# JuliaSmoothOptimizers/Krylov.jl

Measured on NVIDIA B200. Metric: CG iterations/s, higher is better.
Workload: dtype f64

## Files before the change

### include/krylov_b200.h

```cpp
#ifndef KRYLOV_B200_H
#define KRYLOV_B200_H

#ifdef __cplusplus
extern "C" {
#endif


#ifndef KRYLOV_H

#define KRYLOV_VERSION_MAJOR 0
#define KRYLOV_VERSION_MINOR 10
#define KRYLOV_VERSION_PATCH 8

typedef enum { KRYLOV_FLOAT32 = 0, KRYLOV_FLOAT64 = 1, KRYLOV_COMPLEX32 = 2, KRYLOV_COMPLEX64 = 3 } KrylovDataType;

typedef enum { KRYLOV_CPU = 0, KRYLOV_CUDA = 1 } KrylovDeviceType;

typedef enum {
  KRYLOV_CG = 0, KRYLOV_CR = 1, KRYLOV_SYMMLQ = 2, KRYLOV_MINRES = 3, KRYLOV_MINRES_QLP = 4, KRYLOV_DIOM = 5,
  KRYLOV_DQGMRES = 6, KRYLOV_FOM = 7, KRYLOV_GMRES = 8, KRYLOV_FGMRES = 9, KRYLOV_BICGSTAB = 10, KRYLOV_CGS = 11,
  KRYLOV_BILQ = 12, KRYLOV_QMR = 13, KRYLOV_USYMLQ = 14, KRYLOV_USYMQR = 15, KRYLOV_TRICG = 16, KRYLOV_TRIMR = 17,
  KRYLOV_TRILQR = 18, KRYLOV_BILQR = 19, KRYLOV_LSLQ = 20, KRYLOV_LSQR = 21, KRYLOV_LSMR = 22, KRYLOV_USYMLQR = 23,
  KRYLOV_CGLS = 24, KRYLOV_CRLS = 25, KRYLOV_CGNE = 26, KRYLOV_CRMR = 27, KRYLOV_CRAIG = 28, KRYLOV_CRAIGMR = 29,
  KRYLOV_LNLQ = 30, KRYLOV_GPMR = 31, KRYLOV_CAR = 32, KRYLOV_MINARES = 33
} KrylovSolverType;

typedef enum { KRYLOV_BLOCK_GMRES = 0, KRYLOV_BLOCK_MINRES = 1 } KrylovBlockSolverType;

typedef void (*KrylovMatvec)(const void *x, void *y, void *userdata);
typedef void (*KrylovBlockMatvec)(const void *X, void *Y, int p, void *userdata);

typedef struct {
  int memory;
  int window;
} KrylovWorkspaceOptions;

typedef struct {
  double atol;
  double rtol;
  int itmax;
  int verbose;
  double lambda;
  double tau;
  double nu;
  double timemax;
  double radius;
  int restart;
  int reorthogonalization;
  int linesearch;
} KrylovOptions;

#endif

int krylov_workspace_create(KrylovSolverType solver, int m, int n, KrylovDataType dtype, KrylovDeviceType device,
                            const KrylovWorkspaceOptions *wopts, void **ws_out);
KrylovWorkspaceOptions krylov_default_workspace_options(void);
KrylovOptions krylov_default_options(void);
void krylov_get_version(int *major, int *minor, int *patch);
int krylov_solve(void *ws, KrylovMatvec matvec_A, KrylovMatvec matvec_At, KrylovMatvec matvec_M, KrylovMatvec matvec_N,
                 const void *b, const void *c, void *userdata, const KrylovOptions *opts);
int krylov_get_x(void *ws, void *x, int n);
int krylov_get_y(void *ws, void *y, int m);
int krylov_is_solved(void *ws);
int krylov_niter(void *ws);
double krylov_elapsed_time(void *ws);
int krylov_warm_start(void *ws, const void *x0, int n);
int krylov_warm_start2(void *ws, const void *x0, const void *y0, int nx, int ny);
int krylov_workspace_free(void *ws);

int krylov_block_workspace_create(KrylovBlockSolverType solver, int m, int n, int p, KrylovDataType dtype,
                                  KrylovDeviceType device, const KrylovWorkspaceOptions *wopts, void **ws_out);
int krylov_block_solve(void *ws, KrylovBlockMatvec matvec_A, KrylovBlockMatvec matvec_M, KrylovBlockMatvec matvec_N,
                       const void *B, void *userdata, const KrylovOptions *opts);
int krylov_block_get_X(void *ws, void *X, int n, int p);
int krylov_block_is_solved(void *ws);
int krylov_block_niter(void *ws);
double krylov_block_elapsed_time(void *ws);
int krylov_block_warm_start(void *ws, const void *x0, int n, int p);
int krylov_block_workspace_free(void *ws);
long long krylov_b200_block_qr_fallbacks(void *ws);


int krylov_b200_device_count(void);
int krylov_b200_set_device(int device);
const char *krylov_b200_last_error(void);

int krylov_b200_set_operator_csr(void *ws, int n, long long nnz, const void *rowptr, const void *colind,
                                 const void *values, int index_base, int index_bytes, int location);
int krylov_b200_share_operator(void *ws, void *src);
int krylov_b200_attach_csr(void *ws, void *csr);
int krylov_b200_set_preconditioner_diag(void *ws, int which, const void *d, int location);
int krylov_b200_set_preconditioner_blockdiag(void *ws, int which, int bs, const void *blocks, int location);

#define KRYLOV_B200_CG_LANCZOS 100

typedef struct {
  int history;
  int ldiv;
  double etol;
  double conlim;
  int fused;
  int batch;
  int (*callback)(void *ws, void *user);
  void *callback_user;
  int time_kernels;
  int check_curvature;
  double cr_gamma;
} KrylovB200Options;
KrylovB200Options krylov_b200_default_options(void);
int krylov_b200_set_options(void *ws, const KrylovB200Options *opts);

typedef struct {
  int niter;
  int solved;
  int inconsistent;
  int indefinite;
  int npcCount;
  int nresiduals;
  int nAresiduals;
  int nAcond;
  double allocation_timer;
  double timer;
  char status[96];
  double Anorm;
} KrylovB200Stats;
int krylov_b200_get_stats(void *ws, KrylovB200Stats *out);
int krylov_b200_get_history(void *ws, int which, double *out, int cap);
int krylov_b200_get_vector(void *ws, const char *name, void **dev_ptr);
int krylov_b200_get_kernel_times(void *ws, double *out3);
long long krylov_b200_launch_count(void *ws);
void *krylov_b200_stream(void *ws);
int krylov_b200_wait_stream(void *ws, void *producer_stream);

int krylov_b200_dist_handle_bytes(void);
int krylov_b200_dist_init(void *ws, int rank, int world, int nhalo, const int *halo_rank, const int *halo_off);
int krylov_b200_dist_set_push(void *ws, int nranges, const int *ranges4, const int *nhalo_all);
int krylov_b200_dist_set_sendlist(void *ws, int nsend, const int *rows, const int *peers, const int *slots,
                                  const int *nhalo_all, long long nglobal);
int krylov_b200_dist_export(void *ws, void *handles_out);
int krylov_b200_dist_import(void *ws, const void *all_handles);

void *kb200_ctx_create(int device);
void kb200_ctx_destroy(void *ctx);
int kb200_sync(void *ctx);
void *kb200_alloc(long long bytes);
int kb200_free(void *p);
int kb200_h2d(void *dst, const void *src, long long bytes);
int kb200_d2h(void *dst, const void *src, long long bytes);
int kb200_dot(void *ctx, int dtype, int n, const void *x, const void *y, double *result);
int kb200_nrm2(void *ctx, int dtype, int n, const void *x, double *result);
int kb200_axpy(void *ctx, int dtype, int n, double s, const void *x, void *y);
int kb200_axpby(void *ctx, int dtype, int n, double s, const void *x, double t, void *y);
int kb200_scal(void *ctx, int dtype, int n, double s, void *x);
int kb200_copy(void *ctx, int dtype, int n, void *y, const void *x);
int kb200_scalcopy(void *ctx, int dtype, int n, void *y, double s, const void *x);
int kb200_divcopy(void *ctx, int dtype, int n, void *y, const void *x, double s);
int kb200_fill(void *ctx, int dtype, int n, void *x, double v);
void *kb200_csr_create(void *ctx, int dtype, int n, long long nnz, const void *rowptr, const void *colind,
                       const void *values, int index_base, int index_bytes, int location);
void kb200_csr_destroy(void *csr);
void *kb200_csr_read_mtx(void *ctx, const char *path, int dtype);
void *kb200_csr_transpose(void *ctx, void *csr);
int kb200_csr_info(void *csr, int *n, long long *nnz);
int kb200_csr_download(void *ctx, void *csr, int *rowptr, int *colind, void *values);
int kb200_mtx_read(const char *path, int *n, long long *nnz, int *rowptr, int *colind, double *values);
int kb200_host_householder(int m, int k, double *Q, double *R, double *tau, int compact);
int kb200_host_cholqr_factors(int p, const double *G, double *R, double *Rinv);
int kb200_host_householder_signs(int p, const double *top, double *s);
int kb200_spmv_csr(void *ctx, void *csr, const void *x, void *y, int variant);
int kb200_csr_plan(void *csr, long long *out7);

#ifdef __cplusplus
}
#endif
#endif
```

### krylov.jl_b200/csrc/capi.cu

```cuda
#include <cmath>
#include <cstring>
#include <memory>
#include <mutex>
#include <unordered_map>

#include "../../include/krylov_b200.h"
#include "kb_internal.h"
#include "block.h"
#include "mtx.h"
#include "dense_small.h"

using namespace kb;

namespace {

thread_local std::string g_last_error;
int g_device = -1;

struct CsrAny {
  int dtype = 1;
  Csr<double> d;
  Csr<float> f;
  Ctx* owner_ctx = nullptr;
  ~CsrAny() { csr_free(d); csr_free(f); }
};

struct Handle {
  int solver = 0, dtype = 1, device_kind = 0;
  bool block = false;
  int p = 0;
  void* ws = nullptr;
  std::shared_ptr<CsrAny> csr;
  void* Mdiag = nullptr;
  void* Ndiag = nullptr;
  void* Pblk[2] = {nullptr, nullptr};
  void* Pblk_inv[2] = {nullptr, nullptr};
  int Pbs[2] = {0, 0};
  KrylovB200Options ext;
  void *hx = nullptr, *hy = nullptr;
};

std::mutex g_mu;
std::unordered_map<void*, Handle*> g_handles;

Handle* lookup_any(void* p) {
  std::lock_guard<std::mutex> lk(g_mu);
  auto it = g_handles.find(p);
  return it == g_handles.end() ? nullptr : it->second;
}
Handle* lookup(void* p) { Handle* h = lookup_any(p); return (h && !h->block) ? h : nullptr; }
Handle* lookup_block(void* p) { Handle* h = lookup_any(p); return (h && h->block) ? h : nullptr; }

int fail(const char* where, const std::exception& e) {
  g_last_error = std::string(where) + ": " + e.what();
  fprintf(stderr, "[krylov_b200] %s\n", g_last_error.c_str());
  return -1;
}
int fail(const char* where, const char* msg) {
  g_last_error = std::string(where) + ": " + msg;
  fprintf(stderr, "[krylov_b200] %s\n", g_last_error.c_str());
  return -1;
}

bool supported_solver(int s) {
  return s == S_CG || s == S_MINRES || s == S_GMRES || s == S_BICGSTAB || s == S_FOM || s == S_FGMRES || s == S_CGS ||
         s == S_CG_LANCZOS || s == S_CR || s == S_DIOM || s == S_DQGMRES;
}

int pick_device() {
  int cnt = 0;
  if (cudaGetDeviceCount(&cnt) != cudaSuccess || cnt <= 0) {
    cudaGetLastError();
    throw std::runtime_error("no usable CUDA device: libkrylov_b200 has no CPU compute path");
  }
  int dev = g_device;
  if (dev < 0) { if (cudaGetDevice(&dev) != cudaSuccess) dev = 0; }
  if (dev >= cnt) throw std::runtime_error("device index out of range");
  cudaDeviceProp prop;
  KB_CUDA(cudaGetDeviceProperties(&prop, dev));
  if (prop.major < 10) throw std::runtime_error("libkrylov_b200 is built for sm_100a only");
  return dev;
}

template <class T> Workspace<T>* W(Handle* h) { return reinterpret_cast<Workspace<T>*>(h->ws); }
template <class T> BlockWorkspace<T>* BW(Handle* h) { return reinterpret_cast<BlockWorkspace<T>*>(h->ws); }
Ctx& ctx_of(Handle* h) {
  if (h->block) return h->dtype == KRYLOV_FLOAT64 ? BW<double>(h)->ctx : BW<float>(h)->ctx;
  return h->dtype == KRYLOV_FLOAT64 ? W<double>(h)->ctx : W<float>(h)->ctx;
}
int n_of(Handle* h) {
  if (h->block) return h->dtype == KRYLOV_FLOAT64 ? BW<double>(h)->n : BW<float>(h)->n;
  return h->dtype == KRYLOV_FLOAT64 ? W<double>(h)->n : W<float>(h)->n;
}
template <class T> Csr<T>& csr_of(CsrAny& a);
template <> Csr<double>& csr_of<double>(CsrAny& a) { return a.d; }
template <> Csr<float>& csr_of<float>(CsrAny& a) { return a.f; }

template <class T> void destroy_handle(Handle* h) {
  Workspace<T>* ws = W<T>(h);
  if (ws) {
    KB_CUDA(cudaSetDevice(ws->ctx.device));
    if (ws->ctx.stream) cudaStreamSynchronize(ws->ctx.stream);
  }
  h->csr.reset();
  dev_free(h->Mdiag); dev_free(h->Ndiag);
  for (int w = 0; w < 2; w++) { dev_free(h->Pblk[w]); dev_free(h->Pblk_inv[w]); }
  if (h->hx) cudaFreeHost(h->hx);
  if (h->hy) cudaFreeHost(h->hy);
  ws_destroy<T>(ws);
  delete h;
}

template <class T> const T* stage_in(Handle* h, Workspace<T>* ws, const void* src, T*& buf) {
  if (!src) return nullptr;
  if (h->device_kind == KRYLOV_CUDA) return (const T*)src;
  if (!buf) buf = dev_alloc<T>((size_t)ws->n);
  KB_CUDA(cudaMemcpyAsync(buf, src, sizeof(T) * (size_t)ws->n, cudaMemcpyHostToDevice, ws->ctx.stream));
  return buf;
}

template <class T> LinOp<T> make_cb_op(Handle* h, Workspace<T>* ws, KrylovMatvec fn, void* ud) {
  LinOp<T> op;
  op.n = ws->n;
  if (!fn) return op;
  op.fn = fn; op.userdata = ud;
  if (h->device_kind == KRYLOV_CUDA) { op.kind = LinOp<T>::DEV_CB; return op; }
  op.kind = LinOp<T>::HOST_CB;
  if (!h->hx) {
    KB_CUDA(cudaHostAlloc(&h->hx, sizeof(T) * (size_t)ws->n, cudaHostAllocDefault));
    KB_CUDA(cudaHostAlloc(&h->hy, sizeof(T) * (size_t)ws->n, cudaHostAllocDefault));
  }
  op.hx = (T*)h->hx; op.hy = (T*)h->hy;
  return op;
}

SolveOpts map_opts(const Handle* h, const KrylovOptions* o) {
  SolveOpts s;
  KrylovOptions d = krylov_default_options();
  if (!o) o = &d;
  s.atol = std::isnan(o->atol) ? -1 : o->atol;
  s.rtol = std::isnan(o->rtol) ? -1 : o->rtol;
  s.itmax = o->itmax;
  s.verbose = o->verbose;
  s.timemax = std::isnan(o->timemax) ? INFINITY : o->timemax;
  if (h->solver == S_CG || h->solver == S_CR) { s.radius = o->radius; s.linesearch = o->linesearch != 0; }
  if (h->solver == S_DIOM || h->solver == S_DQGMRES) s.reorthogonalization = o->reorthogonalization != 0;
  s.cr_gamma = std::isnan(h->ext.cr_gamma) ? -1 : h->ext.cr_gamma;
  if (h->solver == S_MINRES) { s.lambda = o->lambda; s.linesearch = o->linesearch != 0; }
  if (h->solver == S_GMRES || h->solver == S_FGMRES || h->solver == S_FOM) {
    s.restart = o->restart != 0; s.reorthogonalization = o->reorthogonalization != 0;
  }
  s.check_curvature = h->ext.check_curvature != 0;
  s.history = h->ext.history != 0;
  s.ldiv = h->ext.ldiv != 0;
  s.etol = std::isnan(h->ext.etol) ? -1 : h->ext.etol;
  s.conlim = std::isnan(h->ext.conlim) ? -1 : h->ext.conlim;
  s.fused = h->ext.fused;
  s.persist = h->ext.fused != 2;
  s.batch = h->ext.batch;
  s.callback = h->ext.callback;
  s.callback_user = h->ext.callback_user;
  s.time_kernels = h->ext.time_kernels;
  return s;
}

template <class T>
int do_solve(Handle* h, KrylovMatvec fA, KrylovMatvec fM, KrylovMatvec fN, const void* b, const void* c, void* ud,
             const KrylovOptions* opts) {
  Workspace<T>* ws = W<T>(h);
  KB_CUDA(cudaSetDevice(ws->ctx.device));
  SolveOpts so = map_opts(h, opts);
  LinOp<T> A;
  if (fA) A = make_cb_op<T>(h, ws, fA, ud);
  else if (h->csr) {
    A.kind = LinOp<T>::CSR; A.csr = &csr_of<T>(*h->csr); A.n = ws->n;
    const long long ncols = (long long)ws->n + (ws->dist.world > 1 ? ws->dist.halo.nhalo : 0);
    if (A.csr->n != ws->n || A.csr->max_col >= ncols)
      throw std::runtime_error("CSR operator: size or column index inconsistent with the workspace (n = " + std::to_string(ws->n) +
                               ", operator rows = " + std::to_string(A.csr->n) + ", largest column = " + std::to_string(A.csr->max_col) + ")");
  }
  else throw std::runtime_error("no operator: pass matvec_A or attach one with krylov_b200_set_operator_csr");
  if (A.kind == LinOp<T>::CSR && A.csr->n != ws->n) throw std::runtime_error("(workspace.m, workspace.n) is inconsistent with size(A)");
  LinOp<T> M = make_cb_op<T>(h, ws, fM, ud), N = make_cb_op<T>(h, ws, fN, ud);
  if (!fM && h->Mdiag) { M.kind = LinOp<T>::DIAG; M.diag = (const T*)h->Mdiag; }
  if (!fN && h->Ndiag) { N.kind = LinOp<T>::DIAG; N.diag = (const T*)h->Ndiag; }
  if (!fM && !h->Mdiag && h->Pblk[0]) { M.kind = LinOp<T>::BDIAG; M.blocks = (const T*)h->Pblk[0]; M.blocks_inv = (const T*)h->Pblk_inv[0]; M.bs = h->Pbs[0]; M.n = ws->n; }
  if (!fN && !h->Ndiag && h->Pblk[1]) { N.kind = LinOp<T>::BDIAG; N.blocks = (const T*)h->Pblk[1]; N.blocks_inv = (const T*)h->Pblk_inv[1]; N.bs = h->Pbs[1]; N.n = ws->n; }
  if (!b) throw std::runtime_error("b is NULL");
  const T* bd = stage_in<T>(h, ws, b, ws->bbuf);
  dist_check_alive(ws->ctx);
  switch (h->solver) {
    case S_CG: cg_solve<T>(*ws, A, bd, M, so); break;
    case S_MINRES: minres_solve<T>(*ws, A, bd, M, so); break;
    case S_GMRES: gmres_solve<T>(*ws, A, bd, M, N, so); break;
    case S_FOM: fom_solve<T>(*ws, A, bd, M, N, so); break;
    case S_FGMRES: fgmres_solve<T>(*ws, A, bd, M, N, so); break;
    case S_CG_LANCZOS: cg_lanczos_solve<T>(*ws, A, bd, M, so); break;
    case S_CR: cr_solve<T>(*ws, A, bd, M, so); break;
    case S_DQGMRES: dqgmres_solve<T>(*ws, A, bd, M, N, so); break;
    case S_DIOM: diom_solve<T>(*ws, A, bd, M, N, so); break;
    case S_CGS: {
      const T* cd = stage_in<T>(h, ws, c, ws->cbuf);
      cgs_solve<T>(*ws, A, bd, cd, M, N, so);
      break;
    }
    case S_BICGSTAB: {
      const T* cd = stage_in<T>(h, ws, c, ws->cbuf);
      bicgstab_solve<T>(*ws, A, bd, cd, M, N, so);
      break;
    }
  }
  dist_check_alive(ws->ctx);
  return 0;
}

template <class T> int do_get_x(Handle* h, void* x, int n) {
  Workspace<T>* ws = W<T>(h);
  if (n > ws->n) n = ws->n;
  KB_CUDA(cudaSetDevice(ws->ctx.device));
  KB_CUDA(cudaMemcpyAsync(x, ws->x, sizeof(T) * (size_t)n,
                          h->device_kind == KRYLOV_CUDA ? cudaMemcpyDeviceToDevice : cudaMemcpyDeviceToHost, ws->ctx.stream));
  ws->ctx.sync();
  return 0;
}

template <class T> int do_warm_start(Handle* h, const void* x0, int n) {
  Workspace<T>* ws = W<T>(h);
  if (n != ws->n) throw std::runtime_error("x0 should have size n");
  KB_CUDA(cudaSetDevice(ws->ctx.device));
  if (!ws->dx) ws->dx = dev_alloc<T>((size_t)ws->n);
  KB_CUDA(cudaMemcpyAsync(ws->dx, x0, sizeof(T) * (size_t)n,
                          h->device_kind == KRYLOV_CUDA ? cudaMemcpyDeviceToDevice : cudaMemcpyHostToDevice, ws->ctx.stream));
  ws->ctx.sync();
  ws->warm_start = true;
  return 0;
}

template <class T> Stats& stats_of(Handle* h) { return W<T>(h)->stats; }
Stats& stats_any(Handle* h) {
  if (h->block) return h->dtype == KRYLOV_FLOAT64 ? BW<double>(h)->stats : BW<float>(h)->stats;
  return h->dtype == KRYLOV_FLOAT64 ? stats_of<double>(h) : stats_of<float>(h);
}

template <class T> void* vec_by_name(Workspace<T>* ws, const char* nm) {
  struct { const char* n; T* p; } tab[] = {
      {"x", ws->x}, {"dx", ws->dx}, {"r", ws->r}, {"p", ws->p}, {"Ap", ws->Ap}, {"z", ws->z}, {"npc_dir", ws->npc_dir},
      {"v", ws->kind == S_MINRES ? (ws->vv ? ws->vv : ws->r2) : ws->v}, {"s", ws->s}, {"qd", ws->qd}, {"t", ws->t}, {"yz", ws->yz},
      {"r1", ws->r1}, {"r2", ws->r2}, {"w1", ws->w1}, {"w2", ws->w2}, {"y", ws->y}, {"w", ws->w}, {"q", ws->q},
      {"u", ws->u}, {"ts", ws->ts}, {"vw", ws->vw}, {"Mv", ws->Mv}, {"Mv_prev", ws->Mv_prev}, {"Mv_next", ws->Mv_next}};
  for (auto& e : tab) if (!strcmp(e.n, nm)) return e.p;
  if (nm[0] == 'P' && nm[1]) { int i = atoi(nm + 1); if (i >= 1 && i <= (int)ws->Z.size()) return ws->Z[i - 1]; return nullptr; }
  if (!strcmp(nm, "Ar")) return ws->Ap;
  if (!strcmp(nm, "Mq")) return ws->z;
  if (nm[0] == 'Z') { int i = atoi(nm + 1); if (i >= 1 && i <= (int)ws->Z.size()) return ws->Z[i - 1]; return nullptr; }
  if (nm[0] == 'V') { int i = atoi(nm + 1); if (i >= 1 && i <= (int)ws->V.size()) return ws->V[i - 1]; }
  return nullptr;
}

}

extern "C" {

int krylov_workspace_create(KrylovSolverType solver, int m, int n, KrylovDataType dtype, KrylovDeviceType device,
                            const KrylovWorkspaceOptions* wopts, void** ws_out) {
  try {
    if (!supported_solver((int)solver) || (dtype != KRYLOV_FLOAT32 && dtype != KRYLOV_FLOAT64)) return -2;
    if (device != KRYLOV_CPU && device != KRYLOV_CUDA) return fail("krylov_workspace_create", "unknown device");
    if (!ws_out) return fail("krylov_workspace_create", "ws_out is NULL");
    if (m < 0 || n < 0) return fail("krylov_workspace_create", "negative dimension");
    const int dev = pick_device();
    const int memory = wopts ? wopts->memory : 0, window = wopts ? wopts->window : 0;
    Handle* h = new Handle();
    h->solver = (int)solver; h->dtype = (int)dtype; h->device_kind = (int)device;
    h->ext = krylov_b200_default_options();
    try {
      if (dtype == KRYLOV_FLOAT64) h->ws = ws_create<double>((SolverKind)solver, m, n, memory, window, dev);
      else h->ws = ws_create<float>((SolverKind)solver, m, n, memory, window, dev);
    } catch (...) { delete h; throw; }
    {
      std::lock_guard<std::mutex> lk(g_mu);
      g_handles[h] = h;
    }
    *ws_out = h;
    return 0;
  } catch (const std::exception& e) { return fail("krylov_workspace_create", e); }
}

KrylovWorkspaceOptions krylov_default_workspace_options(void) { KrylovWorkspaceOptions w = {0, 0}; return w; }

KrylovOptions krylov_default_options(void) {
  KrylovOptions o;
  o.atol = NAN; o.rtol = NAN; o.itmax = 0; o.verbose = 0; o.lambda = 0.0; o.tau = NAN; o.nu = NAN;
  o.timemax = NAN; o.radius = 0.0; o.restart = 0; o.reorthogonalization = 0; o.linesearch = 0;
  return o;
}

void krylov_get_version(int* major, int* minor, int* patch) {
  if (major) *major = KRYLOV_VERSION_MAJOR;
  if (minor) *minor = KRYLOV_VERSION_MINOR;
  if (patch) *patch = KRYLOV_VERSION_PATCH;
}

int krylov_solve(void* ws, KrylovMatvec matvec_A, KrylovMatvec matvec_At, KrylovMatvec matvec_M, KrylovMatvec matvec_N,
                 const void* b, const void* c, void* userdata, const KrylovOptions* opts) {
  (void)matvec_At;
  try {
    Handle* h = lookup(ws);
    if (!h) return fail("krylov_solve", "unknown workspace handle");
    return h->dtype == KRYLOV_FLOAT64 ? do_solve<double>(h, matvec_A, matvec_M, matvec_N, b, c, userdata, opts)
                                      : do_solve<float>(h, matvec_A, matvec_M, matvec_N, b, c, userdata, opts);
  } catch (const std::exception& e) { return fail("krylov_solve", e); }
}

int krylov_get_x(void* ws, void* x, int n) {
  try {
    Handle* h = lookup(ws);
    if (!h) return fail("krylov_get_x", "unknown workspace handle");
    return h->dtype == KRYLOV_FLOAT64 ? do_get_x<double>(h, x, n) : do_get_x<float>(h, x, n);
  } catch (const std::exception& e) { return fail("krylov_get_x", e); }
}

int krylov_get_y(void* ws, void* y, int m) {
  (void)y; (void)m;
  Handle* h = lookup(ws);
  if (!h) return fail("krylov_get_y", "unknown workspace handle");
  return -2;
}

int krylov_is_solved(void* ws) { Handle* h = lookup(ws); return h ? (stats_any(h).solved ? 1 : 0) : -1; }
int krylov_niter(void* ws) { Handle* h = lookup(ws); return h ? stats_any(h).niter : -1; }
double krylov_elapsed_time(void* ws) { Handle* h = lookup(ws); return h ? stats_any(h).timer : -1.0; }

int krylov_warm_start(void* ws, const void* x0, int n) {
  try {
    Handle* h = lookup(ws);
    if (!h) return fail("krylov_warm_start", "unknown workspace handle");
    return h->dtype == KRYLOV_FLOAT64 ? do_warm_start<double>(h, x0, n) : do_warm_start<float>(h, x0, n);
  } catch (const std::exception& e) { return fail("krylov_warm_start", e); }
}

int krylov_warm_start2(void* ws, const void* x0, const void* y0, int nx, int ny) {
  (void)x0; (void)y0; (void)nx; (void)ny;
  Handle* h = lookup(ws);
  if (!h) return fail("krylov_warm_start2", "unknown workspace handle");
  return -2;
}

static void destroy_any(Handle* h) {
  if (h->block) {
    Ctx& c = ctx_of(h);
    KB_CUDA(cudaSetDevice(c.device));
    if (c.stream) cudaStreamSynchronize(c.stream);
    h->csr.reset();
    dev_free(h->Mdiag); dev_free(h->Ndiag);
    if (h->hx) cudaFreeHost(h->hx);
    if (h->hy) cudaFreeHost(h->hy);
    if (h->dtype == KRYLOV_FLOAT64) block_ws_destroy<double>(BW<double>(h)); else block_ws_destroy<float>(BW<float>(h));
    delete h;
  } else if (h->dtype == KRYLOV_FLOAT64) {
    destroy_handle<double>(h);
  } else {
    destroy_handle<float>(h);
  }
}

int krylov_workspace_free(void* ws) {
  Handle* h = nullptr;
  {
    std::lock_guard<std::mutex> lk(g_mu);
    auto it = g_handles.find(ws);
    if (it == g_handles.end()) return 1;
    h = it->second;
    g_handles.erase(it);
  }
  try {
    destroy_any(h);
  } catch (const std::exception& e) { fail("krylov_workspace_free", e); }
  return 0;
}

int krylov_block_workspace_create(KrylovBlockSolverType solver, int m, int n, int p, KrylovDataType dtype, KrylovDeviceType device,
                                  const KrylovWorkspaceOptions* wopts, void** ws_out) {
  try {
    if (solver != KRYLOV_BLOCK_GMRES || (dtype != KRYLOV_FLOAT32 && dtype != KRYLOV_FLOAT64)) return -2;
    if (device != KRYLOV_CPU && device != KRYLOV_CUDA) return fail("krylov_block_workspace_create", "unknown device");
    if (!ws_out) return fail("krylov_block_workspace_create", "ws_out is NULL");
    if (m < 0 || n < 0 || p < 1) return fail("krylov_block_workspace_create", "bad dimensions");
    const int dev = pick_device();
    const int memory = wopts ? wopts->memory : 0;
    Handle* h = new Handle();
    h->block = true; h->p = p; h->solver = (int)solver; h->dtype = (int)dtype; h->device_kind = (int)device;
    h->ext = krylov_b200_default_options();
    try {
      if (dtype == KRYLOV_FLOAT64) h->ws = block_ws_create<double>(m, n, p, memory, dev);
      else h->ws = block_ws_create<float>(m, n, p, memory, dev);
    } catch (...) { delete h; throw; }
    {
      std::lock_guard<std::mutex> lk(g_mu);
      g_handles[h] = h;
    }
    *ws_out = h;
    return 0;
  } catch (const std::exception& e) { return fail("krylov_block_workspace_create", e); }
}

}
namespace {
template <class T> BlockOp<T> make_block_cb(Handle* h, KrylovBlockMatvec fn, void* ud) {
  BlockOp<T> op;
  if (!fn) return op;
  op.fn = fn; op.userdata = ud;
  op.kind = h->device_kind == KRYLOV_CUDA ? BlockOp<T>::DEV_CB : BlockOp<T>::HOST_CB;
  return op;
}
template <class T> const T* stage_block(Handle* h, BlockWorkspace<T>* ws, const void* src) {
  if (h->device_kind == KRYLOV_CUDA) return (const T*)src;
  const size_t np = (size_t)ws->n * ws->p;
  if (!ws->tmp2) ws->tmp2 = dev_alloc<T>(np);
  KB_CUDA(cudaMemcpyAsync(ws->tmp2, src, sizeof(T) * np, cudaMemcpyHostToDevice, ws->ctx.stream));
  return ws->tmp2;
}
template <class T> int do_block_solve(Handle* h, KrylovBlockMatvec fA, KrylovBlockMatvec fM, KrylovBlockMatvec fN, const void* B,
                                      void* ud, const KrylovOptions* opts) {
  BlockWorkspace<T>* ws = BW<T>(h);
  KB_CUDA(cudaSetDevice(ws->ctx.device));
  SolveOpts so = map_opts(h, opts);
  KrylovOptions d = krylov_default_options();
  const KrylovOptions* o = opts ? opts : &d;
  so.restart = o->restart != 0; so.reorthogonalization = o->reorthogonalization != 0;
  BlockOp<T> A = make_block_cb<T>(h, fA, ud);
  if (!fA) {
    if (!h->csr) throw std::runtime_error("no operator: pass matvec_A or attach one with krylov_b200_set_operator_csr");
    A.kind = BlockOp<T>::CSR; A.csr = &csr_of<T>(*h->csr);
    if (A.csr->n != ws->n) throw std::runtime_error("(workspace.m, workspace.n) is inconsistent with size(A)");
  }
  BlockOp<T> M = make_block_cb<T>(h, fM, ud), N = make_block_cb<T>(h, fN, ud);
  if (!fM && h->Mdiag) { M.kind = BlockOp<T>::DIAG; M.diag = (const T*)h->Mdiag; }
  if (!fN && h->Ndiag) { N.kind = BlockOp<T>::DIAG; N.diag = (const T*)h->Ndiag; }
  if (!B) throw std::runtime_error("B is NULL");
  const T* Bd = stage_block<T>(h, ws, B);
  block_gmres_solve<T>(*ws, A, Bd, M, N, so);
  return 0;
}
template <class T> int do_block_get_X(Handle* h, void* X, int n, int p) {
  BlockWorkspace<T>* ws = BW<T>(h);
  if (n != ws->n || p != ws->p) throw std::runtime_error("X should have size n x p");
  KB_CUDA(cudaSetDevice(ws->ctx.device));
  const size_t np = (size_t)n * p;
  if (h->device_kind == KRYLOV_CUDA) { block_get_X<T>(*ws, (T*)X); return 0; }
  block_get_X<T>(*ws, ws->tmp);
  KB_CUDA(cudaMemcpyAsync(X, ws->tmp, sizeof(T) * np, cudaMemcpyDeviceToHost, ws->ctx.stream));
  ws->ctx.sync();
  return 0;
}
template <class T> int do_block_warm_start(Handle* h, const void* X0, int n, int p) {
  BlockWorkspace<T>* ws = BW<T>(h);
  if (n != ws->n || p != ws->p) throw std::runtime_error("X0 should have size n x p");
  KB_CUDA(cudaSetDevice(ws->ctx.device));
  block_warm_start<T>(*ws, stage_block<T>(h, ws, X0));
  return 0;
}
}
extern "C" {

int krylov_block_solve(void* ws, KrylovBlockMatvec matvec_A, KrylovBlockMatvec matvec_M, KrylovBlockMatvec matvec_N, const void* B,
                       void* userdata, const KrylovOptions* opts) {
  try {
    Handle* h = lookup_block(ws);
    if (!h) return fail("krylov_block_solve", "unknown block workspace handle");
    return h->dtype == KRYLOV_FLOAT64 ? do_block_solve<double>(h, matvec_A, matvec_M, matvec_N, B, userdata, opts)
                                      : do_block_solve<float>(h, matvec_A, matvec_M, matvec_N, B, userdata, opts);
  } catch (const std::exception& e) { return fail("krylov_block_solve", e); }
}
int krylov_block_get_X(void* ws, void* X, int n, int p) {
  try {
    Handle* h = lookup_block(ws);
    if (!h || !X) return fail("krylov_block_get_X", "bad arguments");
    return h->dtype == KRYLOV_FLOAT64 ? do_block_get_X<double>(h, X, n, p) : do_block_get_X<float>(h, X, n, p);
  } catch (const std::exception& e) { return fail("krylov_block_get_X", e); }
}
int krylov_block_is_solved(void* ws) { Handle* h = lookup_block(ws); return h ? (stats_any(h).solved ? 1 : 0) : -1; }
int krylov_block_niter(void* ws) { Handle* h = lookup_block(ws); return h ? stats_any(h).niter : -1; }
double krylov_block_elapsed_time(void* ws) { Handle* h = lookup_block(ws); return h ? stats_any(h).timer : -1.0; }
int krylov_block_warm_start(void* ws, const void* x0, int n, int p) {
  try {
    Handle* h = lookup_block(ws);
    if (!h || !x0) return fail("krylov_block_warm_start", "bad arguments");
    return h->dtype == KRYLOV_FLOAT64 ? do_block_warm_start<double>(h, x0, n, p) : do_block_warm_start<float>(h, x0, n, p);
  } catch (const std::exception& e) { return fail("krylov_block_warm_start", e); }
}
long long krylov_b200_block_qr_fallbacks(void* ws) {
  Handle* h = lookup_block(ws);
  if (!h) return -1;
  return h->dtype == KRYLOV_FLOAT64 ? BW<double>(h)->qr_fallbacks : BW<float>(h)->qr_fallbacks;
}
int krylov_block_workspace_free(void* ws) {
  try {
    Handle* h = lookup_block(ws);
    if (!h) return 1;
    {
      std::lock_guard<std::mutex> lk(g_mu);
      g_handles.erase(ws);
    }
    destroy_any(h);
    return 0;
  } catch (const std::exception& e) { return fail("krylov_block_workspace_free", e); }
}

int krylov_b200_device_count(void) {
  int cnt = 0;
  if (cudaGetDeviceCount(&cnt) != cudaSuccess) { cudaGetLastError(); return 0; }
  return cnt;
}
int krylov_b200_set_device(int device) { g_device = device; return 0; }
const char* krylov_b200_last_error(void) { return g_last_error.c_str(); }

int krylov_b200_set_operator_csr(void* ws, int n, long long nnz, const void* rowptr, const void* colind, const void* values,
                                 int index_base, int index_bytes, int location) {
  try {
    Handle* h = lookup_any(ws);
    if (!h) return fail("krylov_b200_set_operator_csr", "unknown workspace handle");
    auto a = std::make_shared<CsrAny>();
    a->dtype = h->dtype;
    Ctx& cx = ctx_of(h);
    KB_CUDA(cudaSetDevice(cx.device));
    if (n != n_of(h)) throw std::runtime_error("(workspace.m, workspace.n) is inconsistent with size(A)");
    if (h->dtype == KRYLOV_FLOAT64)
      csr_upload<double>(cx, a->d, n, nnz, rowptr, colind, (const double*)values, index_base, index_bytes, location != 0);
    else
      csr_upload<float>(cx, a->f, n, nnz, rowptr, colind, (const float*)values, index_base, index_bytes, location != 0);
    h->csr = a;
    return 0;
  } catch (const std::exception& e) { return fail("krylov_b200_set_operator_csr", e); }
}

int krylov_b200_share_operator(void* ws, void* src) {
  Handle* h = lookup_any(ws); Handle* s = lookup_any(src);
  if (!h || !s) return fail("krylov_b200_share_operator", "unknown workspace handle");
  if (!s->csr || s->dtype != h->dtype) return fail("krylov_b200_share_operator", "source has no CSR operator of this dtype");
  h->csr = s->csr;
  return 0;
}

int krylov_b200_attach_csr(void* ws, void* csr) {
  Handle* h = lookup_any(ws);
  if (!h || !csr) return fail("krylov_b200_attach_csr", "bad arguments");
  CsrAny* a = (CsrAny*)csr;
  if (a->dtype != h->dtype) return fail("krylov_b200_attach_csr", "dtype mismatch");
  h->csr = std::shared_ptr<CsrAny>(std::shared_ptr<CsrAny>(), a);
  return 0;
}

int krylov_b200_set_preconditioner_diag(void* ws, int which, const void* d, int location) {
  try {
    Handle* h = lookup_any(ws);
    if (!h) return fail("krylov_b200_set_preconditioner_diag", "unknown workspace handle");
    void*& slot = which == 0 ? h->Mdiag : h->Ndiag;
    if (!d) { dev_free(slot); slot = nullptr; return 0; }
    const size_t esz = h->dtype == KRYLOV_FLOAT64 ? 8 : 4;
    const int n = n_of(h);
    KB_CUDA(cudaSetDevice(ctx_of(h).device));
    if (!slot) slot = dev_alloc<char>(esz * (size_t)n);
    KB_CUDA(cudaMemcpy(slot, d, esz * (size_t)n, location ? cudaMemcpyDeviceToDevice : cudaMemcpyHostToDevice));
    return 0;
  } catch (const std::exception& e) { return fail("krylov_b200_set_preconditioner_diag", e); }
}

int krylov_b200_set_preconditioner_blockdiag(void* ws, int which, int bs, const void* blocks, int location) {
  try {
    Handle* h = lookup(ws);
    if (!h) return fail("krylov_b200_set_preconditioner_blockdiag", "unknown (single right-hand side) workspace handle");
    if (which != 0 && which != 1) return fail("krylov_b200_set_preconditioner_blockdiag", "which must be 0 (M) or 1 (N)");
    dev_free(h->Pblk[which]); dev_free(h->Pblk_inv[which]);
    h->Pblk[which] = h->Pblk_inv[which] = nullptr; h->Pbs[which] = 0;
    if (!blocks) return 0;
    if (bs < 2 || bs > 8) return fail("krylov_b200_set_preconditioner_blockdiag", "block size must be in 2..8");
    const size_t esz = h->dtype == KRYLOV_FLOAT64 ? 8 : 4;
    const int n = n_of(h);
    const size_t cnt = (size_t)((n + bs - 1) / bs) * bs * bs;
    Ctx& c = ctx_of(h);
    KB_CUDA(cudaSetDevice(c.device));
    h->Pblk[which] = dev_alloc<char>(esz * cnt);
    h->Pblk_inv[which] = dev_alloc<char>(esz * cnt);
    h->Pbs[which] = bs;
    KB_CUDA(cudaMemcpyAsync(h->Pblk[which], blocks, esz * cnt, location ? cudaMemcpyDeviceToDevice : cudaMemcpyHostToDevice, c.stream));
    int* dsing = nullptr;
    KB_CUDA(cudaMalloc((void**)&dsing, sizeof(int)));
    KB_CUDA(cudaMemsetAsync(dsing, 0, sizeof(int), c.stream));
    if (h->dtype == KRYLOV_FLOAT64) k_blockdiag_invert<double>(c, n, bs, (const double*)h->Pblk[which], (double*)h->Pblk_inv[which], dsing);
    else k_blockdiag_invert<float>(c, n, bs, (const float*)h->Pblk[which], (float*)h->Pblk_inv[which], dsing);
    int sing = 0;
    KB_CUDA(cudaMemcpyAsync(&sing, dsing, sizeof(int), cudaMemcpyDeviceToHost, c.stream));
    c.sync();
    cudaFree(dsing);
    if (sing) fprintf(stderr, "[krylov_b200] warning: a diagonal block of the block-Jacobi preconditioner is singular (its inverse, used by ldiv = true, is zero)\n");
    return 0;
  } catch (const std::exception& e) { return fail("krylov_b200_set_preconditioner_blockdiag", e); }
}

KrylovB200Options krylov_b200_default_options(void) {
  KrylovB200Options o;
  memset(&o, 0, sizeof(o));
  o.etol = NAN; o.conlim = NAN; o.fused = 1; o.cr_gamma = NAN;
  return o;
}

int krylov_b200_set_options(void* ws, const KrylovB200Options* opts) {
  Handle* h = lookup_any(ws);
  if (!h) return fail("krylov_b200_set_options", "unknown workspace handle");
  h->ext = opts ? *opts : krylov_b200_default_options();
  return 0;
}

int krylov_b200_get_stats(void* ws, KrylovB200Stats* out) {
  Handle* h = lookup_any(ws);
  if (!h || !out) return fail("krylov_b200_get_stats", "unknown workspace handle");
  const Stats& s = stats_any(h);
  memset(out, 0, sizeof(*out));
  out->niter = s.niter; out->solved = s.solved; out->inconsistent = s.inconsistent; out->indefinite = s.indefinite;
  out->npcCount = s.npcCount; out->nresiduals = (int)s.residuals.size(); out->nAresiduals = (int)s.Aresiduals.size();
  out->nAcond = (int)s.Acond.size(); out->allocation_timer = s.allocation_timer; out->timer = s.timer;
  strncpy(out->status, s.status.c_str(), sizeof(out->status) - 1);
  out->Anorm = s.Anorm;
  return 0;
}

int krylov_b200_get_history(void* ws, int which, double* out, int cap) {
  Handle* h = lookup_any(ws);
  if (!h) return fail("krylov_b200_get_history", "unknown workspace handle");
  if (!out || cap < 0) return fail("krylov_b200_get_history", "bad arguments (out is NULL or cap < 0)");
  const Stats& s = stats_any(h);
  const std::vector<double>& v = which == 0 ? s.residuals : which == 1 ? s.Aresiduals : s.Acond;
  int k = (int)v.size() < cap ? (int)v.size() : cap;
  for (int i = 0; i < k; i++) out[i] = v[i];
  return k;
}

int krylov_b200_get_vector(void* ws, const char* name, void** dev_ptr) {
  Handle* h = lookup(ws);
  if (!h || !name || !dev_ptr) return fail("krylov_b200_get_vector", "bad arguments");
  void* p = h->dtype == KRYLOV_FLOAT64 ? vec_by_name<double>(W<double>(h), name) : vec_by_name<float>(W<float>(h), name);
  *dev_ptr = p;
  return p ? 0 : -2;
}

int krylov_b200_get_kernel_times(void* ws, double* out) {
  Handle* h = lookup(ws);
  if (!h || !out) return fail("krylov_b200_get_kernel_times", "bad arguments");
  if (h->dtype == KRYLOV_FLOAT64) { auto* w = W<double>(h); out[0] = w->k1_ms; out[1] = w->k2_ms; out[2] = w->timed_pairs; }
  else { auto* w = W<float>(h); out[0] = w->k1_ms; out[1] = w->k2_ms; out[2] = w->timed_pairs; }
  return 0;
}

long long krylov_b200_launch_count(void* ws) {
  Handle* h = lookup_any(ws);
  if (!h) return -1;
  return ctx_of(h).launches;
}

void* krylov_b200_stream(void* ws) {
  Handle* h = lookup_any(ws);
  if (!h) return nullptr;
  return (void*)ctx_of(h).stream;
}

int krylov_b200_wait_stream(void* ws, void* producer_stream) {
  try {
    Handle* h = lookup_any(ws);
    if (!h) return fail("krylov_b200_wait_stream", "unknown workspace handle");
    Ctx& c = ctx_of(h);
    KB_CUDA(cudaSetDevice(c.device));
    cudaEvent_t ev;
    KB_CUDA(cudaEventCreateWithFlags(&ev, cudaEventDisableTiming));
    cudaError_t e1 = cudaEventRecord(ev, (cudaStream_t)producer_stream);
    cudaError_t e2 = e1 == cudaSuccess ? cudaStreamWaitEvent(c.stream, ev, 0) : e1;
    cudaEventDestroy(ev);
    if (e2 != cudaSuccess) throw std::runtime_error(cudaGetErrorString(e2));
    return 0;
  } catch (const std::exception& e) { return fail("krylov_b200_wait_stream", e); }
}

}
namespace {
constexpr int kIpcHandles = 6;
constexpr size_t kMailBytes = kMailWords * sizeof(unsigned long long);

template <class T> int dist_init_t(Handle* h, int rank, int world, int nhalo, const int* halo_rank, const int* halo_off) {
  Workspace<T>* ws = W<T>(h);
  if (world < 1 || world > kMaxRanks || rank < 0 || rank >= world) throw std::runtime_error("bad rank/world");
  KB_CUDA(cudaSetDevice(ws->ctx.device));
  if (h->solver == S_CG) {
    KB_CUDA(cudaStreamSynchronize(ws->ctx.stream));
    const size_t len = (size_t)ws->n + (size_t)(nhalo > 0 ? nhalo : 0);
    T** bufs[3] = {&ws->r, &ws->p, &ws->p2};
    for (T** b : bufs) {
      dev_free(*b);
      *b = dev_alloc<T>(len);
      KB_CUDA(cudaMemset(*b, 0, sizeof(T) * len));
    }
  }
  ws->dist.rank = rank; ws->dist.world = world;
  int *dr = nullptr, *dof = nullptr;
  KB_CUDA(cudaMalloc((void**)&dr, sizeof(int) * (size_t)(nhalo > 0 ? nhalo : 1)));
  KB_CUDA(cudaMalloc((void**)&dof, sizeof(int) * (size_t)(nhalo > 0 ? nhalo : 1)));
  if (nhalo > 0) {
    KB_CUDA(cudaMemcpy(dr, halo_rank, sizeof(int) * (size_t)nhalo, cudaMemcpyHostToDevice));
    KB_CUDA(cudaMemcpy(dof, halo_off, sizeof(int) * (size_t)nhalo, cudaMemcpyHostToDevice));
  }
  ws->dist.halo = HaloMap{ws->n, nhalo, dr, dof};
  KB_CUDA(cudaMalloc(&ws->dist.mailbox, kMailBytes));
  KB_CUDA(cudaMemset(ws->dist.mailbox, 0, kMailBytes));
  ws->dist.halo_buf = dev_alloc<T>(3 * (size_t)(nhalo > 0 ? nhalo : 1));
  KB_CUDA(cudaMemset(ws->dist.halo_buf, 0, sizeof(T) * 3 * (size_t)(nhalo > 0 ? nhalo : 1)));
  ws->dist.npush = 0;
  ws->dist.xhalo = dev_alloc<T>(2 * (size_t)(nhalo > 0 ? nhalo : 1));
  KB_CUDA(cudaMemset(ws->dist.xhalo, 0, sizeof(T) * 2 * (size_t)(nhalo > 0 ? nhalo : 1)));
  ws->dist.nglobal = ws->n;
  if (h->solver != S_CG) for (int i = 0; i < 3; i++) KB_CUDA(cudaMalloc(&ws->dist.dummy[i], 256));
  return 0;
}

template <class T> int dist_export_t(Handle* h, void* out) {
  Workspace<T>* ws = W<T>(h);
  if (!ws->dist.mailbox) throw std::runtime_error("call krylov_b200_dist_init first");
  KB_CUDA(cudaSetDevice(ws->ctx.device));
  cudaIpcMemHandle_t* hs = (cudaIpcMemHandle_t*)out;
  void* vr = ws->kind == S_CG ? (void*)ws->r : ws->dist.dummy[0];
  void* vp = ws->kind == S_CG ? (void*)ws->p : ws->dist.dummy[1];
  void* vp2 = ws->kind == S_CG ? (void*)ws->p2 : ws->dist.dummy[2];
  void* ptrs[kIpcHandles] = {vr, vp, vp2, ws->dist.mailbox, ws->dist.halo_buf, ws->dist.xhalo};
  for (int i = 0; i < kIpcHandles; i++) KB_CUDA(cudaIpcGetMemHandle(&hs[i], ptrs[i]));
  return 0;
}

template <class T> int dist_import_t(Handle* h, const void* all) {
  Workspace<T>* ws = W<T>(h);
  auto& D = ws->dist;
  KB_CUDA(cudaSetDevice(ws->ctx.device));
  const cudaIpcMemHandle_t* hs = (const cudaIpcMemHandle_t*)all;
  DistComm hc;
  memset(&hc, 0, sizeof(hc));
  hc.rank = D.rank; hc.world = D.world;
  {
    const char* es = getenv("KB200_DIST_TIMEOUT_S");
    double secs = es ? atof(es) : 30.0;
    if (!(secs > 0)) secs = 30.0;
    int khz = 0;
    cudaDeviceGetAttribute(&khz, cudaDevAttrClockRate, ws->ctx.device);
    hc.timeout_cycles = (long long)(secs * 1e3 * (khz > 0 ? khz : 1965000));
  }
  for (int k = 0; k < D.world; k++) {
    void* ptr[kIpcHandles];
    if (k == D.rank) {
      ptr[0] = ws->r; ptr[1] = ws->p; ptr[2] = ws->p2; ptr[3] = D.mailbox; ptr[4] = D.halo_buf; ptr[5] = D.xhalo;
    } else {
      for (int i = 0; i < kIpcHandles; i++) {
        KB_CUDA(cudaIpcOpenMemHandle(&ptr[i], hs[k * kIpcHandles + i], cudaIpcMemLazyEnablePeerAccess));
        D.opened.push_back(ptr[i]);
      }
    }
    D.r_peer[k] = (T*)ptr[0]; D.bufA_peer[k] = (T*)ptr[1]; D.bufB_peer[k] = (T*)ptr[2];
    D.halo_buf_peer[k] = (T*)ptr[4];
    D.xhalo_peer[k] = (T*)ptr[5];
    hc.mail[k] = (unsigned long long*)ptr[3];
  }
  D.swapped = false;
  DistExchange* ex = ws->ctx.dex ? ws->ctx.dex : new DistExchange();
  memset(ex, 0, sizeof(*ex));
  ex->nsend = D.nsend; ex->send_row = D.send_row; ex->send_peer = D.send_peer; ex->send_slot = D.send_slot;
  for (int k = 0; k < D.world; k++) { ex->xhalo_peer[k] = D.xhalo_peer[k]; ex->nhalo_peer[k] = D.nhalo_peer[k]; }
  ex->xhalo = D.xhalo; ex->nhalo = D.halo.nhalo; ex->nloc = ws->n; ex->count = 0;
  ws->ctx.dex = ex;
  if (!ws->ctx.dcomm) KB_CUDA(cudaMalloc((void**)&ws->ctx.dcomm, sizeof(DistComm)));
  KB_CUDA(cudaMemcpy(ws->ctx.dcomm, &hc, sizeof(DistComm), cudaMemcpyHostToDevice));
  return 0;
}
}
extern "C" {

int krylov_b200_dist_handle_bytes(void) { return (int)(kIpcHandles * sizeof(cudaIpcMemHandle_t)); }

int krylov_b200_dist_init(void* ws, int rank, int world, int nhalo, const int* halo_rank, const int* halo_off) {
  try {
    Handle* h = lookup(ws);
    if (!h) return fail("krylov_b200_dist_init", "unknown workspace handle");
    return h->dtype == KRYLOV_FLOAT64 ? dist_init_t<double>(h, rank, world, nhalo, halo_rank, halo_off)
                                      : dist_init_t<float>(h, rank, world, nhalo, halo_rank, halo_off);
  } catch (const std::exception& e) { return fail("krylov_b200_dist_init", e); }
}
int krylov_b200_dist_set_sendlist(void* ws, int nsend, const int* rows, const int* peers, const int* slots,
                                  const int* nhalo_all, long long nglobal) {
  try {
    Handle* h = lookup(ws);
    if (!h) return fail("krylov_b200_dist_set_sendlist", "unknown workspace handle");
    auto apply = [&](auto* w) {
      KB_CUDA(cudaSetDevice(w->ctx.device));
      auto up = [&](const int* src) {
        int* d = nullptr;
        KB_CUDA(cudaMalloc((void**)&d, sizeof(int) * (size_t)(nsend > 0 ? nsend : 1)));
        if (nsend > 0) KB_CUDA(cudaMemcpy(d, src, sizeof(int) * (size_t)nsend, cudaMemcpyHostToDevice));
        return d;
      };
      w->dist.send_row = up(rows); w->dist.send_peer = up(peers); w->dist.send_slot = up(slots);
      w->dist.nsend = nsend;
      for (int k = 0; k < w->dist.world; k++) w->dist.nhalo_peer[k] = nhalo_all[k];
      w->dist.nglobal = nglobal;
    };
    if (h->dtype == KRYLOV_FLOAT64) apply(W<double>(h)); else apply(W<float>(h));
    return 0;
  } catch (const std::exception& e) { return fail("krylov_b200_dist_set_sendlist", e); }
}
int krylov_b200_dist_set_push(void* ws, int nranges, const int* ranges4, const int* nhalo_all) {
  try {
    Handle* h = lookup(ws);
    if (!h) return fail("krylov_b200_dist_set_push", "unknown workspace handle");
    if (nranges < 0 || nranges > kMaxPushRanges) return fail("krylov_b200_dist_set_push", "too many ranges (pull mode stays on)");
    auto apply = [&](auto* w) {
      for (int q = 0; q < nranges; q++) w->dist.push[q] = PushRange{ranges4[4 * q], ranges4[4 * q + 1], ranges4[4 * q + 2], ranges4[4 * q + 3]};
      for (int k = 0; k < w->dist.world; k++) w->dist.nhalo_peer[k] = nhalo_all[k];
      w->dist.npush = nranges;
    };
    if (h->dtype == KRYLOV_FLOAT64) apply(W<double>(h)); else apply(W<float>(h));
    return 0;
  } catch (const std::exception& e) { return fail("krylov_b200_dist_set_push", e); }
}
int krylov_b200_dist_export(void* ws, void* handles_out) {
  try {
    Handle* h = lookup(ws);
    if (!h) return fail("krylov_b200_dist_export", "unknown workspace handle");
    return h->dtype == KRYLOV_FLOAT64 ? dist_export_t<double>(h, handles_out) : dist_export_t<float>(h, handles_out);
  } catch (const std::exception& e) { return fail("krylov_b200_dist_export", e); }
}
int krylov_b200_dist_import(void* ws, const void* all_handles) {
  try {
    Handle* h = lookup(ws);
    if (!h) return fail("krylov_b200_dist_import", "unknown workspace handle");
    return h->dtype == KRYLOV_FLOAT64 ? dist_import_t<double>(h, all_handles) : dist_import_t<float>(h, all_handles);
  } catch (const std::exception& e) { return fail("krylov_b200_dist_import", e); }
}

void* kb200_ctx_create(int device) {
  try {
    if (device < 0) device = pick_device();
    Ctx* c = new Ctx();
    c->init(device);
    return c;
  } catch (const std::exception& e) { fail("kb200_ctx_create", e); return nullptr; }
}
void kb200_ctx_destroy(void* ctx) {
  Ctx* c = (Ctx*)ctx;
  if (!c) return;
  cudaSetDevice(c->device);
  if (c->stream) cudaStreamSynchronize(c->stream);
  c->destroy();
  delete c;
}
int kb200_sync(void* ctx) {
  try { ((Ctx*)ctx)->sync(); return 0; } catch (const std::exception& e) { return fail("kb200_sync", e); }
}
void* kb200_alloc(long long bytes) {
  try { return dev_alloc<char>((size_t)bytes); } catch (const std::exception& e) { fail("kb200_alloc", e); return nullptr; }
}
int kb200_free(void* p) { dev_free(p); return 0; }
int kb200_h2d(void* dst, const void* src, long long bytes) {
  return cudaMemcpy(dst, src, (size_t)bytes, cudaMemcpyHostToDevice) == cudaSuccess ? 0 : fail("kb200_h2d", "cudaMemcpy failed");
}
int kb200_d2h(void* dst, const void* src, long long bytes) {
  return cudaMemcpy(dst, src, (size_t)bytes, cudaMemcpyDeviceToHost) == cudaSuccess ? 0 : fail("kb200_d2h", "cudaMemcpy failed");
}

#define FLAT(name, body_d, body_f)                                                        \
  try {                                                                                   \
    Ctx& c = *(Ctx*)ctx;                                                                  \
    if (dtype == KRYLOV_FLOAT64) { typedef double T; (void)sizeof(T); body_d; }           \
    else if (dtype == KRYLOV_FLOAT32) { typedef float T; (void)sizeof(T); body_f; }       \
    else return -2;                                                                       \
    return 0;                                                                             \
  } catch (const std::exception& e) { return fail(name, e); }

int kb200_dot(void* ctx, int dtype, int n, const void* x, const void* y, double* result) {
  FLAT("kb200_dot", *result = k_dot<T>(c, n, (const T*)x, (const T*)y), *result = k_dot<T>(c, n, (const T*)x, (const T*)y))
}
int kb200_nrm2(void* ctx, int dtype, int n, const void* x, double* result) {
  FLAT("kb200_nrm2", *result = k_nrm2<T>(c, n, (const T*)x), *result = k_nrm2<T>(c, n, (const T*)x))
}
int kb200_axpy(void* ctx, int dtype, int n, double s, const void* x, void* y) {
  FLAT("kb200_axpy", k_axpy<T>(c, n, (T)s, (const T*)x, (T*)y), k_axpy<T>(c, n, (T)s, (const T*)x, (T*)y))
}
int kb200_axpby(void* ctx, int dtype, int n, double s, const void* x, double t, void* y) {
  FLAT("kb200_axpby", k_axpby<T>(c, n, (T)s, (const T*)x, (T)t, (T*)y), k_axpby<T>(c, n, (T)s, (const T*)x, (T)t, (T*)y))
}
int kb200_scal(void* ctx, int dtype, int n, double s, void* x) {
  FLAT("kb200_scal", k_scal<T>(c, n, (T)s, (T*)x), k_scal<T>(c, n, (T)s, (T*)x))
}
int kb200_copy(void* ctx, int dtype, int n, void* y, const void* x) {
  FLAT("kb200_copy", k_copy<T>(c, n, (T*)y, (const T*)x), k_copy<T>(c, n, (T*)y, (const T*)x))
}
int kb200_scalcopy(void* ctx, int dtype, int n, void* y, double s, const void* x) {
  FLAT("kb200_scalcopy", k_scalcopy<T>(c, n, (T*)y, (T)s, (const T*)x), k_scalcopy<T>(c, n, (T*)y, (T)s, (const T*)x))
}
int kb200_divcopy(void* ctx, int dtype, int n, void* y, const void* x, double s) {
  FLAT("kb200_divcopy", k_divcopy<T>(c, n, (T*)y, (const T*)x, (T)s), k_divcopy<T>(c, n, (T*)y, (const T*)x, (T)s))
}
int kb200_fill(void* ctx, int dtype, int n, void* x, double v) {
  FLAT("kb200_fill", k_fill<T>(c, n, (T*)x, (T)v), k_fill<T>(c, n, (T*)x, (T)v))
}

void* kb200_csr_create(void* ctx, int dtype, int n, long long nnz, const void* rowptr, const void* colind, const void* values,
                       int index_base, int index_bytes, int location) {
  try {
    Ctx& c = *(Ctx*)ctx;
    CsrAny* a = new CsrAny();
    a->dtype = dtype; a->owner_ctx = &c;
    try {
      if (dtype == KRYLOV_FLOAT64) csr_upload<double>(c, a->d, n, nnz, rowptr, colind, (const double*)values, index_base, index_bytes, location != 0);
      else if (dtype == KRYLOV_FLOAT32) csr_upload<float>(c, a->f, n, nnz, rowptr, colind, (const float*)values, index_base, index_bytes, location != 0);
      else throw std::runtime_error("unsupported dtype");
    } catch (...) { delete a; throw; }
    return a;
  } catch (const std::exception& e) { fail("kb200_csr_create", e); return nullptr; }
}
void kb200_csr_destroy(void* csr) { delete (CsrAny*)csr; }

void* kb200_csr_read_mtx(void* ctx, const char* path, int dtype) {
  try {
    if (!ctx || !path) throw std::runtime_error("bad arguments");
    Ctx& c = *(Ctx*)ctx;
    HostCsr h;
    read_matrix_market(path, h);
    CsrAny* a = new CsrAny();
    a->dtype = dtype; a->owner_ctx = &c;
    try {
      if (dtype == KRYLOV_FLOAT64) csr_from_host<double>(c, a->d, h);
      else if (dtype == KRYLOV_FLOAT32) csr_from_host<float>(c, a->f, h);
      else throw std::runtime_error("unsupported dtype");
    } catch (...) { delete a; throw; }
    return a;
  } catch (const std::exception& e) { fail("kb200_csr_read_mtx", e); return nullptr; }
}

void* kb200_csr_transpose(void* ctx, void* csr) {
  try {
    if (!ctx || !csr) throw std::runtime_error("bad arguments");
    Ctx& c = *(Ctx*)ctx;
    CsrAny* src = (CsrAny*)csr;
    HostCsr h, ht;
    if (src->dtype == KRYLOV_FLOAT64) csr_to_host<double>(c, src->d, h); else csr_to_host<float>(c, src->f, h);
    transpose_csr(h, ht);
    CsrAny* a = new CsrAny();
    a->dtype = src->dtype; a->owner_ctx = &c;
    try {
      if (a->dtype == KRYLOV_FLOAT64) csr_from_host<double>(c, a->d, ht); else csr_from_host<float>(c, a->f, ht);
    } catch (...) { delete a; throw; }
    return a;
  } catch (const std::exception& e) { fail("kb200_csr_transpose", e); return nullptr; }
}

int kb200_csr_info(void* csr, int* n, long long* nnz) {
  CsrAny* a = (CsrAny*)csr;
  if (!a) return -1;
  if (n) *n = a->dtype == KRYLOV_FLOAT64 ? a->d.n : a->f.n;
  if (nnz) *nnz = a->dtype == KRYLOV_FLOAT64 ? a->d.nnz : a->f.nnz;
  return 0;
}

int kb200_csr_download(void* ctx, void* csr, int* rowptr, int* colind, void* values) {
  try {
    if (!ctx || !csr) throw std::runtime_error("bad arguments");
    Ctx& c = *(Ctx*)ctx;
    CsrAny* a = (CsrAny*)csr;
    HostCsr h;
    if (a->dtype == KRYLOV_FLOAT64) csr_to_host<double>(c, a->d, h); else csr_to_host<float>(c, a->f, h);
    if (rowptr) for (size_t i = 0; i < h.rowptr.size(); i++) rowptr[i] = (int)h.rowptr[i];
    if (colind) for (size_t i = 0; i < h.colind.size(); i++) colind[i] = (int)h.colind[i];
    if (values) {
      if (a->dtype == KRYLOV_FLOAT64) std::memcpy(values, h.val.data(), sizeof(double) * h.val.size());
      else for (size_t i = 0; i < h.val.size(); i++) ((float*)values)[i] = (float)h.val[i];
    }
    return 0;
  } catch (const std::exception& e) { return fail("kb200_csr_download", e); }
}

int kb200_mtx_read(const char* path, int* n, long long* nnz, int* rowptr, int* colind, double* values) {
  try {
    if (!path) throw std::runtime_error("path is NULL");
    HostCsr h;
    read_matrix_market(path, h);
    if (n) *n = h.n;
    if (nnz) *nnz = (long long)h.colind.size();
    if (rowptr) for (size_t i = 0; i < h.rowptr.size(); i++) rowptr[i] = (int)h.rowptr[i];
    if (colind) for (size_t i = 0; i < h.colind.size(); i++) colind[i] = (int)h.colind[i];
    if (values) std::memcpy(values, h.val.data(), sizeof(double) * h.val.size());
    return 0;
  } catch (const std::exception& e) { return fail("kb200_mtx_read", e); }
}

int kb200_host_householder(int m, int k, double* Q, double* R, double* tau, int compact) {
  if (!Q || !R || !tau || m < k || k < 1) return fail("kb200_host_householder", "bad arguments");
  dense::householder_compact<double>(m, k, Q, R, tau);
  if (!compact) dense::org2r<double>(m, k, Q, m, tau);
  return 0;
}

int kb200_host_cholqr_factors(int p, const double* G, double* R, double* Rinv) {
  if (!G || !R || !Rinv || p < 1) return fail("kb200_host_cholqr_factors", "bad arguments");
  if (!dense::cholesky_upper<double>(p, G, R)) return 1;
  dense::inv_upper<double>(p, R, Rinv);
  return 0;
}

int kb200_host_householder_signs(int p, const double* top, double* s) {
  if (!top || !s || p < 1) return fail("kb200_host_householder_signs", "bad arguments");
  std::vector<double> W(top, top + (size_t)p * p);
  dense::householder_signs<double>(p, W.data(), s);
  return 0;
}

int kb200_spmv_csr(void* ctx, void* csr, const void* x, void* y, int variant) {
  try {
    Ctx& c = *(Ctx*)ctx;
    CsrAny* a = (CsrAny*)csr;
    if (a->dtype == KRYLOV_FLOAT64) k_spmv<double>(c, a->d, (const double*)x, (double*)y, variant);
    else k_spmv<float>(c, a->f, (const float*)x, (float*)y, variant);
    return 0;
  } catch (const std::exception& e) { return fail("kb200_spmv_csr", e); }
}

int kb200_csr_plan(void* csr, long long* out) {
  CsrAny* a = (CsrAny*)csr;
  if (!a || !out) return -1;
  if (a->dtype == KRYLOV_FLOAT64) {
    const Csr<double>& A = a->d;
    out[0] = A.ntiles; out[1] = A.tile_cap; out[2] = A.max_row; out[3] = A.tma_ok; out[4] = A.stages; out[5] = A.grid; out[6] = (long long)A.smem_bytes;
  } else {
    const Csr<float>& A = a->f;
    out[0] = A.ntiles; out[1] = A.tile_cap; out[2] = A.max_row; out[3] = A.tma_ok; out[4] = A.stages; out[5] = A.grid; out[6] = (long long)A.smem_bytes;
  }
  return 0;
}

}
```

### krylov.jl_b200/csrc/cg_fused.cu

```cuda
#include "solver_common.h"
#include "spmv_tiles.cuh"

namespace kb {

constexpr int kHist = 64;

template <class T>
struct CgState {
  T gamma, pAp, alpha, beta, pNorm2, rNorm, eps_tol, pad0;
  int iter, itmax, done, linesearch;
  int solved, tired, zero_curvature, inconsistent;
  int npc, not_spd, comm_error, pad2;
  T hist[kHist];
};

static_assert(sizeof(CgState<double>) % 8 == 0 && sizeof(CgState<float>) % 8 == 0, "CgState is copied as 8-byte words");

template <class T>
struct CgPeers {
  HaloMap halo;
  const T* r[kMaxRanks];
  const T* p_old[kMaxRanks];
  const T* mdiag;
  const T* r_halo;
  const T* p_halo_old;
  PushPlan<T> push_p;
};

template <class T>
__device__ __forceinline__ void cg_k1_finalize(CgState<T>* st, T pAp) {
  st->pAp = pAp;
  const T lim = mul_rn(Eps<T>::v, st->pNorm2);
  if (pAp <= lim) {
    if (fabs(pAp) <= lim) { st->zero_curvature = 1; st->inconsistent = !st->linesearch; }
    if (st->linesearch) { st->npc = 1; st->solved = 1; }
    if (st->zero_curvature || st->solved) { st->done = 1; return; }
  }
  st->alpha = div_rn(st->gamma, pAp);
}

template <class T>
__device__ __forceinline__ void cg_k2_finalize(CgState<T>* st, T gamma_next) {
  if (!(gamma_next >= T(0))) { st->not_spd = 1; st->done = 1; return; }
  const T rNorm = sqrt_rn(gamma_next);
  st->rNorm = rNorm;
  const int it1 = st->iter + 1;
  st->hist[it1 % kHist] = rNorm;
  const bool solved = (rNorm <= st->eps_tol) || (add_rn(rNorm, T(1)) <= T(1));
  if (!solved) {
    const T beta = div_rn(gamma_next, st->gamma);
    st->beta = beta;
    st->pNorm2 = add_rn(gamma_next, mul_rn(mul_rn(beta, beta), st->pNorm2));
    st->gamma = gamma_next;
  }
  st->iter = it1;
  st->solved = solved;
  st->tired = it1 >= st->itmax;
  st->done = solved || st->tired;
}

template <class T>
__device__ __forceinline__ bool cg_global_sum(CgState<T>* st, DistComm* dc, T& v) {
  if (dc) {
    v = dist_reduce(dc, v);
    if (dc->error) { st->comm_error = 1; st->done = 1; return false; }
  }
  return true;
}

constexpr int kPlain = 0, kDist = 1, kJacobi = 2, kBlockJac = 3;

template <class T, int MODE>
struct PVal {
  const T* r; const T* p_old; T beta; const CgPeers<T>* peers;
  const T* mdiag;
  __device__ __forceinline__ T operator()(int j) const {
    if (MODE == kDist && j >= peers->halo.nloc) {
      const int h = j - peers->halo.nloc;
      if (peers->r_halo)
        return add_rn(__ldg(&peers->r_halo[h]), mul_rn(beta, __ldg(&peers->p_halo_old[h])));
      const int rk = __ldg(&peers->halo.src_rank[h]), off = __ldg(&peers->halo.src_off[h]);
      return add_rn(__ldg(&peers->r[rk][off]), mul_rn(beta, __ldg(&peers->p_old[rk][off])));
    }
    T z = __ldg(&r[j]);
    if (MODE == kJacobi) z = mul_rn(__ldg(&mdiag[j]), z);
    return add_rn(z, mul_rn(beta, __ldg(&p_old[j])));
  }
};

template <class T> struct RowPre { T pn, po, xr; };

template <class T, int MODE, int MINB, bool XUP>
__global__ void __launch_bounds__(kTileThreads, MINB) cg_k1_tma(Csr<T> A, const T* __restrict__ r, const T* __restrict__ p_old,
                                                          T* __restrict__ p_new, T* __restrict__ Ap, CgState<T>* st,
                                                          T* part, unsigned* ticket, DistComm* dc, CgPeers<T> peers,
                                                          T* __restrict__ x) {
  extern __shared__ __align__(128) unsigned char smem[];
  __shared__ T sm[32];
  if (*(volatile int*)&st->done) return;
  T dacc = T(0);
  bool sent = false;
  const T beta = st->beta, alpha_prev = st->alpha;
  const bool xup = XUP && st->iter > 0;
  const PVal<T, MODE> pval{r, p_old, beta, &peers, peers.mdiag};
  auto row_begin = [&](int row) {
    RowPre<T> q;
    q.po = __ldg(&p_old[row]);
    T z = __ldg(&r[row]);
    if (MODE == kJacobi) z = mul_rn(__ldg(&peers.mdiag[row]), z);
    q.pn = add_rn(z, mul_rn(beta, q.po));
    q.xr = xup ? x[row] : T(0);
    return q;
  };
  spmv_tiles_run<T>(A, smem, pval, row_begin, [&](int row, T acc, RowPre<T> q) {
    p_new[row] = q.pn;
    if (MODE == kDist) sent |= peers.push_p(row, q.pn);
    Ap[row] = acc;
    if (xup) x[row] = add_rn(q.xr, mul_rn(alpha_prev, q.po));
    dacc += q.pn * acc;
  });
  if (MODE == kDist && sent) __threadfence_system();
  T mine[1] = {block_sum(dacc, sm)}, tot[1];
  if (grid_sum_last<T, 1>(mine, part, ticket, sm, tot) && threadIdx.x == 0) {
    if (cg_global_sum(st, MODE == kDist ? dc : nullptr, tot[0])) cg_k1_finalize(st, tot[0]);
  }
}

template <class T, int MODE, bool XUP>
__global__ void __launch_bounds__(kBlock) cg_k1_rows(Csr<T> A, const T* __restrict__ r, const T* __restrict__ p_old,
                                                     T* __restrict__ p_new, T* __restrict__ Ap, CgState<T>* st, T* part,
                                                     unsigned* ticket, DistComm* dc, CgPeers<T> peers, T* __restrict__ x) {
  __shared__ T sm[32];
  if (*(volatile int*)&st->done) return;
  T dacc = T(0);
  bool sent = false;
  const T alpha_prev = st->alpha;
  const bool xup = XUP && st->iter > 0;
  const PVal<T, MODE> pval{r, p_old, st->beta, &peers, peers.mdiag};
  const int stride = gridDim.x * blockDim.x;
  for (int row = blockIdx.x * blockDim.x + threadIdx.x; row < A.n; row += stride) {
    const int kb = A.rowptr[row], ke = A.rowptr[row + 1];
    T acc = T(0);
    for (int k = kb; k < ke; k++) acc = add_rn(acc, mul_rn(A.val[k], pval(A.colind[k])));
    const T pn = pval(row);
    p_new[row] = pn;
    if (MODE == kDist) sent |= peers.push_p(row, pn);
    Ap[row] = acc;
    if (xup) x[row] = add_rn(x[row], mul_rn(alpha_prev, __ldg(&p_old[row])));
    dacc += pn * acc;
  }
  if (MODE == kDist && sent) __threadfence_system();
  T mine[1] = {block_sum(dacc, sm)}, tot[1];
  if (grid_sum_last<T, 1>(mine, part, ticket, sm, tot) && threadIdx.x == 0) {
    if (cg_global_sum(st, MODE == kDist ? dc : nullptr, tot[0])) cg_k1_finalize(st, tot[0]);
  }
}

template <class T, int MODE, bool XK2>
__global__ void __launch_bounds__(kBlock) cg_k2(int n, T* __restrict__ x, T* __restrict__ r, const T* __restrict__ p,
                                                const T* __restrict__ Ap, CgState<T>* st, T* part, unsigned* ticket,
                                                DistComm* dc, const T* __restrict__ mdiag, PushPlan<T> push_r) {
  __shared__ T sm[32];
  if (*(volatile int*)&st->done) return;
  const T alpha = st->alpha, nalpha = -alpha;
  T acc = T(0);
  bool sent = false;
  const int stride = gridDim.x * blockDim.x;
  int i = blockIdx.x * blockDim.x + threadIdx.x;
  for (; i + 3 * stride < n; i += 4 * stride) {
    T xv[4], rv[4], pv[4], av[4];
#pragma unroll
    for (int u = 0; u < 4; u++) {
      const int j = i + u * stride;
      rv[u] = r[j]; av[u] = __ldg(&Ap[j]);
      if (XK2) { xv[u] = x[j]; pv[u] = __ldg(&p[j]); }
    }
#pragma unroll
    for (int u = 0; u < 4; u++) {
      const int j = i + u * stride;
      if (XK2) x[j] = add_rn(xv[u], mul_rn(alpha, pv[u]));
      const T rn = add_rn(rv[u], mul_rn(nalpha, av[u]));
      r[j] = rn;
      if (MODE == kDist) sent |= push_r(j, rn);
      acc += rn * (MODE == kJacobi ? mul_rn(__ldg(&mdiag[j]), rn) : rn);
    }
  }
  for (; i < n; i += stride) {
    const int j = i;
    if (XK2) x[j] = add_rn(x[j], mul_rn(alpha, p[j]));
    const T rn = add_rn(r[j], mul_rn(nalpha, Ap[j]));
    r[j] = rn;
    if (MODE == kDist) sent |= push_r(j, rn);
    acc += rn * (MODE == kJacobi ? mul_rn(__ldg(&mdiag[j]), rn) : rn);
  }
  if (MODE == kDist && sent) __threadfence_system();
  T mine[1] = {block_sum(acc, sm)}, tot[1];
  if (grid_sum_last<T, 1>(mine, part, ticket, sm, tot) && threadIdx.x == 0) {
    if (cg_global_sum(st, dc, tot[0])) cg_k2_finalize(st, tot[0]);
  }
}

struct GridBar { unsigned count, gen, halo_ready, timed_iters; unsigned long long ns_a, ns_b; };

__device__ __forceinline__ unsigned ld_acquire_gpu_u32(const unsigned* p) {
  unsigned v;
  asm volatile("ld.acquire.gpu.global.u32 %0, [%1];" : "=r"(v) : "l"(p) : "memory");
  return v;
}
__device__ __forceinline__ void st_release_gpu_u32(unsigned* p, unsigned v) {
  asm volatile("st.release.gpu.global.u32 [%0], %1;" ::"l"(p), "r"(v) : "memory");
}
__device__ __forceinline__ double ld_sys(const double* p) {
  double v;
  asm volatile("ld.relaxed.sys.global.f64 %0, [%1];" : "=d"(v) : "l"(p) : "memory");
  return v;
}
__device__ __forceinline__ float ld_sys(const float* p) {
  float v;
  asm volatile("ld.relaxed.sys.global.f32 %0, [%1];" : "=f"(v) : "l"(p) : "memory");
  return v;
}

template <class T> struct CgScal { T alpha, beta; int iter, done; };
template <class T>
__device__ __forceinline__ void cg_load_scal(const CgState<T>* st, CgScal<T>* sc) {
  const volatile CgState<T>* v = st;
  const T al = v->alpha, be = v->beta;
  const int it = v->iter, dn = v->done;
  sc->alpha = al; sc->beta = be; sc->iter = it; sc->done = dn;
}

template <class T, class Fin>
__device__ __forceinline__ bool grid_reduce_barrier(GridBar* gb, T v, T* part, T* sm, unsigned* sflag, const CgState<T>* st,
                                                    CgScal<T>* sc, Fin fin) {
  const T mine = block_sum(v, sm);
  if (threadIdx.x == 0) {
    const unsigned g = *(volatile unsigned*)&gb->gen;
    __stcg(&part[blockIdx.x], mine);
    __threadfence();
    const unsigned t = atomicAdd(&gb->count, 1u);
    sflag[0] = (t == gridDim.x - 1);
    sflag[1] = g;
  }
  __syncthreads();
  const bool last = sflag[0] != 0;
  const unsigned g = sflag[1];
  bool ok = true;
  if (last) {
    if (threadIdx.x < 32) {
      __threadfence();
      T acc = T(0);
      for (int i = threadIdx.x; i < (int)gridDim.x; i += 32) acc += __ldcg(&part[i]);
      const T tot = warp_sum(acc);
      fin(tot);
      __syncwarp();
      if (threadIdx.x == 0) {
        cg_load_scal<T>(st, sc);
        gb->count = 0u;
        st_release_gpu_u32(&gb->gen, g + 1u);
      }
    }
  } else if (threadIdx.x == 0) {
    const long long t0 = clock64();
    while (ld_acquire_gpu_u32(&gb->gen) == g) {
      if (clock64() - t0 > 120000000000LL) { sflag[0] = 2; break; }
    }
    cg_load_scal<T>(st, sc);
  }
  __syncthreads();
  if (sflag[0] == 2) ok = false;
  __syncthreads();
  return ok;
}

template <class T>
struct CgPeerTab {
  const T* r[kMaxRanks];
  const T* p[2][kMaxRanks];
};

template <class T>
struct CgPersistArgs {
  T* r; T* P0; T* P1; T* Ap; T* x;
  const T* mdiag;
  T* z;
  const T* mblocks;
  int mbs;
  HaloMap halo;
  const CgPeerTab<T>* tab;
  const int* tile_order;
  int n_interior;
  int max_iters;
  int timed;
  CgState<T>* hsnap;
  unsigned long long* hseq;
  unsigned long long seq;
};

template <class T>
__device__ __forceinline__ void cg_report_to_host(const CgPersistArgs<T>& a, const CgState<T>* st) {
  if (blockIdx.x != 0 || threadIdx.x >= 32 || a.hsnap == nullptr) return;
  const unsigned long long* src = reinterpret_cast<const unsigned long long*>(st);
  unsigned long long* dst = reinterpret_cast<unsigned long long*>(a.hsnap);
  for (int w = threadIdx.x; w < (int)(sizeof(CgState<T>) / 8); w += 32) dst[w] = __ldcg(&src[w]);
  __threadfence_system();
  __syncwarp();
  if (threadIdx.x == 0) { *(volatile unsigned long long*)a.hseq = a.seq; __threadfence_system(); }
}

__device__ __forceinline__ unsigned long long globaltimer_ns() {
  unsigned long long t;
  asm volatile("mov.u64 %0, %globaltimer;" : "=l"(t));
  return t;
}

template <class T, int BS>
__device__ __forceinline__ T cg_phase_b_block(int n, int bs_rt, T nalpha, T* r, const T* Ap, T* z, const T* __restrict__ B, int first, int stride) {
  const int bs = BS ? BS : bs_rt;
  const int nb = (n + bs - 1) / bs;
  T acc = T(0);
  for (int blk = first; blk < nb; blk += stride) {
    const int r0 = blk * bs, rows = min(bs, n - r0);
    T rn[BS ? BS : 8];
#pragma unroll
    for (int i = 0; i < (BS ? BS : 8); i++)
      if (i < rows) { rn[i] = add_rn(r[r0 + i], mul_rn(nalpha, Ap[r0 + i])); r[r0 + i] = rn[i]; }
    const T* Bk = B + (size_t)blk * bs * bs;
#pragma unroll
    for (int i = 0; i < (BS ? BS : 8); i++) {
      if (i < rows) {
        T zi = T(0);
#pragma unroll
        for (int j = 0; j < (BS ? BS : 8); j++)
          if (j < rows) zi = add_rn(zi, mul_rn(__ldg(&Bk[i * bs + j]), rn[j]));
        z[r0 + i] = zi;
        acc += rn[i] * zi;
      }
    }
  }
  return acc;
}

template <class T>
__device__ __forceinline__ void cg_stage_halo(HaloMap halo, const CgPeerTab<T>* tab, T* r, T* p_old, int pb, int G, int tid, int nthreads) {
  const int nh = halo.nhalo, nloc = halo.nloc;
  const int per = (nh + G - 1) / G;
  const int h0 = (int)blockIdx.x * per, h1 = min(nh, h0 + per);
  for (int h = h0 + tid; h < h1; h += nthreads) {
    const int rk = __ldg(&halo.src_rank[h]), off = __ldg(&halo.src_off[h]);
    const T rv = ld_sys(tab->r[rk] + off);
    const T pv = ld_sys(tab->p[pb][rk] + off);
    __stcg(&r[nloc + h], rv);
    __stcg(&p_old[nloc + h], pv);
  }
}

template <class T, int MODE, int MINB, int DEPTH>
__global__ void __launch_bounds__(kTileThreads, MINB) cg_persist(Csr<T> A, CgPersistArgs<T> a, CgState<T>* st, T* part,
                                                                GridBar* gb, DistComm* dc) {
  extern __shared__ __align__(128) unsigned char smem[];
  __shared__ T sm[32];
  __shared__ unsigned sflag[2];
  __shared__ CgScal<T> sc;
  volatile CgState<T>* vst = st;
  if (vst->done) { cg_report_to_host<T>(a, st); return; }
  if (threadIdx.x == 0) cg_load_scal<T>(st, &sc);
  TilePipe<T> P;
  P.init(A, smem);
  const int G = gridDim.x, tid = threadIdx.x, warp = tid >> 5, lane = tid & 31;
  const int cnt = (A.ntiles - (int)blockIdx.x + G - 1) / G;
  auto tile_at = [&](int j) -> int {
    const int q = blockIdx.x + j * G;
    return MODE == kDist ? __ldg(&a.tile_order[q]) : q;
  };
  const int cnt_int = MODE == kDist ? max(0, min(cnt, (a.n_interior - (int)blockIdx.x + G - 1) / G)) : cnt;
  const unsigned pre = (unsigned)min(P.S, cnt);
  const uint64_t pol = l2_evict_first_policy();
  unsigned ppos = 0, cpos = 0;
  int passes = 0;
  const int n = A.n;
  for (int k = 0; k < a.max_iters; k++) {
    const int iter = sc.iter;
    const T beta = sc.beta, alpha_prev = sc.alpha;
    const bool xup = iter > 0;
    T* p_old = (iter & 1) ? a.P1 : a.P0;
    T* p_new = (iter & 1) ? a.P0 : a.P1;
    T dacc = T(0);
    const bool timing = a.timed && blockIdx.x == 0 && tid == 0;
    unsigned long long t0 = 0, t1 = 0;
    if (timing) t0 = globaltimer_ns();
    if (warp == kConsumerWarps) {
      if (lane == 0) {
        const unsigned target = (unsigned)(k + 1) * (unsigned)cnt + (k + 1 < a.max_iters ? pre : 0u);
        tile_issue_until<T>(A, P, ppos, target, cnt, tile_at, pol);
      }
    } else {
      const T* r = MODE == kBlockJac ? a.z : a.r;
      const T* mdiag = a.mdiag;
      auto gather = [&](int j) -> T {
        T z = r[j];
        if (MODE == kJacobi) z = mul_rn(__ldg(&mdiag[j]), z);
        return add_rn(z, mul_rn(beta, p_old[j]));
      };
      auto row_begin = [&](int row) {
        RowPre<T> q;
        q.po = p_old[row];
        T z = r[row];
        if (MODE == kJacobi) z = mul_rn(__ldg(&mdiag[row]), z);
        q.pn = add_rn(z, mul_rn(beta, q.po));
        q.xr = xup ? a.x[row] : T(0);
        return q;
      };
      auto row_done = [&](int row, T acc, RowPre<T> q) {
        p_new[row] = q.pn;
        a.Ap[row] = acc;
        if (xup) a.x[row] = add_rn(q.xr, mul_rn(alpha_prev, q.po));
        dacc += q.pn * acc;
      };
      if (MODE == kDist) {
        cg_stage_halo<T>(a.halo, a.tab, a.r, p_old, iter & 1, G, tid, kTileRows);
        __threadfence();
        __syncwarp();
        if (lane == 0) atomicAdd(&gb->halo_ready, 1u);
        tile_consume_pass<T, DEPTH>(A, P, cpos, 0, cnt_int, tile_at, gather, row_begin, row_done);
        if (cnt_int < cnt) {
          if (lane == 0) { while (ld_acquire_gpu_u32(&gb->halo_ready) < (unsigned)(G * kConsumerWarps)) { } }
          __syncwarp();
          tile_consume_pass<T, DEPTH>(A, P, cpos, cnt_int, cnt, tile_at, gather, row_begin, row_done);
        }
      } else {
        tile_consume_pass<T, DEPTH>(A, P, cpos, 0, cnt, tile_at, gather, row_begin, row_done);
      }
    }
    passes = k + 1;
    bool ok = grid_reduce_barrier<T>(gb, dacc, part, sm, sflag, st, &sc, [&](T tot) {
      if (MODE == kDist) {
        tot = (T)dist_allreduce_sum_warp<T>(dc, (double)tot);
        if (*(volatile int*)&dc->error) { if (lane == 0) { st->comm_error = 1; st->done = 1; } return; }
      }
      if (lane == 0) cg_k1_finalize(st, tot);
    });
    if (!ok || sc.done) break;
    if (timing) t1 = globaltimer_ns();
    {
      const T alpha = sc.alpha, nalpha = -alpha;
      T* r = a.r;
      const T* Ap = a.Ap;
      const T* mdiag = a.mdiag;
      T acc = T(0);
      const int stride = G * kTileThreads;
      int i = (int)blockIdx.x * kTileThreads + tid;
      if (MODE == kBlockJac) {
        if (a.mbs == 4) acc = cg_phase_b_block<T, 4>(n, 4, nalpha, r, Ap, a.z, a.mblocks, i, stride);
        else if (a.mbs == 2) acc = cg_phase_b_block<T, 2>(n, 2, nalpha, r, Ap, a.z, a.mblocks, i, stride);
        else if (a.mbs == 8) acc = cg_phase_b_block<T, 8>(n, 8, nalpha, r, Ap, a.z, a.mblocks, i, stride);
        else acc = cg_phase_b_block<T, 0>(n, a.mbs, nalpha, r, Ap, a.z, a.mblocks, i, stride);
        i = n;
      }
      for (; i + 3 * stride < n; i += 4 * stride) {
        T rv[4], av[4];
#pragma unroll
        for (int u = 0; u < 4; u++) { rv[u] = r[i + u * stride]; av[u] = Ap[i + u * stride]; }
#pragma unroll
        for (int u = 0; u < 4; u++) {
          const int j = i + u * stride;
          const T rn = add_rn(rv[u], mul_rn(nalpha, av[u]));
          r[j] = rn;
          acc += rn * (MODE == kJacobi ? mul_rn(__ldg(&mdiag[j]), rn) : rn);
        }
      }
      for (; i < n; i += stride) {
        const T rn = add_rn(r[i], mul_rn(nalpha, Ap[i]));
        r[i] = rn;
        acc += rn * (MODE == kJacobi ? mul_rn(__ldg(&mdiag[i]), rn) : rn);
      }
      ok = grid_reduce_barrier<T>(gb, acc, part, sm, sflag, st, &sc, [&](T tot) {
        if (MODE == kDist) {
          tot = (T)dist_allreduce_sum_warp<T>(dc, (double)tot);
          if (*(volatile int*)&dc->error) { if (lane == 0) { st->comm_error = 1; st->done = 1; } return; }
        }
        if (lane == 0) {
          cg_k2_finalize(st, tot);
          gb->halo_ready = 0u;
        }
      });
      if (timing) {
        const unsigned long long t2 = globaltimer_ns();
        gb->ns_a += t1 - t0; gb->ns_b += t2 - t1; gb->timed_iters += 1;
      }
      if (!ok || sc.done) break;
    }
  }
  if (warp == kConsumerWarps && lane == 0) tile_drain<T>(P, (unsigned)passes * (unsigned)cnt, ppos);
  cg_report_to_host<T>(a, st);
}

template <class T>
__global__ void push_ranges_kernel(const T* __restrict__ v, PushPlan<T> plan) {
  const int stride = gridDim.x * blockDim.x, tid = blockIdx.x * blockDim.x + threadIdx.x;
  for (int q = 0; q < plan.nranges; q++)
    for (int d = tid; d < plan.rg[q].count; d += stride) plan.dst[q][plan.rg[q].slot + d] = v[plan.rg[q].start + d];
  __threadfence_system();
}

template <class T> void cg_dist_push_r(Workspace<T>& ws) {
  if (ws.dist.world <= 1 || ws.dist.npush <= 0) return;
  PushPlan<T> plan;
  memset(&plan, 0, sizeof(plan));
  plan.nranges = ws.dist.npush;
  for (int q = 0; q < ws.dist.npush; q++) { plan.rg[q] = ws.dist.push[q]; plan.dst[q] = ws.dist.halo_buf_peer[plan.rg[q].peer]; }
  push_ranges_kernel<T><<<sm_count(), kBlock, 0, ws.ctx.stream>>>(ws.r, plan);
  KB_CUDA(cudaGetLastError());
  ws.ctx.launches++;
}

constexpr size_t kOffGridBar = 1024, kOffPeerTab = 2048, kOffHostSeq = 3072;

template <class T> void cg_fused_prepare(Workspace<T>& ws) {
  static_assert(sizeof(CgState<T>) <= kOffGridBar && sizeof(CgPeerTab<T>) <= kFusedBlockBytes - kOffPeerTab, "block layout");
  if (!ws.fused_state) {
    KB_CUDA(cudaMalloc(&ws.fused_state, kFusedBlockBytes));
    KB_CUDA(cudaMemset(ws.fused_state, 0, kFusedBlockBytes));
    KB_CUDA(cudaHostAlloc(&ws.fused_host, kFusedBlockBytes, cudaHostAllocPortable | cudaHostAllocMapped));
    memset(ws.fused_host, 0, kFusedBlockBytes);
  }
  if (!ws.p2) ws.p2 = dev_alloc<T>((size_t)ws.n);
  for (int i = 0; i < 2; i++)
    if (!ws.fused_ev[i]) KB_CUDA(cudaEventCreateWithFlags(&ws.fused_ev[i], cudaEventDisableTiming));
}

template <class T>
__global__ void tile_halo_flags_kernel(Csr<T> A, int nloc, int* flags) {
  const int warp = (blockIdx.x * blockDim.x + threadIdx.x) >> 5, lane = threadIdx.x & 31;
  const int nw = (gridDim.x * blockDim.x) >> 5;
  for (int t = warp; t < A.ntiles; t += nw) {
    const int k0 = A.rowptr[t * kTileRows], k1 = A.rowptr[min(t * kTileRows + kTileRows, A.n)];
    bool any = false;
    for (int k = k0 + lane; k < k1; k += 32) any |= A.colind[k] >= nloc;
    any = __any_sync(0xffffffffu, any);
    if (lane == 0) flags[t] = any ? 1 : 0;
  }
}

template <class T> void cg_dist_tile_order(Workspace<T>& ws, const Csr<T>& A) {
  if (ws.dist.tile_order && ws.dist.tile_order_for == (const void*)A.rowptr && ws.dist.tile_order_n == A.ntiles) return;
  Ctx& c = ws.ctx;
  if (ws.dist.tile_order) { cudaFree(ws.dist.tile_order); ws.dist.tile_order = nullptr; }
  const int nt = A.ntiles;
  KB_CUDA(cudaMalloc((void**)&ws.dist.tile_order, sizeof(int) * (size_t)(nt > 0 ? nt : 1)));
  if (nt > 0) {
    tile_halo_flags_kernel<T><<<sm_count() * 4, 256, 0, c.stream>>>(A, ws.n, ws.dist.tile_order);
    KB_CUDA(cudaGetLastError());
    std::vector<int> fl(nt), ord;
    KB_CUDA(cudaMemcpyAsync(fl.data(), ws.dist.tile_order, sizeof(int) * nt, cudaMemcpyDeviceToHost, c.stream));
    c.sync();
    ord.reserve(nt);
    for (int t = 0; t < nt; t++) if (!fl[t]) ord.push_back(t);
    ws.dist.tile_order_interior = (int)ord.size();
    for (int t = 0; t < nt; t++) if (fl[t]) ord.push_back((int)((unsigned)t | 0x80000000u));
    KB_CUDA(cudaMemcpyAsync(ws.dist.tile_order, ord.data(), sizeof(int) * nt, cudaMemcpyHostToDevice, c.stream));
    c.sync();
  }
  ws.dist.tile_order_for = (const void*)A.rowptr;
  ws.dist.tile_order_n = nt;
}

template <class T> bool cg_fused_eligible(const LinOp<T>& A, const LinOp<T>& M, const SolveOpts& o) {
  const bool m_ok = M.is_identity() || (M.kind == LinOp<T>::DIAG && !o.ldiv);
  if (o.fused && A.kind == LinOp<T>::CSR && M.kind == LinOp<T>::BDIAG && !o.ldiv && o.radius == 0) {
    const char* epers = getenv("KB200_PERSIST");
    const bool single_step = (o.callback != nullptr) || (o.timemax < 1e300) || o.verbose > 0;
    return A.csr->tma_ok && o.persist != 0 && !single_step && !(epers && atoi(epers) == 0);
  }
  return o.fused && A.kind == LinOp<T>::CSR && m_ok && o.radius == 0;
}

template <class T>
void cg_fused_loop(Workspace<T>& ws, const Csr<T>& A, const SolveOpts& o, T gamma0, T eps_tol, int itmax, double start_time,
                   bool& solved, bool& tired, bool& zero_curvature, bool& inconsistent, bool& user_exit, bool& overtimed,
                   int& iter) {
  Ctx& c = ws.ctx;
  const int n = ws.n;
  typedef CgState<T> St;
  const bool dist = ws.dist.world > 1;
  cg_fused_prepare<T>(ws);
  St* dst = (St*)ws.fused_state;
  St* hst = (St*)ws.fused_host;
  auto hslot = [&](int i) -> St* { return (St*)((char*)hst + (size_t)i * kOffGridBar); };

  St init;
  memset(&init, 0, sizeof(init));
  init.gamma = gamma0; init.pNorm2 = gamma0; init.beta = T(0); init.eps_tol = eps_tol;
  init.rNorm = sqrt(gamma0); init.itmax = itmax; init.linesearch = o.linesearch ? 1 : 0;
  *hslot(0) = init;
  KB_CUDA(cudaMemcpyAsync(dst, hslot(0), sizeof(St), cudaMemcpyHostToDevice, c.stream));
  KB_CUDA(cudaMemsetAsync((char*)ws.fused_state + kOffGridBar, 0, sizeof(GridBar), c.stream));

  const bool jac = ws.mdiag_fused != nullptr;
  const bool single_step = (o.callback != nullptr) || (o.timemax < 1e300) || o.verbose > 0;
  const char* exu = getenv("KB200_XUP");
  const bool xup = !single_step && !(exu && atoi(exu) == 0);
  typedef void (*K1Fn)(Csr<T>, const T*, const T*, T*, T*, CgState<T>*, T*, unsigned*, DistComm*, CgPeers<T>, T*);
  typedef void (*K2Fn)(int, T*, T*, const T*, const T*, CgState<T>*, T*, unsigned*, DistComm*, const T*, PushPlan<T>);
  K1Fn k1 = nullptr;
  K2Fn k2 = nullptr;
  if (A.tma_ok) {
    if (dist) k1 = xup ? cg_k1_tma<T, kDist, 3, true> : cg_k1_tma<T, kDist, 3, false>;
    else if (jac) k1 = xup ? cg_k1_tma<T, kJacobi, 3, true> : cg_k1_tma<T, kJacobi, 3, false>;
    else if (A.ctas_per_sm >= 4) k1 = xup ? cg_k1_tma<T, kPlain, 4, true> : cg_k1_tma<T, kPlain, 4, false>;
    else if (A.ctas_per_sm == 3) k1 = xup ? cg_k1_tma<T, kPlain, 3, true> : cg_k1_tma<T, kPlain, 3, false>;
    else k1 = xup ? cg_k1_tma<T, kPlain, 1, true> : cg_k1_tma<T, kPlain, 1, false>;
  } else {
    if (dist) k1 = xup ? cg_k1_rows<T, kDist, true> : cg_k1_rows<T, kDist, false>;
    else if (jac) k1 = xup ? cg_k1_rows<T, kJacobi, true> : cg_k1_rows<T, kJacobi, false>;
    else k1 = xup ? cg_k1_rows<T, kPlain, true> : cg_k1_rows<T, kPlain, false>;
  }
  if (dist) k2 = xup ? cg_k2<T, kDist, false> : cg_k2<T, kDist, true>;
  else if (jac) k2 = xup ? cg_k2<T, kJacobi, false> : cg_k2<T, kJacobi, true>;
  else k2 = xup ? cg_k2<T, kPlain, false> : cg_k2<T, kPlain, true>;
  int k1_grid = A.grid;
  if (A.tma_ok) {
    ensure_dyn_smem((const void*)k1, 220 * 1024);
    int occ = 0;
    KB_CUDA(cudaOccupancyMaxActiveBlocksPerMultiprocessor(&occ, k1, kTileThreads, A.smem_bytes));
    if (occ < 1) throw std::runtime_error("cg_k1_tma does not fit on an SM with the planned shared-memory ring");
    const int resident = std::min(occ, A.ctas_per_sm) * sm_count();
    k1_grid = std::min(resident, std::max(1, A.ntiles));
  }
  const int g2 = stream_grid(n, 4, 8);
  const int g1r = stream_grid(n, 1, 8);
  T* P[2] = {ws.p, ws.p2};
  T* part = (T*)c.partials;
  CgPeers<T> peersP[2];
  memset(peersP, 0, sizeof(peersP));
  const T* md = ws.mdiag_fused;
  peersP[0].mdiag = md; peersP[1].mdiag = md;
  PushPlan<T> push_r;
  memset(&push_r, 0, sizeof(push_r));
  if (dist) {
    for (int b = 0; b < 2; b++) {
      peersP[b].halo = ws.dist.halo;
      const bool wantB = (b == 1) != ws.dist.swapped;
      for (int k = 0; k < ws.dist.world; k++) {
        peersP[b].r[k] = ws.dist.r_peer[k];
        peersP[b].p_old[k] = wantB ? ws.dist.bufB_peer[k] : ws.dist.bufA_peer[k];
      }
      if (ws.dist.npush > 0) {
        const size_t nh = (size_t)ws.dist.halo.nhalo;
        peersP[b].r_halo = ws.dist.halo_buf;
        peersP[b].p_halo_old = ws.dist.halo_buf + (wantB ? 2 : 1) * nh;
        peersP[b].push_p.nranges = ws.dist.npush;
        for (int q = 0; q < ws.dist.npush; q++) {
          const PushRange& rg = ws.dist.push[q];
          peersP[b].push_p.rg[q] = rg;
          peersP[b].push_p.dst[q] = ws.dist.halo_buf_peer[rg.peer] + (wantB ? 1 : 2) * (size_t)ws.dist.nhalo_peer[rg.peer];
          push_r.rg[q] = rg;
          push_r.dst[q] = ws.dist.halo_buf_peer[rg.peer];
        }
        push_r.nranges = ws.dist.npush;
      }
    }
  }

  static const char* ebatch = getenv("KB200_BATCH");
  int batch = o.batch > 0 ? o.batch : (single_step ? 1 : (ebatch && atoi(ebatch) > 0 ? atoi(ebatch) : 32));
  if (batch > kHist / 2) batch = kHist / 2;
  if (single_step) batch = 1;

  const char* epers = getenv("KB200_PERSIST");
  const bool persist = A.tma_ok && xup && !(epers && atoi(epers) == 0) && o.persist != 0;
  const bool bjac = ws.mblocks_fused != nullptr;
  if (bjac && !persist) throw std::runtime_error("block-Jacobi M reached the fused CG loop without the persistent kernel");
  typedef void (*KpFn)(Csr<T>, CgPersistArgs<T>, CgState<T>*, T*, GridBar*, DistComm*);
  KpFn kp = nullptr;
  int pgrid = 0;
  CgPersistArgs<T> pa;
  memset(&pa, 0, sizeof(pa));
  GridBar* gbar = (GridBar*)((char*)ws.fused_state + kOffGridBar);
  if (persist) {
    static const char* edep = getenv("KB200_GATHER_DEPTH");
    const int depth = edep ? atoi(edep) : 0;
    if (A.ctas_per_sm >= 3) {
      if (bjac) kp = cg_persist<T, kBlockJac, 2, 8>;
      else if (depth == 4) kp = dist ? cg_persist<T, kDist, 3, 4> : (jac ? cg_persist<T, kJacobi, 3, 4> : cg_persist<T, kPlain, 3, 4>);
      else kp = dist ? cg_persist<T, kDist, 3, 8> : (jac ? cg_persist<T, kJacobi, 3, 8> : cg_persist<T, kPlain, 3, 8>);
    } else {
      if (bjac) kp = cg_persist<T, kBlockJac, 2, 8>;
      else if (depth == 4) kp = dist ? cg_persist<T, kDist, 2, 4> : (jac ? cg_persist<T, kJacobi, 2, 4> : cg_persist<T, kPlain, 2, 4>);
      else kp = dist ? cg_persist<T, kDist, 2, 8> : (jac ? cg_persist<T, kJacobi, 2, 8> : cg_persist<T, kPlain, 2, 8>);
    }
    ensure_dyn_smem((const void*)kp, 220 * 1024);
    int occ = 0;
    KB_CUDA(cudaOccupancyMaxActiveBlocksPerMultiprocessor(&occ, kp, kTileThreads, A.smem_bytes));
    if (occ < 1) throw std::runtime_error("cg_persist does not fit on an SM with the planned shared-memory ring");
    pgrid = std::min(std::min(occ, A.ctas_per_sm) * sm_count(), std::max(1, A.ntiles));
    pa.r = ws.r; pa.P0 = ws.p; pa.P1 = ws.p2; pa.Ap = ws.Ap; pa.x = ws.x;
    pa.mdiag = md;
    pa.z = ws.z; pa.mblocks = ws.mblocks_fused; pa.mbs = ws.mbs_fused;
    pa.max_iters = batch;
    pa.timed = o.time_kernels ? 1 : 0;
    if (dist) {
      cg_dist_tile_order<T>(ws, A);
      CgPeerTab<T>* htab = (CgPeerTab<T>*)((char*)ws.fused_host + kOffPeerTab);
      memset(htab, 0, sizeof(*htab));
      for (int b = 0; b < 2; b++) {
        const bool wantB = (b == 1) != ws.dist.swapped;
        for (int k = 0; k < ws.dist.world; k++) {
          htab->r[k] = ws.dist.r_peer[k];
          htab->p[b][k] = wantB ? ws.dist.bufB_peer[k] : ws.dist.bufA_peer[k];
        }
      }
      CgPeerTab<T>* dtab = (CgPeerTab<T>*)((char*)ws.fused_state + kOffPeerTab);
      KB_CUDA(cudaMemcpyAsync(dtab, htab, sizeof(*htab), cudaMemcpyHostToDevice, c.stream));
      pa.halo = ws.dist.halo;
      pa.tab = dtab;
      pa.tile_order = ws.dist.tile_order;
      pa.n_interior = ws.dist.tile_order_interior;
    }
  }

  cudaEvent_t* ev = ws.fused_ev;
  int enq = 0;
  constexpr int kTimedFirst = 8, kTimedCount = 32;
  std::vector<cudaEvent_t> tev;
  if (o.time_kernels) {
    tev.resize(3 * kTimedCount);
    for (auto& e : tev) KB_CUDA(cudaEventCreate(&e));
  }
  unsigned long long* hseq = (unsigned long long*)((char*)ws.fused_host + kOffHostSeq);
  unsigned long long expect[2] = {0, 0};
  auto wait_report = [&](int slot) {
    long spins = 0;
    while (__atomic_load_n(&hseq[slot], __ATOMIC_ACQUIRE) != expect[slot]) {
      if ((++spins & 1023) == 0) {
        const cudaError_t q = cudaStreamQuery(c.stream);
        if (q != cudaSuccess && q != cudaErrorNotReady) throw CudaError(std::string("persistent CG kernel failed: ") + cudaGetErrorString(q));
        if (q == cudaSuccess && __atomic_load_n(&hseq[slot], __ATOMIC_ACQUIRE) != expect[slot])
          throw std::runtime_error("persistent CG kernel finished without reporting its state");
      }
#if defined(__x86_64__)
      __builtin_ia32_pause();
#endif
    }
  };
  auto enqueue = [&](int slot) {
    if (persist) {
      DistComm* dcm = dist ? c.dcomm : nullptr;
      Csr<T> Acopy = A;
      T* partp = part;
      pa.hsnap = hslot(slot);
      pa.hseq = hseq + slot;
      pa.seq = expect[slot] = ++ws.fused_seq;
      void* args[] = {(void*)&Acopy, (void*)&pa, (void*)&dst, (void*)&partp, (void*)&gbar, (void*)&dcm};
      KB_CUDA(cudaLaunchCooperativeKernel((const void*)kp, dim3(pgrid), dim3(kTileThreads), args, A.smem_bytes, c.stream));
      c.launches += 1;
      enq += batch;
      return;
    }
    for (int b = 0; !persist && b < batch; b++, enq++) {
      T* p_old = P[enq & 1];
      T* p_new = P[(enq + 1) & 1];
      const CgPeers<T>& pe = peersP[enq & 1];
      const int ti = enq - kTimedFirst;
      const bool timed = o.time_kernels && ti >= 0 && ti < kTimedCount;
      if (timed) KB_CUDA(cudaEventRecord(tev[3 * ti], c.stream));
      DistComm* dcm = dist ? c.dcomm : nullptr;
      if (A.tma_ok) k1<<<k1_grid, kTileThreads, A.smem_bytes, c.stream>>>(A, ws.r, p_old, p_new, ws.Ap, dst, part, c.tickets + 2, dcm, pe, ws.x);
      else k1<<<g1r, kBlock, 0, c.stream>>>(A, ws.r, p_old, p_new, ws.Ap, dst, part, c.tickets + 2, dcm, pe, ws.x);
      if (timed) KB_CUDA(cudaEventRecord(tev[3 * ti + 1], c.stream));
      k2<<<g2, kBlock, 0, c.stream>>>(n, ws.x, ws.r, p_new, ws.Ap, dst, part, c.tickets + 3, dcm, md, push_r);
      if (timed) KB_CUDA(cudaEventRecord(tev[3 * ti + 2], c.stream));
      c.launches += 2;
    }
    KB_CUDA(cudaGetLastError());
    KB_CUDA(cudaMemcpyAsync(hslot(slot), dst, sizeof(St), cudaMemcpyDeviceToHost, c.stream));
    KB_CUDA(cudaEventRecord(ev[slot], c.stream));
  };

  int cur = 0, seen = 0;
  St last;
  enqueue(0);
  for (;;) {
    if (!single_step) enqueue(cur ^ 1);
    if (persist) wait_report(cur);
    else KB_CUDA(cudaEventSynchronize(ev[cur]));
    last = *hslot(cur);
    for (int k = seen + 1; k <= last.iter; k++) {
      if (o.history) ws.stats.residuals.push_back((double)last.hist[k % kHist]);
    }
    seen = last.iter;
    if (last.done) break;
    if (single_step) {
      if (o.verbose > 0 && (last.iter % o.verbose == 0))
        fprintf(stdout, "%5d  %7.1e  %8.1e  %8.1e\n", last.iter, (double)last.rNorm, (double)last.pAp, (double)last.alpha);
      if (o.callback) {
        ws.stats.niter = last.iter;
        user_exit = o.callback(&ws, o.callback_user) != 0;
      }
      overtimed = (now_seconds() - start_time) > o.timemax;
      agree_exit(ws, o, user_exit, overtimed);
      if (user_exit || overtimed) break;
      enqueue(cur);
    } else {
      cur ^= 1;
    }
  }
  c.sync();
  if (o.time_kernels && persist) {
    GridBar hb;
    KB_CUDA(cudaMemcpy(&hb, gbar, sizeof(hb), cudaMemcpyDeviceToHost));
    ws.timed_pairs = (int)hb.timed_iters;
    ws.k1_ms = hb.timed_iters ? 1e-6 * (double)hb.ns_a / hb.timed_iters : 0;
    ws.k2_ms = hb.timed_iters ? 1e-6 * (double)hb.ns_b / hb.timed_iters : 0;
    for (auto& e : tev) cudaEventDestroy(e);
  } else if (o.time_kernels) {
    const int pairs = std::min(kTimedCount, std::max(0, std::min(enq, last.iter) - kTimedFirst));
    double s1 = 0, s2 = 0;
    for (int i = 0; i < pairs; i++) {
      float a = 0, b = 0;
      cudaEventElapsedTime(&a, tev[3 * i], tev[3 * i + 1]);
      cudaEventElapsedTime(&b, tev[3 * i + 1], tev[3 * i + 2]);
      s1 += a; s2 += b;
    }
    ws.timed_pairs = pairs;
    ws.k1_ms = pairs ? s1 / pairs : 0;
    ws.k2_ms = pairs ? s2 / pairs : 0;
    for (auto& e : tev) cudaEventDestroy(e);
  }
  if (last.comm_error) throw std::runtime_error("cross-GPU all-reduce timed out: a peer rank is not participating");
  if (last.not_spd) throw std::runtime_error("The linear operator `A` or the preconditioner `M` is not symmetric positive definite.");

  iter = last.iter;
  solved = last.solved != 0;
  tired = last.tired != 0;
  zero_curvature = last.zero_curvature != 0;
  inconsistent = last.inconsistent != 0;
  const bool k1_exit = zero_curvature || last.npc;
  T* pcur = k1_exit ? P[(iter + 1) & 1] : P[iter & 1];
  if (pcur != ws.p) { T* tmp = ws.p; ws.p = ws.p2; ws.p2 = tmp; ws.dist.swapped = !ws.dist.swapped; }
  if (xup && !k1_exit && iter > 0) k_axpy<T>(c, n, last.alpha, ws.p, ws.x);
  if (last.npc) {
    if (iter == 0) k_copy<T>(c, n, ws.x, ws.p);
    k_copy<T>(c, n, ws.npc_dir, ws.p);
    ws.stats.npcCount = 1;
    ws.stats.indefinite = true;
  }
}

#define INST(T)                                                                                              \
  template bool cg_fused_eligible<T>(const LinOp<T>&, const LinOp<T>&, const SolveOpts&);                    \
  template void cg_fused_prepare<T>(Workspace<T>&);                                                          \
  template void cg_dist_push_r<T>(Workspace<T>&);                                                            \
  template void cg_fused_loop<T>(Workspace<T>&, const Csr<T>&, const SolveOpts&, T, T, int, double, bool&, bool&, \
                                 bool&, bool&, bool&, bool&, int&);
INST(double)
INST(float)
#undef INST

}
```

### krylov.jl_b200/csrc/kb_internal.h

```cpp
#pragma once
#include <cuda_runtime.h>
#include <cstddef>
#include <cstdint>
#include <string>
#include <vector>

#include "common.cuh"
#include "dist.cuh"

namespace kb {

struct Ctx {
  int device = 0;
  cudaStream_t stream = nullptr;
  bool own_stream = false;
  void* partials = nullptr;
  unsigned* tickets = nullptr;
  void* dscal = nullptr;
  void* hscal = nullptr;
  long long launches = 0;
  DistComm* dcomm = nullptr;
  DistExchange* dex = nullptr;

  void init(int dev);
  void destroy();
  void sync() { KB_CUDA(cudaStreamSynchronize(stream)); }
};

template <class T> T* dev_alloc(size_t n);
void dev_free(void* p);

template <class T> T    k_dot(Ctx& c, int n, const T* x, const T* y);
template <class T> T    k_nrm2(Ctx& c, int n, const T* x);
template <class T> T    k_cg_prologue(Ctx& c, int n, const T* b, T* x, T* r, T* p);
template <class T> void k_dot2(Ctx& c, int n, const T* a, const T* b, const T* u, const T* v, T* r1, T* r2);
template <class T> void k_dot_dev(Ctx& c, int n, const T* x, const T* y, int slot);
template <class T> void k_axpy(Ctx& c, int n, T s, const T* x, T* y);
template <class T> void k_axpby(Ctx& c, int n, T s, const T* x, T t, T* y);
template <class T> void k_scal(Ctx& c, int n, T s, T* x);
template <class T> void k_copy(Ctx& c, int n, T* y, const T* x);
template <class T> void k_scalcopy(Ctx& c, int n, T* y, T s, const T* x);
template <class T> void k_divcopy(Ctx& c, int n, T* y, const T* x, T s);
template <class T> void k_fill(Ctx& c, int n, T* x, T v);
template <class T> void k_diagmul(Ctx& c, int n, T* y, const T* d, const T* x, bool ldiv);
template <class T> void k_blockdiag_mul(Ctx& c, int n, int bs, const T* blocks, const T* x, T* y);
template <class T> void k_blockdiag_invert(Ctx& c, int n, int bs, const T* blocks, T* inv, int* singular);
double k_dist_sum(Ctx& c, double v);
void dist_agree_on_exit(Ctx& c, bool& user_exit, bool& overtimed);
void dist_check_alive(Ctx& c);
inline void dist_nan_guard(Ctx& c, double v) { if (c.dcomm && v != v) dist_check_alive(c); }

constexpr int kTileRows = 256;

template <class T>
struct Csr {
  int n = 0;
  long long nnz = 0;
  int* rowptr = nullptr;
  int* colind = nullptr;
  T* val = nullptr;
  int ntiles = 0;
  int tile_cap = 0;
  int max_row = 0;
  int max_col = -1;
  bool tma_ok = false;
  int stages = 0;
  size_t smem_bytes = 0;
  int grid = 0;
  int ctas_per_sm = 0;
};

template <class T> void csr_upload(Ctx& c, Csr<T>& A, int n, long long nnz, const void* rowptr, const void* colind,
                                   const T* val, int index_base, int index_bytes, bool on_device);
template <class T> void csr_free(Csr<T>& A);
template <class T> void csr_plan(Ctx& c, Csr<T>& A);
template <class T> void k_spmv(Ctx& c, const Csr<T>& A, const T* x, T* y, int variant = 0);
template <class T> void k_halo_exchange(Ctx& c, const T* x);

typedef void (*MatvecFn)(const void* x, void* y, void* userdata);

template <class T>
struct LinOp {
  enum Kind { NONE, CSR, DIAG, BDIAG, HOST_CB, DEV_CB } kind = NONE;
  const Csr<T>* csr = nullptr;
  const T* diag = nullptr;
  const T* blocks = nullptr;
  const T* blocks_inv = nullptr;
  int bs = 0;
  MatvecFn fn = nullptr;
  void* userdata = nullptr;
  T* hx = nullptr;
  T* hy = nullptr;
  int n = 0;
  bool is_identity() const { return kind == NONE; }
};
template <class T> void op_apply(Ctx& c, const LinOp<T>& op, const T* x, T* y, bool ldiv = false);

struct SolveOpts {
  double atol = -1, rtol = -1;
  int itmax = 0;
  double timemax = 1.0 / 0.0;
  int verbose = 0;
  bool history = false;
  double radius = 0;
  bool linesearch = false;
  double lambda = 0;
  double etol = -1, conlim = -1;
  bool restart = false;
  bool reorthogonalization = false;
  bool check_curvature = false;
  double cr_gamma = -1;
  bool ldiv = false;
  int (*callback)(void* ws, void* user) = nullptr;
  void* callback_user = nullptr;
  int fused = 1;
  int batch = 0;
  int time_kernels = 0;
  int persist = 1;
};

struct Stats {
  int niter = 0;
  bool solved = false, inconsistent = false, indefinite = false;
  int npcCount = 0;
  std::vector<double> residuals, Aresiduals, Acond;
  double allocation_timer = 0, timer = 0;
  double Anorm = NAN;
  std::string status = "unknown";
  void reset() { residuals.clear(); Aresiduals.clear(); Acond.clear(); indefinite = false; npcCount = 0; }
};

enum SolverKind { S_CG = 0, S_CR = 1, S_MINRES = 3, S_DIOM = 5, S_DQGMRES = 6, S_FOM = 7, S_GMRES = 8, S_FGMRES = 9, S_BICGSTAB = 10,
                  S_CGS = 11, S_CG_LANCZOS = 100 };

template <class T>
struct Workspace {
  SolverKind kind;
  int m = 0, n = 0;
  Ctx ctx;
  Stats stats;
  bool warm_start = false;
  T *x = nullptr, *dx = nullptr;
  T *r = nullptr, *p = nullptr, *Ap = nullptr, *z = nullptr, *npc_dir = nullptr;
  T *p2 = nullptr;
  T *v = nullptr, *s = nullptr, *qd = nullptr, *t = nullptr, *yz = nullptr;
  T *r1 = nullptr, *r2 = nullptr, *w1 = nullptr, *w2 = nullptr, *y = nullptr, *vv = nullptr;
  T *w = nullptr, *q = nullptr, *pp = nullptr;
  T *u = nullptr, *ts = nullptr, *vw = nullptr;
  T *Mv = nullptr, *Mv_prev = nullptr, *Mv_next = nullptr;
  std::vector<T*> V;
  std::vector<T*> Z;
  std::vector<T> c, sgiv, zg, R;
  std::vector<T> err_vec;
  int memory = 20, window = 5;
  int inner_iter = 0;
  const T* mdiag_fused = nullptr;
  const T* mblocks_fused = nullptr;
  int mbs_fused = 0;
  double k1_ms = 0, k2_ms = 0;
  int timed_pairs = 0;
  void* fused_state = nullptr;
  void* fused_host = nullptr;
  cudaEvent_t fused_ev[2] = {nullptr, nullptr};
  unsigned long long fused_seq = 0;
  T* bbuf = nullptr;
  T* cbuf = nullptr;
  struct Dist {
    int rank = 0, world = 1;
    HaloMap halo{0, 0, nullptr, nullptr};
    void* mailbox = nullptr;
    T* bufA_peer[kMaxRanks] = {};
    T* bufB_peer[kMaxRanks] = {};
    T* r_peer[kMaxRanks] = {};
    std::vector<void*> opened;
    bool swapped = false;
    T* halo_buf = nullptr;
    T* halo_buf_peer[kMaxRanks] = {};
    int nhalo_peer[kMaxRanks] = {};
    void* dummy[3] = {nullptr, nullptr, nullptr};
    T* xhalo = nullptr;
    T* xhalo_peer[kMaxRanks] = {};
    int nsend = 0;
    int* send_row = nullptr; int* send_peer = nullptr; int* send_slot = nullptr;
    long long nglobal = 0;
    int npush = 0;
    int* tile_order = nullptr;
    const void* tile_order_for = nullptr;
    int tile_order_n = 0;
    int tile_order_interior = 0;
    PushRange push[kMaxPushRanges];
  } dist;
};

template <class T> Workspace<T>* ws_create(SolverKind kind, int m, int n, int memory, int window, int device);
template <class T> void ws_destroy(Workspace<T>* ws);
template <class T> void ws_warm_start(Workspace<T>* ws, const T* x0_dev);

template <class T> void cg_solve(Workspace<T>& ws, const LinOp<T>& A, const T* b, const LinOp<T>& M, const SolveOpts& o);
template <class T> void gmres_solve(Workspace<T>& ws, const LinOp<T>& A, const T* b, const LinOp<T>& M, const LinOp<T>& N, const SolveOpts& o);
template <class T> void bicgstab_solve(Workspace<T>& ws, const LinOp<T>& A, const T* b, const T* c, const LinOp<T>& M, const LinOp<T>& N, const SolveOpts& o);
template <class T> void minres_solve(Workspace<T>& ws, const LinOp<T>& A, const T* b, const LinOp<T>& M, const SolveOpts& o);
template <class T> void cgs_solve(Workspace<T>& ws, const LinOp<T>& A, const T* b, const T* c, const LinOp<T>& M, const LinOp<T>& N, const SolveOpts& o);
template <class T> void cg_lanczos_solve(Workspace<T>& ws, const LinOp<T>& A, const T* b, const LinOp<T>& M, const SolveOpts& o);
template <class T> void fom_solve(Workspace<T>& ws, const LinOp<T>& A, const T* b, const LinOp<T>& M, const LinOp<T>& N, const SolveOpts& o);
template <class T> void fgmres_solve(Workspace<T>& ws, const LinOp<T>& A, const T* b, const LinOp<T>& M, const LinOp<T>& N, const SolveOpts& o);
template <class T> void dqgmres_solve(Workspace<T>& ws, const LinOp<T>& A, const T* b, const LinOp<T>& M, const LinOp<T>& N, const SolveOpts& o);
template <class T> void diom_solve(Workspace<T>& ws, const LinOp<T>& A, const T* b, const LinOp<T>& M, const LinOp<T>& N, const SolveOpts& o);
template <class T> void cr_solve(Workspace<T>& ws, const LinOp<T>& A, const T* b, const LinOp<T>& M, const SolveOpts& o);

template <class T> bool cg_fused_eligible(const LinOp<T>& A, const LinOp<T>& M, const SolveOpts& o);
template <class T> void cg_dist_push_r(Workspace<T>& ws);
template <class T> void cg_fused_prepare(Workspace<T>& ws);
constexpr size_t kFusedBlockBytes = 4096;
template <class T> void cg_fused_loop(Workspace<T>& ws, const Csr<T>& A, const SolveOpts& o, T gamma0, T eps_tol, int itmax,
                                      double start_time, bool& solved, bool& tired, bool& zero_curvature,
                                      bool& inconsistent, bool& user_exit, bool& overtimed, int& iter);

template <class T> void bicgstab_fused_iteration(Workspace<T>& ws, const Csr<T>& A, const T* cvec, bool first, T rho_in, T* alpha,
                                                 T* omega, T* next_rho, T* rNorm);
template <class T> void minres_fused_lanczos(Workspace<T>& ws, const Csr<T>& A, int iter, T lambda, T beta, T oldbeta, T cs, T sn,
                                             T deltabar, T eps_rot, T* w, T* alpha, T* beta2);
template <class T> T minres_fused_update(Workspace<T>& ws, T* w, T gamma, T phi);
template <class T> void gmres_fused_arnoldi(Workspace<T>& ws, const Csr<T>& A, int k, T* h_out, T* Hbis, const T* xin = nullptr);
template <class T> void fused_multi_axpy(Workspace<T>& ws, T* xr, int k, const T* y, T* const* vecs);
template <class T> void fused_orth_chain(Workspace<T>& ws, const Csr<T>& A, const T* xin, T* q, const T* const* vecs, int cnt, T* h_out, T* Hbis);
template <class T> void trunc_fused_direction(Workspace<T>& ws, T* pp, int cnt, T* const* pvecs, const T* coefs, const T* z, T h0, T step);
template <class T> T cgs_fused_sigma(Workspace<T>& ws, const Csr<T>& A, const T* cvec);
template <class T> void cgs_fused_update(Workspace<T>& ws, const Csr<T>& A, const T* cvec, T alpha, T* rho_next, T* rr);
template <class T> void cgs_fused_directions(Workspace<T>& ws, T beta);
template <class T> T lanczos_fused_delta(Workspace<T>& ws, const Csr<T>& A);
template <class T> T lanczos_fused_recur(Workspace<T>& ws, T delta, T beta, bool later);
template <class T> void lanczos_fused_update(Workspace<T>& ws, T beta, T gamma, T sigma, T omega);
template <class T> void cr_fused_step(Workspace<T>& ws, const Csr<T>& A, T alpha, T* xx, T* rr, T* ArAr, T* rAr);
template <class T> T cr_fused_directions(Workspace<T>& ws, T beta);
template <class T> void gmres_fused_update_x(Workspace<T>& ws, T* xr, int k, const T* y);
int gmres_fused_max();

double now_seconds();

}
```

### krylov.jl_b200/csrc/spmv.cu

```cuda
#include "kb_internal.h"
#include "spmv_tiles.cuh"

#include <vector>

namespace kb {

template <class I>
__global__ void index_convert_kernel(long long cnt, const I* __restrict__ in, int* __restrict__ out, int base, int* bad) {
  long long i = (long long)blockIdx.x * blockDim.x + threadIdx.x;
  const long long stride = (long long)gridDim.x * blockDim.x;
  for (; i < cnt; i += stride) {
    long long v = (long long)in[i] - base;
    if (v < 0 || v > 2147483647LL) atomicExch(bad, 1);
    out[i] = (int)v;
  }
}

__global__ void fill_int_kernel(int cnt, int* out, int v) {
  int i = blockIdx.x * blockDim.x + threadIdx.x;
  if (i < cnt) out[i] = v;
}

template <class T>
void csr_upload(Ctx& c, Csr<T>& A, int n, long long nnz, const void* rowptr, const void* colind, const T* val,
                int index_base, int index_bytes, bool on_device) {
  if (n < 0 || nnz < 0 || nnz > 2147483647LL - 64) throw std::runtime_error("CSR operator: n/nnz out of int32 range");
  if (index_bytes != 4 && index_bytes != 8) throw std::runtime_error("CSR operator: index_bytes must be 4 or 8");
  if (index_base != 0 && index_base != 1) throw std::runtime_error("CSR operator: index_base must be 0 or 1");
  csr_free(A);
  A.n = n; A.nnz = nnz;
  const size_t rp_len = (size_t)n + 1, rp_pad = kTileRows + 16;
  A.rowptr = dev_alloc<int>(rp_len + rp_pad);
  A.colind = dev_alloc<int>((size_t)nnz + 16);
  A.val = dev_alloc<T>((size_t)nnz + 16);
  const cudaMemcpyKind kind = on_device ? cudaMemcpyDeviceToDevice : cudaMemcpyHostToDevice;
  KB_CUDA(cudaMemcpyAsync(A.val, val, sizeof(T) * (size_t)nnz, kind, c.stream));
  KB_CUDA(cudaMemsetAsync(A.val + nnz, 0, sizeof(T) * 16, c.stream));
  KB_CUDA(cudaMemsetAsync(A.colind + nnz, 0, sizeof(int) * 16, c.stream));
  int* bad = nullptr;
  KB_CUDA(cudaMalloc((void**)&bad, sizeof(int)));
  KB_CUDA(cudaMemsetAsync(bad, 0, sizeof(int), c.stream));
  void* tmp_rp = nullptr; void* tmp_ci = nullptr;
  if (index_bytes == 4 && index_base == 0) {
    KB_CUDA(cudaMemcpyAsync(A.rowptr, rowptr, sizeof(int) * rp_len, kind, c.stream));
    KB_CUDA(cudaMemcpyAsync(A.colind, colind, sizeof(int) * (size_t)nnz, kind, c.stream));
  } else {
    const void* drp = rowptr; const void* dci = colind;
    if (!on_device) {
      KB_CUDA(cudaMalloc(&tmp_rp, (size_t)index_bytes * rp_len));
      KB_CUDA(cudaMalloc(&tmp_ci, (size_t)index_bytes * (size_t)(nnz ? nnz : 1)));
      KB_CUDA(cudaMemcpyAsync(tmp_rp, rowptr, (size_t)index_bytes * rp_len, cudaMemcpyHostToDevice, c.stream));
      KB_CUDA(cudaMemcpyAsync(tmp_ci, colind, (size_t)index_bytes * (size_t)nnz, cudaMemcpyHostToDevice, c.stream));
      drp = tmp_rp; dci = tmp_ci;
    }
    const int g = sm_count() * 8;
    if (index_bytes == 8) {
      index_convert_kernel<long long><<<g, 256, 0, c.stream>>>((long long)rp_len, (const long long*)drp, A.rowptr, index_base, bad);
      index_convert_kernel<long long><<<g, 256, 0, c.stream>>>(nnz, (const long long*)dci, A.colind, index_base, bad);
    } else {
      index_convert_kernel<int><<<g, 256, 0, c.stream>>>((long long)rp_len, (const int*)drp, A.rowptr, index_base, bad);
      index_convert_kernel<int><<<g, 256, 0, c.stream>>>(nnz, (const int*)dci, A.colind, index_base, bad);
    }
    KB_CUDA(cudaGetLastError());
  }
  fill_int_kernel<<<((int)rp_pad + 255) / 256, 256, 0, c.stream>>>((int)rp_pad, A.rowptr + rp_len, (int)nnz);
  KB_CUDA(cudaGetLastError());
  int hbad = 0;
  KB_CUDA(cudaMemcpyAsync(&hbad, bad, sizeof(int), cudaMemcpyDeviceToHost, c.stream));
  c.sync();
  cudaFree(bad);
  if (tmp_rp) cudaFree(tmp_rp);
  if (tmp_ci) cudaFree(tmp_ci);
  if (hbad) { csr_free(A); throw std::runtime_error("CSR operator: index outside int32 range after rebasing"); }
  try { csr_plan(c, A); } catch (...) { csr_free(A); throw; }
}

template <class T> void csr_free(Csr<T>& A) {
  dev_free(A.rowptr); dev_free(A.colind); dev_free(A.val);
  A = Csr<T>();
}

__global__ void plan_kernel(int n, int ntiles, const int* __restrict__ rowptr,
                            int* out ,
                            const int* __restrict__ colind, long long nnz) {
  int t = blockIdx.x * blockDim.x + threadIdx.x;
  const int stride = gridDim.x * blockDim.x;
  int cap = 0, mr = 0, uns = 0, bad = 0, mc = -1, neg = 0;
  for (int i = t; i < n; i += stride) {
    const int kb = rowptr[i], ke = rowptr[i + 1];
    if (kb > ke || kb < 0 || (long long)ke > nnz) { bad = 1; continue; }
    mr = max(mr, ke - kb);
    for (int k = kb; k < ke; k++) { const int cj = colind[k]; mc = max(mc, cj); neg |= cj < 0; }
    for (int k = kb + 1; k < ke; k++) uns |= (colind[k] <= colind[k - 1]) && colind[k] < n && colind[k - 1] < n;
  }
  if (bad) atomicExch(&out[3], 1);
  __syncthreads();
  for (int i = t; i < ntiles; i += stride) {
    const int r0 = i * kTileRows, r1 = min(r0 + kTileRows, n);
    cap = max(cap, rowptr[r1] - rowptr[r0]);
  }
  atomicMax(&out[0], cap);
  atomicMax(&out[1], mr);
  atomicMax(&out[4], mc);
  if (uns) atomicExch(&out[2], 1);
  if (neg) atomicExch(&out[5], 1);
}

template <class T> void csr_plan(Ctx& c, Csr<T>& A) {
  A.ntiles = (A.n + kTileRows - 1) / kTileRows;
  int* dout = nullptr;
  KB_CUDA(cudaMalloc((void**)&dout, 6 * sizeof(int)));
  KB_CUDA(cudaMemsetAsync(dout, 0, 6 * sizeof(int), c.stream));
  int h[6] = {0, 0, 0, 0, -1, 0};
  int ends[2] = {0, (int)A.nnz};
  if (A.n > 0) {
    KB_CUDA(cudaMemcpyAsync(dout + 4, &h[4], sizeof(int), cudaMemcpyHostToDevice, c.stream));
    plan_kernel<<<sm_count() * 4, 256, 0, c.stream>>>(A.n, A.ntiles, A.rowptr, dout, A.colind, A.nnz);
    KB_CUDA(cudaGetLastError());
    KB_CUDA(cudaMemcpyAsync(&ends[0], A.rowptr, sizeof(int), cudaMemcpyDeviceToHost, c.stream));
    KB_CUDA(cudaMemcpyAsync(&ends[1], A.rowptr + A.n, sizeof(int), cudaMemcpyDeviceToHost, c.stream));
  }
  KB_CUDA(cudaMemcpyAsync(h, dout, sizeof(h), cudaMemcpyDeviceToHost, c.stream));
  c.sync();
  cudaFree(dout);
  if (ends[0] != 0 || (long long)ends[1] != A.nnz || h[3])
    throw std::runtime_error("CSR operator: row pointers must start at 0 (after rebasing), be non-decreasing and end at nnz");
  if (h[5]) throw std::runtime_error("CSR operator: negative column index (after rebasing)");
  A.max_col = h[4];
  if (h[2]) fprintf(stderr, "[krylov_b200] warning: CSR column indices are not strictly ascending within rows; "
                            "results remain correct but are no longer bit-comparable to SparseArrays' order\n");
  A.tile_cap = h[0];
  A.max_row = h[1];
  TileLayout<T> L{A.tile_cap};
  const size_t two_cta = 110 * 1024, one_cta = 220 * 1024;
  A.tma_ok = false;
  int per_sm = 2;
  const char* es = getenv("KB200_STAGES");
  const char* ec = getenv("KB200_CTAS_PER_SM");
  if (es && ec) {
    const int s = atoi(es), cps = atoi(ec);
    if (s >= 1 && s <= 8 && cps >= 1 && cps <= 8 && L.total_bytes(s) * cps <= 226 * 1024) { A.tma_ok = true; A.stages = s; per_sm = cps; }
  }
  if (!A.tma_ok && L.total_bytes(2) * 3 <= 226 * 1024) { A.tma_ok = true; A.stages = 2; per_sm = 3; }
  for (int s = 4; s >= 2 && !A.tma_ok; s--)
    if (L.total_bytes(s) <= two_cta) { A.tma_ok = true; A.stages = s; per_sm = 2; }
  for (int s = 4; s >= 2 && !A.tma_ok; s--)
    if (L.total_bytes(s) <= one_cta) { A.tma_ok = true; A.stages = s; per_sm = 1; }
  if (A.tma_ok) {
    A.smem_bytes = L.total_bytes(A.stages);
    int g = sm_count() * per_sm;
    A.grid = g < A.ntiles ? g : (A.ntiles > 0 ? A.ntiles : 1);
    A.ctas_per_sm = per_sm;
  } else {
    A.stages = 0; A.smem_bytes = 0; A.grid = 0;
  }
}

template <class T, bool DOT, class G>
__global__ void __launch_bounds__(kBlock) spmv_rows_kernel(Csr<T> A, G xg, T* __restrict__ y, T* part,
                                                           unsigned* ticket, T* out) {
  __shared__ T sm[32];
  T dacc = T(0);
  const int stride = gridDim.x * blockDim.x;
  for (int row = blockIdx.x * blockDim.x + threadIdx.x; row < A.n; row += stride) {
    const int kb = A.rowptr[row], ke = A.rowptr[row + 1];
    T acc = T(0);
    for (int k = kb; k < ke; k++) acc = add_rn(acc, mul_rn(A.val[k], xg(A.colind[k])));
    y[row] = acc;
    if (DOT) dacc += __ldg(&xg.x[row]) * acc;
  }
  if (DOT) {
    T mine[1] = {block_sum(dacc, sm)}, tot[1];
    if (grid_sum_last<T, 1>(mine, part, ticket, sm, tot) && threadIdx.x == 0) out[0] = tot[0];
  }
}

template <class T, bool DOT, class G>
__global__ void __launch_bounds__(kTileThreads, 3) spmv_tma_kernel(Csr<T> A, G xg, T* __restrict__ y, T* part,
                                                                unsigned* ticket, T* out) {
  extern __shared__ __align__(128) unsigned char smem[];
  __shared__ T sm[32];
  T dacc = T(0);
  spmv_tiles_run<T>(
      A, smem, xg, [&](int row) { return DOT ? __ldg(&xg.x[row]) : T(0); },
      [&](int row, T acc, T xr) {
        y[row] = acc;
        if (DOT) dacc += xr * acc;
      });
  if (DOT) {
    T mine[1] = {block_sum(dacc, sm)}, tot[1];
    if (grid_sum_last<T, 1>(mine, part, ticket, sm, tot) && threadIdx.x == 0) out[0] = tot[0];
  }
}

template <class T, bool DOT, class G>
static void spmv_launch_g(Ctx& c, const Csr<T>& A, G xg, T* y, int slot, int variant) {
  T* out = reinterpret_cast<T*>(reinterpret_cast<double*>(c.dscal) + slot);
  const bool staged = variant == 2 || (variant == 0 && A.tma_ok);
  if (staged) {
    if (!A.tma_ok) throw std::runtime_error("TMA-staged SpMV requested but the tile plan does not fit shared memory");
    ensure_dyn_smem((const void*)spmv_tma_kernel<T, DOT, G>, 220 * 1024);
    int occ = 0;
    KB_CUDA(cudaOccupancyMaxActiveBlocksPerMultiprocessor(&occ, spmv_tma_kernel<T, DOT, G>, kTileThreads, A.smem_bytes));
    if (occ < 1) throw std::runtime_error("spmv_tma_kernel does not fit on an SM with the planned shared-memory ring");
    const int grid = std::min(std::min(occ, A.ctas_per_sm) * sm_count(), std::max(1, A.ntiles));
    spmv_tma_kernel<T, DOT, G><<<grid, kTileThreads, A.smem_bytes, c.stream>>>(A, xg, y, (T*)c.partials, c.tickets + 1, out);
  } else {
    const int grid = stream_grid(A.n, 1, 8);
    spmv_rows_kernel<T, DOT, G><<<grid, kBlock, 0, c.stream>>>(A, xg, y, (T*)c.partials, c.tickets + 1, out);
  }
  KB_CUDA(cudaGetLastError());
  c.launches++;
}

template <class T, bool DOT>
static void spmv_launch(Ctx& c, const Csr<T>& A, const T* x, T* y, int slot, int variant) {
  if (A.n <= 0) return;
  if (c.dex) spmv_launch_g<T, DOT, XGather<T>>(c, A, xgather_of<T>(c, x), y, slot, variant);
  else spmv_launch_g<T, DOT, XPlain<T>>(c, A, XPlain<T>{x}, y, slot, variant);
}

template <class T> void k_spmv(Ctx& c, const Csr<T>& A, const T* x, T* y, int variant) { spmv_launch<T, false>(c, A, x, y, 1, variant); }

template <class T> struct ExchangeDst { T* p[kMaxRanks]; };

template <class T>
__global__ void __launch_bounds__(kBlock) halo_exchange_kernel(const T* __restrict__ x, int nsend, const int* __restrict__ row,
                                                               const int* __restrict__ peer, const int* __restrict__ slot,
                                                               ExchangeDst<T> dst, unsigned* ticket, DistComm* dc) {
  __shared__ bool is_last;
  const int stride = gridDim.x * blockDim.x;
  bool sent = false;
  for (int e = blockIdx.x * blockDim.x + threadIdx.x; e < nsend; e += stride) {
    dst.p[peer[e]][slot[e]] = x[row[e]];
    sent = true;
  }
  if (sent) __threadfence_system();
  __syncthreads();
  if (threadIdx.x == 0) {
    __threadfence();
    const unsigned t = atomicAdd(ticket, 1u);
    is_last = (t == gridDim.x - 1);
    if (is_last) *ticket = 0u;
  }
  __syncthreads();
  if (is_last && threadIdx.x == 0) dist_allreduce_sum(dc, 0.0);
}

template <class T> void k_halo_exchange(Ctx& c, const T* x) {
  if (!c.dex) return;
  DistExchange& d = *c.dex;
  ExchangeDst<T> dst;
  const size_t par = (size_t)(d.count & 1);
  for (int k = 0; k < kMaxRanks; k++)
    dst.p[k] = d.xhalo_peer[k] ? reinterpret_cast<T*>(d.xhalo_peer[k]) + par * (size_t)d.nhalo_peer[k] : nullptr;
  const int grid = d.nsend > 0 ? std::min(sm_count(), (d.nsend + kBlock - 1) / kBlock) : 1;
  halo_exchange_kernel<T><<<grid, kBlock, 0, c.stream>>>(x, d.nsend, d.send_row, d.send_peer, d.send_slot, dst, c.tickets + 6, c.dcomm);
  KB_CUDA(cudaGetLastError());
  c.launches++;
  d.count++;
}

template <class T> void op_apply(Ctx& c, const LinOp<T>& op, const T* x, T* y, bool ldiv) {
  switch (op.kind) {
    case LinOp<T>::CSR:
      k_halo_exchange<T>(c, x);
      k_spmv<T>(c, *op.csr, x, y, 0);
      break;
    case LinOp<T>::DIAG: k_diagmul<T>(c, op.n, y, op.diag, x, ldiv); break;
    case LinOp<T>::BDIAG: k_blockdiag_mul<T>(c, op.n, op.bs, ldiv ? op.blocks_inv : op.blocks, x, y); break;
    case LinOp<T>::DEV_CB:
      c.sync();
      op.fn(x, y, op.userdata);
      KB_CUDA(cudaDeviceSynchronize());
      break;
    case LinOp<T>::HOST_CB:
      KB_CUDA(cudaMemcpyAsync(op.hx, x, sizeof(T) * (size_t)op.n, cudaMemcpyDeviceToHost, c.stream));
      c.sync();
      op.fn(op.hx, op.hy, op.userdata);
      KB_CUDA(cudaMemcpyAsync(y, op.hy, sizeof(T) * (size_t)op.n, cudaMemcpyHostToDevice, c.stream));
      break;
    case LinOp<T>::NONE: k_copy<T>(c, op.n, y, x); break;
  }
}

#define INST(T)                                                                                                  \
  template void csr_upload<T>(Ctx&, Csr<T>&, int, long long, const void*, const void*, const T*, int, int, bool); \
  template void csr_free<T>(Csr<T>&);                                                                            \
  template void csr_plan<T>(Ctx&, Csr<T>&);                                                                      \
  template void k_spmv<T>(Ctx&, const Csr<T>&, const T*, T*, int);                                               \
  template void k_halo_exchange<T>(Ctx&, const T*);                                                              \
  template void op_apply<T>(Ctx&, const LinOp<T>&, const T*, T*, bool);
INST(double)
INST(float)
#undef INST

}
```

### krylov.jl_b200/csrc/spmv_tiles.cuh

```cuda
#pragma once
#include "common.cuh"
#include "kb_internal.h"

namespace kb {

constexpr int kConsumerWarps = kTileRows / 32;
constexpr int kTileThreads = kTileRows + 32;
constexpr int kGatherDepth = 8;
#ifndef KB_CLAMP_GATHER
#define KB_CLAMP_GATHER 1
#endif

__device__ __forceinline__ uint32_t smem_u32(const void* p) { return (uint32_t)__cvta_generic_to_shared(p); }
__device__ __forceinline__ void mbar_init(uint64_t* bar, unsigned count) {
  asm volatile("mbarrier.init.shared::cta.b64 [%0], %1;" ::"r"(smem_u32(bar)), "r"(count));
}
__device__ __forceinline__ void mbar_expect_tx(uint64_t* bar, unsigned bytes) {
  asm volatile("mbarrier.arrive.expect_tx.shared::cta.b64 _, [%0], %1;" ::"r"(smem_u32(bar)), "r"(bytes) : "memory");
}
__device__ __forceinline__ void mbar_arrive(uint64_t* bar) {
  asm volatile("mbarrier.arrive.shared::cta.b64 _, [%0];" ::"r"(smem_u32(bar)) : "memory");
}
__device__ __forceinline__ void mbar_wait(uint64_t* bar, unsigned parity) {
  unsigned ok;
  do {
    asm volatile(
        "{\n\t.reg .pred p;\n\t"
        "mbarrier.try_wait.parity.shared::cta.b64 p, [%1], %2;\n\t"
        "selp.u32 %0, 1, 0, p;\n\t}"
        : "=r"(ok)
        : "r"(smem_u32(bar)), "r"(parity)
        : "memory");
  } while (!ok);
}
__device__ __forceinline__ void tma_load_1d(void* dst, const void* src, unsigned bytes, uint64_t* bar, uint64_t policy) {
  asm volatile(
      "cp.async.bulk.shared::cluster.global.mbarrier::complete_tx::bytes.L2::cache_hint [%0], [%1], %2, [%3], %4;" ::"r"(
          smem_u32(dst)),
      "l"(src), "r"(bytes), "r"(smem_u32(bar)), "l"(policy)
      : "memory");
}
template <class T>
struct XPlain {
  const T* __restrict__ x;
  __device__ __forceinline__ T operator()(int j) const { return __ldg(&x[j]); }
};

template <class T>
struct XGather {
  const T* x;
  const T* xh_minus_nloc;
  int nloc;
  __device__ __forceinline__ T operator()(int j) const {
    const T* base = j < nloc ? x : xh_minus_nloc;
    return __ldg(&base[j]);
  }
};

template <class T>
inline XGather<T> xgather_of(const Ctx& c, const T* x) {
  if (!c.dex) return XGather<T>{x, x, 2147483647};
  const DistExchange& d = *c.dex;
  const T* section = reinterpret_cast<const T*>(d.xhalo) + (size_t)((d.count + 1) & 1) * (size_t)d.nhalo;
  return XGather<T>{x, section - d.nloc, d.nloc};
}

__device__ __forceinline__ uint64_t l2_evict_first_policy() {
  uint64_t pol;
  asm volatile("createpolicy.fractional.L2::evict_first.b64 %0, 1.0;" : "=l"(pol));
  return pol;
}

template <class T>
struct TileLayout {
  int cap;
  __host__ __device__ static constexpr size_t align_up(size_t v) { return (v + 127) & ~size_t(127); }
  __host__ __device__ size_t rp_bytes() const { return align_up((kTileRows + 4) * sizeof(int)); }
  __host__ __device__ size_t val_bytes() const { return align_up((size_t)(cap + 16 / sizeof(T)) * sizeof(T)); }
  __host__ __device__ size_t col_bytes() const { return align_up((size_t)(cap + 8) * sizeof(int)); }
  __host__ __device__ size_t stage_bytes() const { return rp_bytes() + val_bytes() + col_bytes(); }
  __host__ __device__ size_t total_bytes(int stages) const { return 128 + (size_t)stages * stage_bytes(); }
};

struct NoRowBegin {
  __device__ __forceinline__ int operator()(int) const { return 0; }
};

template <class T>
__device__ __forceinline__ void tile_producer(const Csr<T>& A, const TileLayout<T>& L, int S, unsigned char* ring, uint64_t* full,
                                              uint64_t* empty) {
  constexpr int VA = 16 / sizeof(T);
  const uint64_t pol = l2_evict_first_policy();
  int it = 0;
  int t = blockIdx.x;
  int k0 = 0, k1 = 0;
  if (t < A.ntiles) { k0 = __ldg(&A.rowptr[t * kTileRows]); k1 = __ldg(&A.rowptr[min(t * kTileRows + kTileRows, A.n)]); }
  for (; t < A.ntiles; t += gridDim.x, it++) {
    const int tn = t + gridDim.x;
    int nk0 = 0, nk1 = 0;
    if (tn < A.ntiles) { nk0 = __ldg(&A.rowptr[tn * kTileRows]); nk1 = __ldg(&A.rowptr[min(tn * kTileRows + kTileRows, A.n)]); }
    const int s = it % S;
    mbar_wait(&empty[s], ((it / S) & 1) ^ 1);
    unsigned char* st = ring + (size_t)s * L.stage_bytes();
    const int r0 = t * kTileRows;
    const int k0v = k0 & ~(VA - 1), k1v = (k1 + VA - 1) & ~(VA - 1);
    const int k0c = k0 & ~3, k1c = (k1 + 3) & ~3;
    const unsigned rp_b = (kTileRows + 4) * sizeof(int);
    const unsigned v_b = (unsigned)(k1v - k0v) * sizeof(T);
    const unsigned c_b = (unsigned)(k1c - k0c) * sizeof(int);
    mbar_expect_tx(&full[s], rp_b + v_b + c_b);
    tma_load_1d(st, A.rowptr + r0, rp_b, &full[s], pol);
    if (v_b) tma_load_1d(st + L.rp_bytes(), A.val + k0v, v_b, &full[s], pol);
    if (c_b) tma_load_1d(st + L.rp_bytes() + L.val_bytes(), A.colind + k0c, c_b, &full[s], pol);
    k0 = nk0; k1 = nk1;
  }
}

template <class T, class Gather, class RowBegin, class RowDone>
__device__ __forceinline__ void spmv_tiles_run(const Csr<T>& A, unsigned char* smem, Gather gather, RowBegin row_begin,
                                               RowDone row_done) {
  const TileLayout<T> L{A.tile_cap};
  const int S = A.stages;
  uint64_t* full = reinterpret_cast<uint64_t*>(smem);
  uint64_t* empty = full + S;
  unsigned char* ring = smem + 128;
  const int tid = threadIdx.x, warp = tid >> 5, lane = tid & 31;
  constexpr int VA = 16 / sizeof(T);

  if (tid == 0) {
    for (int s = 0; s < S; s++) { mbar_init(&full[s], 1); mbar_init(&empty[s], kConsumerWarps); }
    asm volatile("fence.mbarrier_init.release.cluster;" ::: "memory");
  }
  __syncthreads();

  if (warp == kConsumerWarps) {
    if (lane == 0) tile_producer<T>(A, L, S, ring, full, empty);
  } else {
    int it = 0;
    for (int t = blockIdx.x; t < A.ntiles; t += gridDim.x, it++) {
      const int row = t * kTileRows + tid;
      auto pre = row_begin(row < A.n ? row : 0);
      const int s = it % S;
      mbar_wait(&full[s], (it / S) & 1);
      const unsigned char* st = ring + (size_t)s * L.stage_bytes();
      const int* rp = reinterpret_cast<const int*>(st);
      const T* vs = reinterpret_cast<const T*>(st + L.rp_bytes());
      const int* cs = reinterpret_cast<const int*>(st + L.rp_bytes() + L.val_bytes());
      if (row < A.n) {
        const int k0 = rp[0];
        const T* vrow = vs - (k0 & ~(VA - 1));
        const int* crow = cs - (k0 & ~3);
        const int kb = rp[tid], ke = rp[tid + 1];
        T acc = T(0);
        for (int k = kb; k < ke; k += kGatherDepth) {
          T xv[kGatherDepth], av[kGatherDepth];
#if KB_CLAMP_GATHER
#pragma unroll
          for (int u = 0; u < kGatherDepth; u++) {
            const int kk = min(k + u, ke - 1);
            av[u] = vrow[kk];
            xv[u] = gather(crow[kk]);
          }
          asm volatile("" ::: "memory");
#pragma unroll
          for (int u = 0; u < kGatherDepth; u++) {
            const T nx = add_rn(acc, mul_rn(av[u], xv[u]));
            acc = (k + u < ke) ? nx : acc;
          }
#else
#pragma unroll
          for (int u = 0; u < kGatherDepth; u++) {
            if (k + u < ke) { av[u] = vrow[k + u]; xv[u] = gather(crow[k + u]); }
          }
#pragma unroll
          for (int u = 0; u < kGatherDepth; u++) {
            if (k + u < ke) acc = add_rn(acc, mul_rn(av[u], xv[u]));
          }
#endif
        }
        row_done(row, acc, pre);
      }
      __syncwarp();
      if (lane == 0) mbar_arrive(&empty[s]);
    }
  }
}


template <class T>
struct TilePipe {
  TileLayout<T> L;
  int S;
  uint64_t* full;
  uint64_t* empty;
  unsigned char* ring;
  __device__ __forceinline__ void init(const Csr<T>& A, unsigned char* smem) {
    L = TileLayout<T>{A.tile_cap};
    S = A.stages;
    full = reinterpret_cast<uint64_t*>(smem);
    empty = full + S;
    ring = smem + 128;
    if (threadIdx.x == 0) {
      for (int s = 0; s < S; s++) { mbar_init(&full[s], 1); mbar_init(&empty[s], kConsumerWarps); }
      asm volatile("fence.mbarrier_init.release.cluster;" ::: "memory");
    }
    __syncthreads();
  }
};

template <class T, class TileAt>
__device__ __forceinline__ void tile_issue_until(const Csr<T>& A, const TilePipe<T>& P, unsigned& pos, unsigned target, int cnt,
                                                 TileAt tile_at, uint64_t pol) {
  constexpr int VA = 16 / sizeof(T);
  if (pos >= target) return;
  int t = tile_at((int)(pos % (unsigned)cnt)) & 0x7fffffff;
  int k0 = __ldg(&A.rowptr[t * kTileRows]), k1 = __ldg(&A.rowptr[min(t * kTileRows + kTileRows, A.n)]);
  for (; pos < target; pos++) {
    int tn = 0, nk0 = 0, nk1 = 0;
    if (pos + 1 < target) {
      tn = tile_at((int)((pos + 1) % (unsigned)cnt)) & 0x7fffffff;
      nk0 = __ldg(&A.rowptr[tn * kTileRows]); nk1 = __ldg(&A.rowptr[min(tn * kTileRows + kTileRows, A.n)]);
    }
    const int s = (int)(pos % (unsigned)P.S);
    mbar_wait(&P.empty[s], ((pos / (unsigned)P.S) & 1) ^ 1);
    unsigned char* st = P.ring + (size_t)s * P.L.stage_bytes();
    const int k0v = k0 & ~(VA - 1), k1v = (k1 + VA - 1) & ~(VA - 1);
    const int k0c = k0 & ~3, k1c = (k1 + 3) & ~3;
    const unsigned rp_b = (kTileRows + 4) * sizeof(int);
    const unsigned v_b = (unsigned)(k1v - k0v) * sizeof(T);
    const unsigned c_b = (unsigned)(k1c - k0c) * sizeof(int);
    mbar_expect_tx(&P.full[s], rp_b + v_b + c_b);
    tma_load_1d(st, A.rowptr + t * kTileRows, rp_b, &P.full[s], pol);
    if (v_b) tma_load_1d(st + P.L.rp_bytes(), A.val + k0v, v_b, &P.full[s], pol);
    if (c_b) tma_load_1d(st + P.L.rp_bytes() + P.L.val_bytes(), A.colind + k0c, c_b, &P.full[s], pol);
    t = tn; k0 = nk0; k1 = nk1;
  }
}

template <class T>
__device__ __forceinline__ void tile_drain(const TilePipe<T>& P, unsigned consumed, unsigned pos) {
  for (unsigned q = consumed; q < pos; q++) mbar_wait(&P.full[q % (unsigned)P.S], (q / (unsigned)P.S) & 1);
}

template <class T, int DEPTH, class TileAt, class Gather, class RowBegin, class RowDone>
__device__ __forceinline__ void tile_consume_pass(const Csr<T>& A, const TilePipe<T>& P, unsigned& cpos, int j0, int j1, TileAt tile_at,
                                                  Gather gather, RowBegin row_begin, RowDone row_done) {
  constexpr int VA = 16 / sizeof(T);
  const int tid = threadIdx.x, lane = tid & 31;
  for (int j = j0; j < j1; j++, cpos++) {
    const int t = tile_at(j) & 0x7fffffff;
    const int row = t * kTileRows + tid;
    auto pre = row_begin(row < A.n ? row : 0);
    const int s = (int)(cpos % (unsigned)P.S);
    mbar_wait(&P.full[s], (cpos / (unsigned)P.S) & 1);
    const unsigned char* st = P.ring + (size_t)s * P.L.stage_bytes();
    const int* rp = reinterpret_cast<const int*>(st);
    const T* vs = reinterpret_cast<const T*>(st + P.L.rp_bytes());
    const int* cs = reinterpret_cast<const int*>(st + P.L.rp_bytes() + P.L.val_bytes());
    if (row < A.n) {
      const int k0 = rp[0];
      const T* vrow = vs - (k0 & ~(VA - 1));
      const int* crow = cs - (k0 & ~3);
      const int kb = rp[tid], ke = rp[tid + 1];
      T acc = T(0);
      for (int k = kb; k < ke; k += DEPTH) {
        T xv[DEPTH], av[DEPTH];
#pragma unroll
        for (int u = 0; u < DEPTH; u++) xv[u] = gather(crow[min(k + u, ke - 1)]);
        asm volatile("" ::: "memory");
#pragma unroll
        for (int u = 0; u < DEPTH; u++) av[u] = vrow[min(k + u, ke - 1)];
#pragma unroll
        for (int u = 0; u < DEPTH; u++) {
          const T nx = add_rn(acc, mul_rn(av[u], xv[u]));
          acc = (k + u < ke) ? nx : acc;
        }
      }
      row_done(row, acc, pre);
    }
    __syncwarp();
    if (lane == 0) mbar_arrive(&P.empty[s]);
  }
}

}
```

### krylov.jl_b200/krylov_b200/_lib.py

```python
from __future__ import annotations

import ctypes as C
import os
import subprocess

_PKG = os.path.dirname(os.path.abspath(__file__))
ROOT = os.path.dirname(_PKG)
SO_PATH = os.environ.get("KB200_LIB") or os.path.join(ROOT, "lib", "libkrylov_b200.so")

KRYLOV_FLOAT32, KRYLOV_FLOAT64 = 0, 1
KRYLOV_CPU, KRYLOV_CUDA = 0, 1
KRYLOV_CG, KRYLOV_MINRES, KRYLOV_GMRES, KRYLOV_BICGSTAB = 0, 3, 8, 10
KRYLOV_FOM, KRYLOV_FGMRES, KRYLOV_CGS, KRYLOV_B200_CG_LANCZOS = 7, 9, 11, 100
KRYLOV_CR, KRYLOV_DIOM, KRYLOV_DQGMRES = 1, 5, 6
SOLVER_IDS = {"cg": KRYLOV_CG, "minres": KRYLOV_MINRES, "gmres": KRYLOV_GMRES, "bicgstab": KRYLOV_BICGSTAB,
              "fom": KRYLOV_FOM, "fgmres": KRYLOV_FGMRES, "cgs": KRYLOV_CGS, "cg_lanczos": KRYLOV_B200_CG_LANCZOS,
              "cr": KRYLOV_CR, "diom": KRYLOV_DIOM, "dqgmres": KRYLOV_DQGMRES}

MATVEC = C.CFUNCTYPE(None, C.c_void_p, C.c_void_p, C.c_void_p)
BLOCK_MATVEC = C.CFUNCTYPE(None, C.c_void_p, C.c_void_p, C.c_int, C.c_void_p)
CALLBACK = C.CFUNCTYPE(C.c_int, C.c_void_p, C.c_void_p)


class KrylovWorkspaceOptions(C.Structure):
    _fields_ = [("memory", C.c_int), ("window", C.c_int)]


class KrylovOptions(C.Structure):
    _fields_ = [("atol", C.c_double), ("rtol", C.c_double), ("itmax", C.c_int), ("verbose", C.c_int),
                ("lambda_", C.c_double), ("tau", C.c_double), ("nu", C.c_double), ("timemax", C.c_double),
                ("radius", C.c_double), ("restart", C.c_int), ("reorthogonalization", C.c_int),
                ("linesearch", C.c_int)]


class KrylovB200Options(C.Structure):
    _fields_ = [("history", C.c_int), ("ldiv", C.c_int), ("etol", C.c_double), ("conlim", C.c_double),
                ("fused", C.c_int), ("batch", C.c_int), ("callback", CALLBACK), ("callback_user", C.c_void_p),
                ("time_kernels", C.c_int), ("check_curvature", C.c_int), ("cr_gamma", C.c_double)]


class KrylovB200Stats(C.Structure):
    _fields_ = [("niter", C.c_int), ("solved", C.c_int), ("inconsistent", C.c_int), ("indefinite", C.c_int),
                ("npcCount", C.c_int), ("nresiduals", C.c_int), ("nAresiduals", C.c_int), ("nAcond", C.c_int),
                ("allocation_timer", C.c_double), ("timer", C.c_double), ("status", C.c_char * 96),
                ("Anorm", C.c_double)]


_P, _I, _D, _LL = C.c_void_p, C.c_int, C.c_double, C.c_longlong
SIGNATURES = {
    "krylov_workspace_create": (_I, [_I, _I, _I, _I, _I, C.POINTER(KrylovWorkspaceOptions), C.POINTER(_P)]),
    "krylov_default_workspace_options": (KrylovWorkspaceOptions, []),
    "krylov_default_options": (KrylovOptions, []),
    "krylov_get_version": (None, [C.POINTER(_I)] * 3),
    "krylov_solve": (_I, [_P, MATVEC, MATVEC, MATVEC, MATVEC, _P, _P, _P, C.POINTER(KrylovOptions)]),
    "krylov_get_x": (_I, [_P, _P, _I]),
    "krylov_get_y": (_I, [_P, _P, _I]),
    "krylov_is_solved": (_I, [_P]),
    "krylov_niter": (_I, [_P]),
    "krylov_elapsed_time": (_D, [_P]),
    "krylov_warm_start": (_I, [_P, _P, _I]),
    "krylov_warm_start2": (_I, [_P, _P, _P, _I, _I]),
    "krylov_workspace_free": (_I, [_P]),
    "krylov_block_workspace_create": (_I, [_I, _I, _I, _I, _I, _I, C.POINTER(KrylovWorkspaceOptions), C.POINTER(_P)]),
    "krylov_block_solve": (_I, [_P, BLOCK_MATVEC, BLOCK_MATVEC, BLOCK_MATVEC, _P, _P, C.POINTER(KrylovOptions)]),
    "krylov_block_get_X": (_I, [_P, _P, _I, _I]),
    "krylov_block_is_solved": (_I, [_P]),
    "krylov_block_niter": (_I, [_P]),
    "krylov_block_elapsed_time": (_D, [_P]),
    "krylov_block_warm_start": (_I, [_P, _P, _I, _I]),
    "krylov_block_workspace_free": (_I, [_P]),
    "krylov_b200_block_qr_fallbacks": (_LL, [_P]),
    "krylov_b200_device_count": (_I, []),
    "krylov_b200_set_device": (_I, [_I]),
    "krylov_b200_last_error": (C.c_char_p, []),
    "krylov_b200_set_operator_csr": (_I, [_P, _I, _LL, _P, _P, _P, _I, _I, _I]),
    "krylov_b200_share_operator": (_I, [_P, _P]),
    "krylov_b200_attach_csr": (_I, [_P, _P]),
    "krylov_b200_set_preconditioner_diag": (_I, [_P, _I, _P, _I]),
    "krylov_b200_set_preconditioner_blockdiag": (C.c_int, [_P, C.c_int, C.c_int, _P, C.c_int]),
    "krylov_b200_default_options": (KrylovB200Options, []),
    "krylov_b200_set_options": (_I, [_P, C.POINTER(KrylovB200Options)]),
    "krylov_b200_get_stats": (_I, [_P, C.POINTER(KrylovB200Stats)]),
    "krylov_b200_get_history": (_I, [_P, _I, C.POINTER(_D), _I]),
    "krylov_b200_get_vector": (_I, [_P, C.c_char_p, C.POINTER(_P)]),
    "krylov_b200_get_kernel_times": (_I, [_P, C.POINTER(_D)]),
    "krylov_b200_launch_count": (_LL, [_P]),
    "krylov_b200_stream": (_P, [_P]),
    "krylov_b200_wait_stream": (C.c_int, [_P, _P]),
    "krylov_b200_dist_handle_bytes": (_I, []),
    "krylov_b200_dist_init": (_I, [_P, _I, _I, _I, _P, _P]),
    "krylov_b200_dist_set_push": (_I, [_P, _I, _P, _P]),
    "krylov_b200_dist_set_sendlist": (_I, [_P, _I, _P, _P, _P, _P, _LL]),
    "krylov_b200_dist_export": (_I, [_P, _P]),
    "krylov_b200_dist_import": (_I, [_P, _P]),
    "kb200_ctx_create": (_P, [_I]),
    "kb200_ctx_destroy": (None, [_P]),
    "kb200_sync": (_I, [_P]),
    "kb200_alloc": (_P, [_LL]),
    "kb200_free": (_I, [_P]),
    "kb200_h2d": (_I, [_P, _P, _LL]),
    "kb200_d2h": (_I, [_P, _P, _LL]),
    "kb200_dot": (_I, [_P, _I, _I, _P, _P, C.POINTER(_D)]),
    "kb200_nrm2": (_I, [_P, _I, _I, _P, C.POINTER(_D)]),
    "kb200_axpy": (_I, [_P, _I, _I, _D, _P, _P]),
    "kb200_axpby": (_I, [_P, _I, _I, _D, _P, _D, _P]),
    "kb200_scal": (_I, [_P, _I, _I, _D, _P]),
    "kb200_copy": (_I, [_P, _I, _I, _P, _P]),
    "kb200_scalcopy": (_I, [_P, _I, _I, _P, _D, _P]),
    "kb200_divcopy": (_I, [_P, _I, _I, _P, _P, _D]),
    "kb200_fill": (_I, [_P, _I, _I, _P, _D]),
    "kb200_csr_create": (_P, [_P, _I, _I, _LL, _P, _P, _P, _I, _I, _I]),
    "kb200_csr_destroy": (None, [_P]),
    "kb200_csr_read_mtx": (_P, [_P, C.c_char_p, _I]),
    "kb200_csr_transpose": (_P, [_P, _P]),
    "kb200_csr_info": (_I, [_P, C.POINTER(_I), C.POINTER(_LL)]),
    "kb200_csr_download": (_I, [_P, _P, _P, _P, _P]),
    "kb200_mtx_read": (_I, [C.c_char_p, C.POINTER(_I), C.POINTER(_LL), _P, _P, _P]),
    "kb200_host_householder": (_I, [_I, _I, _P, _P, _P, _I]),
    "kb200_host_cholqr_factors": (_I, [_I, _P, _P, _P]),
    "kb200_host_householder_signs": (_I, [_I, _P, _P]),
    "kb200_spmv_csr": (_I, [_P, _P, _P, _P, _I]),
    "kb200_csr_plan": (_I, [_P, C.POINTER(_LL)]),
}

_LIB = None


def build(verbose: bool = False) -> str:
    cmd = ["make", "-C", ROOT, "-j8"] + ([] if verbose else ["-s"])
    subprocess.check_call(cmd)
    return SO_PATH


def lib() -> C.CDLL:
    global _LIB
    if _LIB is None:
        if not os.path.exists(SO_PATH):
            raise RuntimeError(f"{SO_PATH} is missing: run `python -c 'import __graft_entry__ as g; g.build()'` "
                               "(there is no CPU fallback)")
        L = C.CDLL(SO_PATH)
        for name, (res, args) in SIGNATURES.items():
            try:
                fn = getattr(L, name)
            except AttributeError:
                if os.environ.get("KB200_LIB"):
                    continue
                raise
            fn.restype = res
            fn.argtypes = args
        _LIB = L
    return _LIB


def last_error() -> str:
    return lib().krylov_b200_last_error().decode("utf-8", "replace")
```

Baseline: 3656.

## Dictionary-encode CSR (column offset, value) pairs into 8-bit codes for persistent CG

At setup, GPU kernels gather the distinct (column minus row, value) pairs of the matrix. When there are at most 256 of them, each nonzero is stored as a one-byte code into a dictionary that the persistent CG kernel keeps in shared memory. The TMA tile pipeline then streams the codes instead of the 8-byte values and 4-byte column indices, cutting SpMV traffic per nonzero. The cost is extra setup kernels, more template instantiations, a smaller shared-memory ring, and dictionary decode work inside the consume loop. Matrices with more distinct pairs, and the dist, block-Jacobi and depth-4 paths, keep the old path.

```diff
diff --git a/include/krylov_b200.h b/include/krylov_b200.h
--- a/include/krylov_b200.h
+++ b/include/krylov_b200.h
@@ -89,6 +89,7 @@
                                  const void *values, int index_base, int index_bytes, int location);
 int krylov_b200_share_operator(void *ws, void *src);
 int krylov_b200_attach_csr(void *ws, void *csr);
+int krylov_b200_operator_encoding(void *ws);
 int krylov_b200_set_preconditioner_diag(void *ws, int which, const void *d, int location);
 int krylov_b200_set_preconditioner_blockdiag(void *ws, int which, int bs, const void *blocks, int location);
 
diff --git a/krylov.jl_b200/csrc/capi.cu b/krylov.jl_b200/csrc/capi.cu
--- a/krylov.jl_b200/csrc/capi.cu
+++ b/krylov.jl_b200/csrc/capi.cu
@@ -551,6 +551,13 @@
   return 0;
 }
 
+int krylov_b200_operator_encoding(void* ws) {
+  Handle* h = lookup_any(ws);
+  if (!h) return fail("krylov_b200_operator_encoding", "unknown workspace handle");
+  if (!h->csr) return fail("krylov_b200_operator_encoding", "no CSR operator attached");
+  return h->dtype == KRYLOV_FLOAT64 ? h->csr->d.ndict : h->csr->f.ndict;
+}
+
 int krylov_b200_set_preconditioner_diag(void* ws, int which, const void* d, int location) {
   try {
     Handle* h = lookup_any(ws);
diff --git a/krylov.jl_b200/csrc/cg_fused.cu b/krylov.jl_b200/csrc/cg_fused.cu
--- a/krylov.jl_b200/csrc/cg_fused.cu
+++ b/krylov.jl_b200/csrc/cg_fused.cu
@@ -355,7 +355,7 @@
   }
 }
 
-template <class T, int MODE, int MINB, int DEPTH>
+template <class T, int MODE, int MINB, int DEPTH, bool DICT>
 __global__ void __launch_bounds__(kTileThreads, MINB) cg_persist(Csr<T> A, CgPersistArgs<T> a, CgState<T>* st, T* part,
                                                                 GridBar* gb, DistComm* dc) {
   extern __shared__ __align__(128) unsigned char smem[];
@@ -365,7 +365,7 @@
   volatile CgState<T>* vst = st;
   if (vst->done) { cg_report_to_host<T>(a, st); return; }
   if (threadIdx.x == 0) cg_load_scal<T>(st, &sc);
-  TilePipe<T> P;
+  TilePipe<T, DICT> P;
   P.init(A, smem);
   const int G = gridDim.x, tid = threadIdx.x, warp = tid >> 5, lane = tid & 31;
   const int cnt = (A.ntiles - (int)blockIdx.x + G - 1) / G;
@@ -392,7 +392,7 @@
     if (warp == kConsumerWarps) {
       if (lane == 0) {
         const unsigned target = (unsigned)(k + 1) * (unsigned)cnt + (k + 1 < a.max_iters ? pre : 0u);
-        tile_issue_until<T>(A, P, ppos, target, cnt, tile_at, pol);
+        tile_issue_until<T, DICT>(A, P, ppos, target, cnt, tile_at, pol);
       }
     } else {
       const T* r = MODE == kBlockJac ? a.z : a.r;
@@ -422,14 +422,14 @@
         __threadfence();
         __syncwarp();
         if (lane == 0) atomicAdd(&gb->halo_ready, 1u);
-        tile_consume_pass<T, DEPTH>(A, P, cpos, 0, cnt_int, tile_at, gather, row_begin, row_done);
+        tile_consume_pass<T, DEPTH, DICT>(A, P, cpos, 0, cnt_int, tile_at, gather, row_begin, row_done);
         if (cnt_int < cnt) {
           if (lane == 0) { while (ld_acquire_gpu_u32(&gb->halo_ready) < (unsigned)(G * kConsumerWarps)) { } }
           __syncwarp();
-          tile_consume_pass<T, DEPTH>(A, P, cpos, cnt_int, cnt, tile_at, gather, row_begin, row_done);
+          tile_consume_pass<T, DEPTH, DICT>(A, P, cpos, cnt_int, cnt, tile_at, gather, row_begin, row_done);
         }
       } else {
-        tile_consume_pass<T, DEPTH>(A, P, cpos, 0, cnt, tile_at, gather, row_begin, row_done);
+        tile_consume_pass<T, DEPTH, DICT>(A, P, cpos, 0, cnt, tile_at, gather, row_begin, row_done);
       }
     }
     passes = k + 1;
@@ -491,7 +491,7 @@
       if (!ok || sc.done) break;
     }
   }
-  if (warp == kConsumerWarps && lane == 0) tile_drain<T>(P, (unsigned)passes * (unsigned)cnt, ppos);
+  if (warp == kConsumerWarps && lane == 0) tile_drain<T, DICT>(P, (unsigned)passes * (unsigned)cnt, ppos);
   cg_report_to_host<T>(a, st);
 }
 
@@ -674,24 +674,29 @@
   typedef void (*KpFn)(Csr<T>, CgPersistArgs<T>, CgState<T>*, T*, GridBar*, DistComm*);
   KpFn kp = nullptr;
   int pgrid = 0;
+  size_t psmem = 0;
   CgPersistArgs<T> pa;
   memset(&pa, 0, sizeof(pa));
   GridBar* gbar = (GridBar*)((char*)ws.fused_state + kOffGridBar);
   if (persist) {
     static const char* edep = getenv("KB200_GATHER_DEPTH");
     const int depth = edep ? atoi(edep) : 0;
-    if (A.ctas_per_sm >= 3) {
-      if (bjac) kp = cg_persist<T, kBlockJac, 2, 8>;
-      else if (depth == 4) kp = dist ? cg_persist<T, kDist, 3, 4> : (jac ? cg_persist<T, kJacobi, 3, 4> : cg_persist<T, kPlain, 3, 4>);
-      else kp = dist ? cg_persist<T, kDist, 3, 8> : (jac ? cg_persist<T, kJacobi, 3, 8> : cg_persist<T, kPlain, 3, 8>);
+    const bool dict = A.ndict > 0 && !dist && !bjac && depth != 4;
+    if (dict) {
+      kp = jac ? cg_persist<T, kJacobi, 3, 8, true> : cg_persist<T, kPlain, 3, 8, true>;
+    } else if (A.ctas_per_sm >= 3) {
+      if (bjac) kp = cg_persist<T, kBlockJac, 2, 8, false>;
+      else if (depth == 4) kp = dist ? cg_persist<T, kDist, 3, 4, false> : (jac ? cg_persist<T, kJacobi, 3, 4, false> : cg_persist<T, kPlain, 3, 4, false>);
+      else kp = dist ? cg_persist<T, kDist, 3, 8, false> : (jac ? cg_persist<T, kJacobi, 3, 8, false> : cg_persist<T, kPlain, 3, 8, false>);
     } else {
-      if (bjac) kp = cg_persist<T, kBlockJac, 2, 8>;
-      else if (depth == 4) kp = dist ? cg_persist<T, kDist, 2, 4> : (jac ? cg_persist<T, kJacobi, 2, 4> : cg_persist<T, kPlain, 2, 4>);
-      else kp = dist ? cg_persist<T, kDist, 2, 8> : (jac ? cg_persist<T, kJacobi, 2, 8> : cg_persist<T, kPlain, 2, 8>);
-    }
+      if (bjac) kp = cg_persist<T, kBlockJac, 2, 8, false>;
+      else if (depth == 4) kp = dist ? cg_persist<T, kDist, 2, 4, false> : (jac ? cg_persist<T, kJacobi, 2, 4, false> : cg_persist<T, kPlain, 2, 4, false>);
+      else kp = dist ? cg_persist<T, kDist, 2, 8, false> : (jac ? cg_persist<T, kJacobi, 2, 8, false> : cg_persist<T, kPlain, 2, 8, false>);
+    }
+    psmem = dict ? A.dict_smem_bytes : A.smem_bytes;
     ensure_dyn_smem((const void*)kp, 220 * 1024);
     int occ = 0;
-    KB_CUDA(cudaOccupancyMaxActiveBlocksPerMultiprocessor(&occ, kp, kTileThreads, A.smem_bytes));
+    KB_CUDA(cudaOccupancyMaxActiveBlocksPerMultiprocessor(&occ, kp, kTileThreads, psmem));
     if (occ < 1) throw std::runtime_error("cg_persist does not fit on an SM with the planned shared-memory ring");
     pgrid = std::min(std::min(occ, A.ctas_per_sm) * sm_count(), std::max(1, A.ntiles));
     pa.r = ws.r; pa.P0 = ws.p; pa.P1 = ws.p2; pa.Ap = ws.Ap; pa.x = ws.x;
@@ -752,7 +757,7 @@
       pa.hseq = hseq + slot;
       pa.seq = expect[slot] = ++ws.fused_seq;
       void* args[] = {(void*)&Acopy, (void*)&pa, (void*)&dst, (void*)&partp, (void*)&gbar, (void*)&dcm};
-      KB_CUDA(cudaLaunchCooperativeKernel((const void*)kp, dim3(pgrid), dim3(kTileThreads), args, A.smem_bytes, c.stream));
+      KB_CUDA(cudaLaunchCooperativeKernel((const void*)kp, dim3(pgrid), dim3(kTileThreads), args, psmem, c.stream));
       c.launches += 1;
       enq += batch;
       return;
diff --git a/krylov.jl_b200/csrc/kb_internal.h b/krylov.jl_b200/csrc/kb_internal.h
--- a/krylov.jl_b200/csrc/kb_internal.h
+++ b/krylov.jl_b200/csrc/kb_internal.h
@@ -68,7 +68,13 @@
   size_t smem_bytes = 0;
   int grid = 0;
   int ctas_per_sm = 0;
-};
+  uint8_t* code = nullptr;
+  void* dict = nullptr;
+  int ndict = 0;
+  int dict_stages = 0;
+  size_t dict_smem_bytes = 0;
+};
+constexpr int kDictMax = 256;
 
 template <class T> void csr_upload(Ctx& c, Csr<T>& A, int n, long long nnz, const void* rowptr, const void* colind,
                                    const T* val, int index_base, int index_bytes, bool on_device);
diff --git a/krylov.jl_b200/csrc/spmv.cu b/krylov.jl_b200/csrc/spmv.cu
--- a/krylov.jl_b200/csrc/spmv.cu
+++ b/krylov.jl_b200/csrc/spmv.cu
@@ -1,6 +1,8 @@
 #include "kb_internal.h"
 #include "spmv_tiles.cuh"
 
+#include <algorithm>
+#include <type_traits>
 #include <vector>
 
 namespace kb {
@@ -76,7 +78,7 @@
 }
 
 template <class T> void csr_free(Csr<T>& A) {
-  dev_free(A.rowptr); dev_free(A.colind); dev_free(A.val);
+  dev_free(A.rowptr); dev_free(A.colind); dev_free(A.val); dev_free(A.code); dev_free(A.dict);
   A = Csr<T>();
 }
 
@@ -104,6 +106,171 @@
   atomicMax(&out[4], mc);
   if (uns) atomicExch(&out[2], 1);
   if (neg) atomicExch(&out[5], 1);
+}
+
+template <class T> using DictBits = typename std::conditional<sizeof(T) == 8, unsigned long long, unsigned>::type;
+__device__ __forceinline__ unsigned long long dict_bits(double v) { return (unsigned long long)__double_as_longlong(v); }
+__device__ __forceinline__ unsigned dict_bits(float v) { return __float_as_uint(v); }
+
+template <class B>
+__device__ __forceinline__ int dict_warp_insert(int* toff, B* tbits, int cnt, bool have, int off, B bits) {
+  const int lane = threadIdx.x & 31;
+  bool need = have;
+  for (int e = 0; need && e < cnt; e++) need = !(toff[e] == off && tbits[e] == bits);
+  const unsigned needm = __ballot_sync(0xffffffffu, need);
+  if (!needm) return cnt;
+  const unsigned same = __match_any_sync(0xffffffffu, off) & __match_any_sync(0xffffffffu, bits) & needm;
+  const bool lead = need && (__ffs(same) - 1 == lane);
+  const unsigned leads = __ballot_sync(0xffffffffu, lead);
+  const int slot = cnt + __popc(leads & ((1u << lane) - 1u));
+  if (lead && slot < kDictMax) { toff[slot] = off; tbits[slot] = bits; }
+  __syncwarp();
+  return cnt + __popc(leads);
+}
+
+constexpr int kDictWarps = 8;
+
+template <class T>
+__global__ void __launch_bounds__(kDictWarps * 32) dict_collect_kernel(int n, const int* __restrict__ rowptr, const int* __restrict__ colind,
+                                                                     const T* __restrict__ val, int* cta_off, DictBits<T>* cta_bits,
+                                                                     int* cta_cnt, int* overflow) {
+  typedef DictBits<T> B;
+  __shared__ int soff[kDictWarps][kDictMax];
+  __shared__ B sbits[kDictWarps][kDictMax];
+  __shared__ int scnt[kDictWarps];
+  const int warp = threadIdx.x >> 5, lane = threadIdx.x & 31;
+  const int stride = gridDim.x * kDictWarps * 32;
+  int cnt = 0;
+  for (int base = (blockIdx.x * kDictWarps + warp) * 32; base < n && cnt <= kDictMax; base += stride) {
+    if (__any_sync(0xffffffffu, *(volatile int*)overflow != 0)) break;
+    const int row = base + lane;
+    int kb = 0, ke = 0;
+    if (row < n) { kb = rowptr[row]; ke = rowptr[row + 1]; }
+    const int len = __reduce_max_sync(0xffffffffu, (unsigned)(ke - kb));
+    for (int j = 0; j < len && cnt <= kDictMax; j++) {
+      const bool have = kb + j < ke;
+      const int off = have ? colind[kb + j] - row : 0;
+      const B bits = have ? dict_bits(val[kb + j]) : B(0);
+      cnt = dict_warp_insert<B>(soff[warp], sbits[warp], cnt, have, off, bits);
+    }
+  }
+  if (lane == 0) { scnt[warp] = cnt; if (cnt > kDictMax) atomicExch(overflow, 1); }
+  __syncthreads();
+  if (warp != 0) return;
+  for (int w = 1; w < kDictWarps && cnt <= kDictMax; w++) {
+    const int m = min(scnt[w], kDictMax);
+    for (int e0 = 0; e0 < m && cnt <= kDictMax; e0 += 32) {
+      const int e = e0 + lane;
+      cnt = dict_warp_insert<B>(soff[0], sbits[0], cnt, e < m, e < m ? soff[w][e] : 0, e < m ? sbits[w][e] : B(0));
+    }
+  }
+  if (cnt > kDictMax) { if (lane == 0) atomicExch(overflow, 1); }
+  for (int e = lane; e < min(cnt, kDictMax); e += 32) {
+    cta_off[blockIdx.x * kDictMax + e] = soff[0][e];
+    cta_bits[blockIdx.x * kDictMax + e] = sbits[0][e];
+  }
+  if (lane == 0) cta_cnt[blockIdx.x] = cnt;
+}
+
+template <class B>
+__global__ void dict_merge_kernel(int ncta, const int* cta_off, const B* cta_bits, const int* cta_cnt, const int* overflow,
+                                  int* out_off, B* out_bits, int* out_cnt) {
+  __shared__ int soff[kDictMax];
+  __shared__ B sbits[kDictMax];
+  const int lane = threadIdx.x;
+  int cnt = *(volatile const int*)overflow ? kDictMax + 1 : 0;
+  for (int b = 0; b < ncta && cnt <= kDictMax; b++) {
+    const int m = cta_cnt[b];
+    for (int e0 = 0; e0 < m && cnt <= kDictMax; e0 += 32) {
+      const int e = e0 + lane;
+      const bool have = e < m;
+      cnt = dict_warp_insert<B>(soff, sbits, cnt, have, have ? cta_off[b * kDictMax + e] : 0, have ? cta_bits[b * kDictMax + e] : B(0));
+    }
+  }
+  for (int e = lane; e < min(cnt, kDictMax); e += 32) { out_off[e] = soff[e]; out_bits[e] = sbits[e]; }
+  if (lane == 0) *out_cnt = min(cnt, kDictMax + 1);
+}
+
+template <class T>
+__global__ void __launch_bounds__(kBlock) dict_encode_kernel(int n, const int* __restrict__ rowptr, const int* __restrict__ colind,
+                                                            const T* __restrict__ val, const void* dict, int ndict,
+                                                            uint8_t* __restrict__ code, int* missing) {
+  typedef DictBits<T> B;
+  __shared__ int soff[kDictMax];
+  __shared__ B sbits[kDictMax];
+  for (int e = threadIdx.x; e < ndict; e += blockDim.x) {
+    soff[e] = reinterpret_cast<const int*>(dict)[e];
+    sbits[e] = dict_bits(reinterpret_cast<const T*>(reinterpret_cast<const int*>(dict) + kDictMax)[e]);
+  }
+  __syncthreads();
+  const int stride = gridDim.x * blockDim.x;
+  for (int row = blockIdx.x * blockDim.x + threadIdx.x; row < n; row += stride) {
+    const int ke = rowptr[row + 1];
+    for (int k = rowptr[row]; k < ke; k++) {
+      const int off = colind[k] - row;
+      const B bits = dict_bits(val[k]);
+      int lo = 0, hi = ndict;
+      while (lo < hi) {
+        const int mid = (lo + hi) >> 1;
+        if (soff[mid] < off || (soff[mid] == off && sbits[mid] < bits)) lo = mid + 1;
+        else hi = mid;
+      }
+      if (lo < ndict && soff[lo] == off && sbits[lo] == bits) code[k] = (uint8_t)lo;
+      else atomicExch(missing, 1);
+    }
+  }
+}
+
+template <class T> static void csr_dict_build(Ctx& c, Csr<T>& A) {
+  typedef DictBits<T> B;
+  const int ncta = sm_count() * 2;
+  char* tmp = nullptr;
+  const size_t tab = (size_t)ncta * kDictMax;
+  const size_t bytes = tab * (sizeof(int) + sizeof(B)) + (size_t)ncta * sizeof(int) + kDictMax * (sizeof(int) + sizeof(B)) + 4 * sizeof(int);
+  KB_CUDA(cudaMalloc((void**)&tmp, bytes));
+  B* cta_bits = (B*)tmp;
+  B* out_bits = cta_bits + tab;
+  int* cta_off = (int*)(out_bits + kDictMax);
+  int* out_off = cta_off + tab;
+  int* cta_cnt = out_off + kDictMax;
+  int* flags = cta_cnt + ncta;
+  int h[3] = {0, 0, 0};
+  std::vector<int> hoff(kDictMax);
+  std::vector<B> hbits(kDictMax);
+  try {
+    KB_CUDA(cudaMemsetAsync(flags, 0, 4 * sizeof(int), c.stream));
+    dict_collect_kernel<T><<<ncta, kDictWarps * 32, 0, c.stream>>>(A.n, A.rowptr, A.colind, A.val, cta_off, cta_bits, cta_cnt, flags);
+    dict_merge_kernel<B><<<1, 32, 0, c.stream>>>(ncta, cta_off, cta_bits, cta_cnt, flags, out_off, out_bits, flags + 1);
+    KB_CUDA(cudaGetLastError());
+    KB_CUDA(cudaMemcpyAsync(h, flags, 2 * sizeof(int), cudaMemcpyDeviceToHost, c.stream));
+    KB_CUDA(cudaMemcpyAsync(hoff.data(), out_off, kDictMax * sizeof(int), cudaMemcpyDeviceToHost, c.stream));
+    KB_CUDA(cudaMemcpyAsync(hbits.data(), out_bits, kDictMax * sizeof(B), cudaMemcpyDeviceToHost, c.stream));
+    c.sync();
+    const int nd = h[1];
+    if (nd >= 1 && nd <= kDictMax) {
+      std::vector<std::pair<int, B>> pairs(nd);
+      for (int e = 0; e < nd; e++) pairs[e] = {hoff[e], hbits[e]};
+      std::sort(pairs.begin(), pairs.end());
+      std::vector<char> hd(TileLayout<T, true>::dict_bytes(), 0);
+      int* doff = (int*)hd.data();
+      T* dval = (T*)(doff + kDictMax);
+      for (int e = 0; e < nd; e++) { doff[e] = pairs[e].first; memcpy(&dval[e], &pairs[e].second, sizeof(T)); }
+      A.dict = dev_alloc<char>(hd.size());
+      A.code = reinterpret_cast<uint8_t*>(dev_alloc<char>((size_t)A.nnz + 64));
+      KB_CUDA(cudaMemcpyAsync(A.dict, hd.data(), hd.size(), cudaMemcpyHostToDevice, c.stream));
+      KB_CUDA(cudaMemsetAsync(A.code + A.nnz, 0, 64, c.stream));
+      dict_encode_kernel<T><<<sm_count() * 4, kBlock, 0, c.stream>>>(A.n, A.rowptr, A.colind, A.val, A.dict, nd, A.code, flags + 2);
+      KB_CUDA(cudaGetLastError());
+      KB_CUDA(cudaMemcpyAsync(&h[2], flags + 2, sizeof(int), cudaMemcpyDeviceToHost, c.stream));
+      c.sync();
+      if (h[2]) throw std::runtime_error("CSR operator: dictionary encoding lost a (column offset, value) pair");
+      A.ndict = nd;
+    }
+  } catch (...) {
+    cudaFree(tmp);
+    throw;
+  }
+  cudaFree(tmp);
 }
 
 template <class T> void csr_plan(Ctx& c, Csr<T>& A) {
@@ -146,6 +313,7 @@
     if (L.total_bytes(s) <= two_cta) { A.tma_ok = true; A.stages = s; per_sm = 2; }
   for (int s = 4; s >= 2 && !A.tma_ok; s--)
     if (L.total_bytes(s) <= one_cta) { A.tma_ok = true; A.stages = s; per_sm = 1; }
+  const bool default_plan = A.tma_ok && per_sm == 3 && !(es && ec);
   if (A.tma_ok) {
     A.smem_bytes = L.total_bytes(A.stages);
     int g = sm_count() * per_sm;
@@ -153,6 +321,17 @@
     A.ctas_per_sm = per_sm;
   } else {
     A.stages = 0; A.smem_bytes = 0; A.grid = 0;
+  }
+  const char* ed = getenv("KB200_CSR_DICT");
+  if (default_plan && A.nnz > 0 && !(ed && atoi(ed) == 0)) {
+    const TileLayout<T, true> Ld{A.tile_cap};
+    for (int s = 4; s >= 2 && !A.dict_stages; s--)
+      if (Ld.total_bytes(s) * 3 <= 226 * 1024) A.dict_stages = s;
+    if (A.dict_stages) {
+      csr_dict_build<T>(c, A);
+      if (A.ndict) A.dict_smem_bytes = Ld.total_bytes(A.dict_stages);
+      else A.dict_stages = 0;
+    }
   }
 }
 
@@ -175,13 +354,13 @@
   }
 }
 
-template <class T, bool DOT, class G>
+template <class T, bool DOT, class G, bool DICT>
 __global__ void __launch_bounds__(kTileThreads, 3) spmv_tma_kernel(Csr<T> A, G xg, T* __restrict__ y, T* part,
                                                                 unsigned* ticket, T* out) {
   extern __shared__ __align__(128) unsigned char smem[];
   __shared__ T sm[32];
   T dacc = T(0);
-  spmv_tiles_run<T>(
+  spmv_tiles_run<T, DICT>(
       A, smem, xg, [&](int row) { return DOT ? __ldg(&xg.x[row]) : T(0); },
       [&](int row, T acc, T xr) {
         y[row] = acc;
@@ -199,12 +378,17 @@
   const bool staged = variant == 2 || (variant == 0 && A.tma_ok);
   if (staged) {
     if (!A.tma_ok) throw std::runtime_error("TMA-staged SpMV requested but the tile plan does not fit shared memory");
-    ensure_dyn_smem((const void*)spmv_tma_kernel<T, DOT, G>, 220 * 1024);
+    auto kern = spmv_tma_kernel<T, DOT, G, false>;
+    size_t smem = A.smem_bytes;
+    if constexpr (std::is_same<G, XPlain<T>>::value) {
+      if (A.ndict > 0) { kern = spmv_tma_kernel<T, DOT, G, true>; smem = A.dict_smem_bytes; }
+    }
+    ensure_dyn_smem((const void*)kern, 220 * 1024);
     int occ = 0;
-    KB_CUDA(cudaOccupancyMaxActiveBlocksPerMultiprocessor(&occ, spmv_tma_kernel<T, DOT, G>, kTileThreads, A.smem_bytes));
+    KB_CUDA(cudaOccupancyMaxActiveBlocksPerMultiprocessor(&occ, kern, kTileThreads, smem));
     if (occ < 1) throw std::runtime_error("spmv_tma_kernel does not fit on an SM with the planned shared-memory ring");
     const int grid = std::min(std::min(occ, A.ctas_per_sm) * sm_count(), std::max(1, A.ntiles));
-    spmv_tma_kernel<T, DOT, G><<<grid, kTileThreads, A.smem_bytes, c.stream>>>(A, xg, y, (T*)c.partials, c.tickets + 1, out);
+    kern<<<grid, kTileThreads, smem, c.stream>>>(A, xg, y, (T*)c.partials, c.tickets + 1, out);
   } else {
     const int grid = stream_grid(A.n, 1, 8);
     spmv_rows_kernel<T, DOT, G><<<grid, kBlock, 0, c.stream>>>(A, xg, y, (T*)c.partials, c.tickets + 1, out);
diff --git a/krylov.jl_b200/csrc/spmv_tiles.cuh b/krylov.jl_b200/csrc/spmv_tiles.cuh
--- a/krylov.jl_b200/csrc/spmv_tiles.cuh
+++ b/krylov.jl_b200/csrc/spmv_tiles.cuh
@@ -71,25 +71,76 @@
   return pol;
 }
 
-template <class T>
+template <class T, bool DICT = false>
 struct TileLayout {
   int cap;
   __host__ __device__ static constexpr size_t align_up(size_t v) { return (v + 127) & ~size_t(127); }
   __host__ __device__ size_t rp_bytes() const { return align_up((kTileRows + 4) * sizeof(int)); }
   __host__ __device__ size_t val_bytes() const { return align_up((size_t)(cap + 16 / sizeof(T)) * sizeof(T)); }
   __host__ __device__ size_t col_bytes() const { return align_up((size_t)(cap + 8) * sizeof(int)); }
-  __host__ __device__ size_t stage_bytes() const { return rp_bytes() + val_bytes() + col_bytes(); }
-  __host__ __device__ size_t total_bytes(int stages) const { return 128 + (size_t)stages * stage_bytes(); }
-};
+  __host__ __device__ size_t code_bytes() const { return align_up((size_t)cap + 32); }
+  __host__ __device__ static constexpr size_t dict_bytes() { return DICT ? (size_t)kDictMax * (sizeof(int) + sizeof(T)) : 0; }
+  __host__ __device__ size_t stage_bytes() const { return rp_bytes() + (DICT ? code_bytes() : val_bytes() + col_bytes()); }
+  __host__ __device__ static constexpr size_t ring_offset() { return 128 + dict_bytes(); }
+  __host__ __device__ size_t total_bytes(int stages) const { return ring_offset() + (size_t)stages * stage_bytes(); }
+};
+
+template <class T, bool DICT>
+__device__ __forceinline__ void tile_stage_issue(const Csr<T>& A, const TileLayout<T, DICT>& L, unsigned char* st, uint64_t* bar,
+                                                 int t, int k0, int k1, uint64_t pol) {
+  const unsigned rp_b = (kTileRows + 4) * sizeof(int);
+  if constexpr (DICT) {
+    const int k0b = k0 & ~15, k1b = (k1 + 15) & ~15;
+    const unsigned c_b = (unsigned)(k1b - k0b);
+    mbar_expect_tx(bar, rp_b + c_b);
+    tma_load_1d(st, A.rowptr + t * kTileRows, rp_b, bar, pol);
+    if (c_b) tma_load_1d(st + L.rp_bytes(), A.code + k0b, c_b, bar, pol);
+  } else {
+    constexpr int VA = 16 / sizeof(T);
+    const int k0v = k0 & ~(VA - 1), k1v = (k1 + VA - 1) & ~(VA - 1);
+    const int k0c = k0 & ~3, k1c = (k1 + 3) & ~3;
+    const unsigned v_b = (unsigned)(k1v - k0v) * sizeof(T);
+    const unsigned c_b = (unsigned)(k1c - k0c) * sizeof(int);
+    mbar_expect_tx(bar, rp_b + v_b + c_b);
+    tma_load_1d(st, A.rowptr + t * kTileRows, rp_b, bar, pol);
+    if (v_b) tma_load_1d(st + L.rp_bytes(), A.val + k0v, v_b, bar, pol);
+    if (c_b) tma_load_1d(st + L.rp_bytes() + L.val_bytes(), A.colind + k0c, c_b, bar, pol);
+  }
+}
+
+template <class T>
+__device__ __forceinline__ void dict_to_smem(const Csr<T>& A, unsigned char* smem) {
+  constexpr int words = (int)(TileLayout<T, true>::dict_bytes() / sizeof(uint4));
+  const uint4* src = reinterpret_cast<const uint4*>(A.dict);
+  uint4* dst = reinterpret_cast<uint4*>(smem + 128);
+  for (int i = threadIdx.x; i < words; i += blockDim.x) dst[i] = __ldg(&src[i]);
+}
+
+template <class T, int DEPTH, class Gather>
+__device__ __forceinline__ T dict_row_sum(const uint8_t* crow, const int* doff, const T* dval, int row, int kb, int ke,
+                                          Gather gather) {
+  T acc = T(0);
+  for (int k = kb; k < ke; k += DEPTH) {
+    T xv[DEPTH];
+#pragma unroll
+    for (int u = 0; u < DEPTH; u++) xv[u] = gather(row + doff[crow[min(k + u, ke - 1)]]);
+    asm volatile("" ::: "memory");
+#pragma unroll
+    for (int u = 0; u < DEPTH; u++) {
+      const T nx = add_rn(acc, mul_rn(dval[crow[min(k + u, ke - 1)]], xv[u]));
+      acc = (k + u < ke) ? nx : acc;
+    }
+  }
+  return acc;
+}
 
 struct NoRowBegin {
   __device__ __forceinline__ int operator()(int) const { return 0; }
 };
 
-template <class T>
-__device__ __forceinline__ void tile_producer(const Csr<T>& A, const TileLayout<T>& L, int S, unsigned char* ring, uint64_t* full,
+template <class T, bool DICT = false>
+__device__ __forceinline__ void tile_producer(const Csr<T>& A, const TileLayout<T, DICT>& L, int S, unsigned char* ring, uint64_t* full,
                                               uint64_t* empty) {
-  constexpr int VA = 16 / sizeof(T);
   const uint64_t pol = l2_evict_first_policy();
   int it = 0;
   int t = blockIdx.x;
@@ -101,32 +152,23 @@
     if (tn < A.ntiles) { nk0 = __ldg(&A.rowptr[tn * kTileRows]); nk1 = __ldg(&A.rowptr[min(tn * kTileRows + kTileRows, A.n)]); }
     const int s = it % S;
     mbar_wait(&empty[s], ((it / S) & 1) ^ 1);
-    unsigned char* st = ring + (size_t)s * L.stage_bytes();
-    const int r0 = t * kTileRows;
-    const int k0v = k0 & ~(VA - 1), k1v = (k1 + VA - 1) & ~(VA - 1);
-    const int k0c = k0 & ~3, k1c = (k1 + 3) & ~3;
-    const unsigned rp_b = (kTileRows + 4) * sizeof(int);
-    const unsigned v_b = (unsigned)(k1v - k0v) * sizeof(T);
-    const unsigned c_b = (unsigned)(k1c - k0c) * sizeof(int);
-    mbar_expect_tx(&full[s], rp_b + v_b + c_b);
-    tma_load_1d(st, A.rowptr + r0, rp_b, &full[s], pol);
-    if (v_b) tma_load_1d(st + L.rp_bytes(), A.val + k0v, v_b, &full[s], pol);
-    if (c_b) tma_load_1d(st + L.rp_bytes() + L.val_bytes(), A.colind + k0c, c_b, &full[s], pol);
+    tile_stage_issue<T, DICT>(A, L, ring + (size_t)s * L.stage_bytes(), &full[s], t, k0, k1, pol);
     k0 = nk0; k1 = nk1;
   }
 }
 
-template <class T, class Gather, class RowBegin, class RowDone>
+template <class T, bool DICT = false, class Gather, class RowBegin, class RowDone>
 __device__ __forceinline__ void spmv_tiles_run(const Csr<T>& A, unsigned char* smem, Gather gather, RowBegin row_begin,
                                                RowDone row_done) {
-  const TileLayout<T> L{A.tile_cap};
-  const int S = A.stages;
+  const TileLayout<T, DICT> L{A.tile_cap};
+  const int S = DICT ? A.dict_stages : A.stages;
   uint64_t* full = reinterpret_cast<uint64_t*>(smem);
   uint64_t* empty = full + S;
-  unsigned char* ring = smem + 128;
+  unsigned char* ring = smem + L.ring_offset();
   const int tid = threadIdx.x, warp = tid >> 5, lane = tid & 31;
   constexpr int VA = 16 / sizeof(T);
 
+  if (DICT) dict_to_smem<T>(A, smem);
   if (tid == 0) {
     for (int s = 0; s < S; s++) { mbar_init(&full[s], 1); mbar_init(&empty[s], kConsumerWarps); }
     asm volatile("fence.mbarrier_init.release.cluster;" ::: "memory");
@@ -134,7 +176,7 @@
   __syncthreads();
 
   if (warp == kConsumerWarps) {
-    if (lane == 0) tile_producer<T>(A, L, S, ring, full, empty);
+    if (lane == 0) tile_producer<T, DICT>(A, L, S, ring, full, empty);
   } else {
     int it = 0;
     for (int t = blockIdx.x; t < A.ntiles; t += gridDim.x, it++) {
@@ -144,9 +186,14 @@
       mbar_wait(&full[s], (it / S) & 1);
       const unsigned char* st = ring + (size_t)s * L.stage_bytes();
       const int* rp = reinterpret_cast<const int*>(st);
-      const T* vs = reinterpret_cast<const T*>(st + L.rp_bytes());
-      const int* cs = reinterpret_cast<const int*>(st + L.rp_bytes() + L.val_bytes());
-      if (row < A.n) {
+      if (DICT && row < A.n) {
+        const uint8_t* crow = reinterpret_cast<const uint8_t*>(st + L.rp_bytes()) - (rp[0] & ~15);
+        const int* doff = reinterpret_cast<const int*>(smem + 128);
+        const T* dval = reinterpret_cast<const T*>(doff + kDictMax);
+        row_done(row, dict_row_sum<T, kGatherDepth>(crow, doff, dval, row, rp[tid], rp[tid + 1], gather), pre);
+      } else if (row < A.n) {
+        const T* vs = reinterpret_cast<const T*>(st + L.rp_bytes());
+        const int* cs = reinterpret_cast<const int*>(st + L.rp_bytes() + L.val_bytes());
         const int k0 = rp[0];
         const T* vrow = vs - (k0 & ~(VA - 1));
         const int* crow = cs - (k0 & ~3);
@@ -187,19 +234,24 @@
 }
 
 
-template <class T>
+template <class T, bool DICT = false>
 struct TilePipe {
-  TileLayout<T> L;
+  TileLayout<T, DICT> L;
   int S;
   uint64_t* full;
   uint64_t* empty;
   unsigned char* ring;
+  const int* doff;
+  const T* dval;
   __device__ __forceinline__ void init(const Csr<T>& A, unsigned char* smem) {
-    L = TileLayout<T>{A.tile_cap};
-    S = A.stages;
+    L = TileLayout<T, DICT>{A.tile_cap};
+    S = DICT ? A.dict_stages : A.stages;
     full = reinterpret_cast<uint64_t*>(smem);
     empty = full + S;
-    ring = smem + 128;
+    ring = smem + L.ring_offset();
+    doff = reinterpret_cast<const int*>(smem + 128);
+    dval = reinterpret_cast<const T*>(doff + kDictMax);
+    if (DICT) dict_to_smem<T>(A, smem);
     if (threadIdx.x == 0) {
       for (int s = 0; s < S; s++) { mbar_init(&full[s], 1); mbar_init(&empty[s], kConsumerWarps); }
       asm volatile("fence.mbarrier_init.release.cluster;" ::: "memory");
@@ -208,10 +260,9 @@
   }
 };
 
-template <class T, class TileAt>
-__device__ __forceinline__ void tile_issue_until(const Csr<T>& A, const TilePipe<T>& P, unsigned& pos, unsigned target, int cnt,
+template <class T, bool DICT, class TileAt>
+__device__ __forceinline__ void tile_issue_until(const Csr<T>& A, const TilePipe<T, DICT>& P, unsigned& pos, unsigned target, int cnt,
                                                  TileAt tile_at, uint64_t pol) {
-  constexpr int VA = 16 / sizeof(T);
   if (pos >= target) return;
   int t = tile_at((int)(pos % (unsigned)cnt)) & 0x7fffffff;
   int k0 = __ldg(&A.rowptr[t * kTileRows]), k1 = __ldg(&A.rowptr[min(t * kTileRows + kTileRows, A.n)]);
@@ -223,27 +274,18 @@
     }
     const int s = (int)(pos % (unsigned)P.S);
     mbar_wait(&P.empty[s], ((pos / (unsigned)P.S) & 1) ^ 1);
-    unsigned char* st = P.ring + (size_t)s * P.L.stage_bytes();
-    const int k0v = k0 & ~(VA - 1), k1v = (k1 + VA - 1) & ~(VA - 1);
-    const int k0c = k0 & ~3, k1c = (k1 + 3) & ~3;
-    const unsigned rp_b = (kTileRows + 4) * sizeof(int);
-    const unsigned v_b = (unsigned)(k1v - k0v) * sizeof(T);
-    const unsigned c_b = (unsigned)(k1c - k0c) * sizeof(int);
-    mbar_expect_tx(&P.full[s], rp_b + v_b + c_b);
-    tma_load_1d(st, A.rowptr + t * kTileRows, rp_b, &P.full[s], pol);
-    if (v_b) tma_load_1d(st + P.L.rp_bytes(), A.val + k0v, v_b, &P.full[s], pol);
-    if (c_b) tma_load_1d(st + P.L.rp_bytes() + P.L.val_bytes(), A.colind + k0c, c_b, &P.full[s], pol);
+    tile_stage_issue<T, DICT>(A, P.L, P.ring + (size_t)s * P.L.stage_bytes(), &P.full[s], t, k0, k1, pol);
     t = tn; k0 = nk0; k1 = nk1;
   }
 }
 
-template <class T>
-__device__ __forceinline__ void tile_drain(const TilePipe<T>& P, unsigned consumed, unsigned pos) {
+template <class T, bool DICT>
+__device__ __forceinline__ void tile_drain(const TilePipe<T, DICT>& P, unsigned consumed, unsigned pos) {
   for (unsigned q = consumed; q < pos; q++) mbar_wait(&P.full[q % (unsigned)P.S], (q / (unsigned)P.S) & 1);
 }
 
-template <class T, int DEPTH, class TileAt, class Gather, class RowBegin, class RowDone>
-__device__ __forceinline__ void tile_consume_pass(const Csr<T>& A, const TilePipe<T>& P, unsigned& cpos, int j0, int j1, TileAt tile_at,
+template <class T, int DEPTH, bool DICT, class TileAt, class Gather, class RowBegin, class RowDone>
+__device__ __forceinline__ void tile_consume_pass(const Csr<T>& A, const TilePipe<T, DICT>& P, unsigned& cpos, int j0, int j1, TileAt tile_at,
                                                   Gather gather, RowBegin row_begin, RowDone row_done) {
   constexpr int VA = 16 / sizeof(T);
   const int tid = threadIdx.x, lane = tid & 31;
@@ -255,9 +297,12 @@
     mbar_wait(&P.full[s], (cpos / (unsigned)P.S) & 1);
     const unsigned char* st = P.ring + (size_t)s * P.L.stage_bytes();
     const int* rp = reinterpret_cast<const int*>(st);
-    const T* vs = reinterpret_cast<const T*>(st + P.L.rp_bytes());
-    const int* cs = reinterpret_cast<const int*>(st + P.L.rp_bytes() + P.L.val_bytes());
-    if (row < A.n) {
+    if (DICT && row < A.n) {
+      const uint8_t* crow = reinterpret_cast<const uint8_t*>(st + P.L.rp_bytes()) - (rp[0] & ~15);
+      row_done(row, dict_row_sum<T, DEPTH>(crow, P.doff, P.dval, row, rp[tid], rp[tid + 1], gather), pre);
+    } else if (row < A.n) {
+      const T* vs = reinterpret_cast<const T*>(st + P.L.rp_bytes());
+      const int* cs = reinterpret_cast<const int*>(st + P.L.rp_bytes() + P.L.val_bytes());
       const int k0 = rp[0];
       const T* vrow = vs - (k0 & ~(VA - 1));
       const int* crow = cs - (k0 & ~3);
diff --git a/krylov.jl_b200/krylov_b200/_lib.py b/krylov.jl_b200/krylov_b200/_lib.py
--- a/krylov.jl_b200/krylov_b200/_lib.py
+++ b/krylov.jl_b200/krylov_b200/_lib.py
@@ -76,6 +76,7 @@
     "krylov_b200_set_operator_csr": (_I, [_P, _I, _LL, _P, _P, _P, _I, _I, _I]),
     "krylov_b200_share_operator": (_I, [_P, _P]),
     "krylov_b200_attach_csr": (_I, [_P, _P]),
+    "krylov_b200_operator_encoding": (_I, [_P]),
     "krylov_b200_set_preconditioner_diag": (_I, [_P, _I, _P, _I]),
     "krylov_b200_set_preconditioner_blockdiag": (C.c_int, [_P, C.c_int, C.c_int, _P, C.c_int]),
     "krylov_b200_default_options": (KrylovB200Options, []),
diff --git a/profiles/ab_csr_dict.py b/profiles/ab_csr_dict.py
--- /dev/null
+++ b/profiles/ab_csr_dict.py
@@ -0,0 +1,69 @@
+import argparse
+import json
+import os
+import statistics
+import subprocess
+import sys
+import tempfile
+
+import numpy as np
+
+ROOT = os.path.dirname(os.path.dirname(os.path.abspath(__file__)))
+CMD = ["--no-cpu", "--no-extra", "--no-cfg5", "--steps", "20", "--warmup", "3"]
+
+
+def dict_bytes_per_iteration(n, nnz):
+    return nnz * 1 + (n + 1) * 4 + 9 * n * 8
+
+
+def run(tree, dump):
+    p = subprocess.run([sys.executable, "bench.py", *CMD, "--dump-outputs", dump], cwd=tree, capture_output=True,
+                       text=True)
+    if p.returncode != 0:
+        sys.stderr.write(p.stdout[-4000:] + p.stderr[-4000:])
+        raise SystemExit(f"bench.py failed in {tree}")
+    return json.loads([l for l in p.stdout.splitlines() if l.startswith("{")][-1])
+
+
+def main():
+    ap = argparse.ArgumentParser()
+    ap.add_argument("--base", required=True, help="tree of the parent commit, built")
+    ap.add_argument("--runs", type=int, default=5)
+    ap.add_argument("--out", help="directory for the dumped outputs and ab.json (default: a new temporary directory)")
+    args = ap.parse_args()
+    args.out = os.path.abspath(args.out or tempfile.mkdtemp(prefix="ab_csr_dict_"))
+    arms = {"base": os.path.abspath(args.base), "branch": ROOT}
+    res = {a: [] for a in arms}
+    for i in range(args.runs):
+        for a, tree in arms.items():
+            line = run(tree, os.path.join(args.out, a))
+            res[a].append(line)
+            print(f"run {i} {a:6s} {line['value']:9.1f} it/s  phase A {line['roofline']['kernels']['phase_a']['ms'] * 1e3:6.1f} us"
+                  f"  phase B {line['roofline']['kernels']['phase_b']['ms'] * 1e3:5.1f} us", flush=True)
+    summary = {}
+    for a, lines in res.items():
+        v = [l["value"] for l in lines]
+        med = sorted(lines, key=lambda l: l["value"])[len(lines) // 2]
+        n, nnz, peak = med["config"]["n"], med["config"]["nnz"], med["roofline"]["peak"]
+        summary[a] = dict(values=v, median=statistics.median(v), min=min(v), max=max(v),
+                          phase_a_us=med["roofline"]["kernels"]["phase_a"]["ms"] * 1e3,
+                          phase_b_us=med["roofline"]["kernels"]["phase_b"]["ms"] * 1e3,
+                          frac_csr_model=med["roofline"]["frac"],
+                          frac_dict_model=dict_bytes_per_iteration(n, nnz) * statistics.median(v) / 1e9 / peak,
+                          peak_GBs=peak, clocks=med.get("clocks"))
+    summary["speedup_median"] = summary["branch"]["median"] / summary["base"]["median"]
+    summary["every_branch_run_faster"] = summary["branch"]["min"] > summary["base"]["max"]
+    same = {}
+    for name in ("x", "x_index", "niter", "solved"):
+        a = np.load(os.path.join(args.out, "base", name + ".npy"))
+        b = np.load(os.path.join(args.out, "branch", name + ".npy"))
+        same[name] = bool(np.array_equal(a, b))
+    summary["outputs_identical"] = same
+    os.makedirs(args.out, exist_ok=True)
+    json.dump(summary, open(os.path.join(args.out, "ab.json"), "w"), indent=1)
+    print(json.dumps(summary, indent=1))
+    print(f"outputs and ab.json in {args.out}")
+
+
+if __name__ == "__main__":
+    main()
```

Result: faster. 4554 (median of 6 runs) (+24.6%).
